# Unsigned-Long/slam-tricks

Hardware: AMD Instinct MI355X
Metric: LM iterations/sec + residuals/sec, 1k-cam/100k-pt BA (higher is better)
Workload: dtype f64

## Files before the change

slam-tricks_amd/csrc/ba_kernels.hip:

```cpp
#include <algorithm>

#include "ba_kernels.hpp"

namespace stba {

template <bool CAMS_IN_LDS, bool WITH_JAC>
__global__ __launch_bounds__(LIN_THREADS) void ba_linearize_kernel(LinArgs a) {
    extern __shared__ __attribute__((aligned(16))) double smem[];
    double* s_j8 = smem;
    double* s_cam = smem + (WITH_JAC ? LIN_THREADS * 9 : 0);
    const int tid = threadIdx.x;
    if (CAMS_IN_LDS) {
        for (int i = tid; i < a.n_cams * 7; i += LIN_THREADS) s_cam[i] = a.cams[i];
        __syncthreads();
    }
    double cost = 0.0;
    const int n_tiles = (a.n_obs + LIN_THREADS - 1) / LIN_THREADS;
    for (int tile = blockIdx.x; tile < n_tiles; tile += gridDim.x) {
        const int base = tile * LIN_THREADS;
        const int i = base + tid;
        if (i < a.n_obs) {
            const double2 f = a.feat[i];
            const int c = a.obs_cam[i], j = a.obs_pt[i];
            const double* cam = CAMS_IN_LDS ? (s_cam + c * 7) : (a.cams + (size_t)c * 7);
// ... 451 lines not shown
#pragma unroll
        for (int k = 0; k < 6; ++k) Hi[k] = 0.0;
    }
#pragma unroll
    for (int k = 0; k < 6; ++k) Hinv6[(size_t)j * 6 + k] = Hi[k];
}

__global__ __launch_bounds__(256) void ba_point_damp_invert_kernel(int n_pts, const double* __restrict__ Hpp6,
                                                                   const unsigned char* __restrict__ pt_fixed,
                                                                   double* __restrict__ scale, int init_scale, int use_scaling,
                                                                   double radius, double dmin, double dmax, double* __restrict__ dp,
                                                                   double* __restrict__ Hinv6, double* __restrict__ zero_buf, int zero_n) {
    const int j = blockIdx.x * 256 + threadIdx.x;
    if (j < zero_n) zero_buf[j] = 0.0;
    if (j >= n_pts) return;
    double H[6], Hi[6] = {0, 0, 0, 0, 0, 0};
#pragma unroll
    for (int k = 0; k < 6; ++k) H[k] = Hpp6[(size_t)j * 6 + k];
    const int dg[3] = {0, 3, 5};
#pragma unroll
    for (int k = 0; k < 3; ++k) {
        const size_t i = (size_t)j * 3 + k;
        const double h = H[dg[k]];
        double s = 1.0;
        if (use_scaling) {
            if (init_scale) { s = 1.0 / (1.0 + sqrt(h)); scale[i] = s; }
            else s = scale[i];
        } else if (init_scale) scale[i] = 1.0;
        const double s2 = s * s;
        const double v = fmin(fmax(h * s2, dmin), dmax);
        const double d = v / radius / s2;
        dp[i] = d;
        H[dg[k]] = h + d;
    }
    const bool fixed = pt_fixed ? (pt_fixed[j] != 0) : false;
    if (fixed || !inv3_sym6(H, Hi)) {
#pragma unroll
        for (int k = 0; k < 6; ++k) Hi[k] = 0.0;
    }
#pragma unroll
    for (int k = 0; k < 6; ++k) Hinv6[(size_t)j * 6 + k] = Hi[k];
}

int launch_point_damp_invert(int n_pts, const double* Hpp6, const unsigned char* pt_fixed, double* scale, int init_scale,
                             int use_scaling, double radius, double dmin, double dmax, double* dp, double* Hinv6,
                             double* zero_buf, int zero_n, hipStream_t st) {
    hipLaunchKernelGGL(ba_point_damp_invert_kernel, dim3((std::max(n_pts, zero_n) + 255) / 256), dim3(256), 0, st, n_pts, Hpp6, pt_fixed, scale,
                       init_scale, use_scaling, radius, dmin, dmax, dp, Hinv6, zero_buf, zero_n);
    STBA_HIP(hipGetLastError());
    return STBA_OK;
}

int launch_point_invert(int n_pts, const double* Hpp6, const double* dp, const unsigned char* pt_fixed,
                        double* Hinv6, hipStream_t st) {
    hipLaunchKernelGGL(ba_point_invert_kernel, dim3((n_pts + 255) / 256), dim3(256), 0, st, n_pts, Hpp6, dp,
                       pt_fixed, Hinv6);
    STBA_HIP(hipGetLastError());
    return STBA_OK;
}

template <int ROTS, bool GEN = false, int MODE = 0>
__global__ __launch_bounds__(SCHUR_THREADS, GEN ? 2 : 4) void ba_schur_pairs_kernel(SchurArgs a) {
    extern __shared__ __attribute__((aligned(16))) double smem[];
    const int task = blockIdx.x;
    const int c = a.task_cam[task];
    const int row_ncols = a.row_col_ptr[c + 1] - a.row_col_ptr[c];
    const int clo = a.task_col_lo[task], chi = a.task_col_hi[task];
    const int col0 = a.row_col_ptr[c] + clo, ncols = chi - clo;
    double* acc = smem;
    double* racc = smem + (size_t)a.max_cols * SCHUR_BLK_LD;
    double* cpart = racc + 8;
    int* cols = reinterpret_cast<int*>(cpart + 8 * SCHUR_CAM_LD);
    int* vsf = cols + a.max_cols;
    const int tid = threadIdx.x;
    const bool diag_piece = (chi == row_ncols);
    const int* vs_g = a.vs_first + a.task_vs_ptr[task];
    const int nslots = vs_g[ncols];
    for (int e = tid; e < nslots * SCHUR_BLK_LD; e += SCHUR_THREADS) acc[e] = 0.0;
    if (tid < 8) racc[tid] = 0.0;
    for (int e = tid; e < ncols; e += SCHUR_THREADS) cols[e] = a.row_cols[col0 + e];
    for (int e = tid; e <= ncols; e += SCHUR_THREADS) vsf[e] = vs_g[e];
    if (tid == 0) vsf[a.max_cols + 1] = 0;
    const bool lms = a.part != nullptr;
    if (!lms) {
        const int cend = min(a.lda, ((c * 6 + 5) / 128 + 1) * 128);
        const int z0 = (clo == 0) ? 0 : 6 * a.row_cols[col0];
        const int z1 = diag_piece ? cend : 6 * a.row_cols[col0 + ncols];
        for (int q = 0; q < 6; ++q) {
            double* row = a.S + (size_t)(c * 6 + q) * a.lda;
            for (int e = z0 + tid; e < z1; e += SCHUR_THREADS) row[e] = 0.0;
        }
    }
    __syncthreads();
    const int wv = tid >> 6;
    constexpr int mode = MODE;
    const int stride = mode == 0 ? 64 : SCHUR_THREADS;
    const int ent = task * (SCHUR_THREADS / 64) + (mode == 0 ? wv : 0);
    const int kb = a.pair_begin[ent], ke = a.pair_end[ent];
    const int ntrips = (ke - kb + stride - 1) / stride;
    int* turn = vsf + a.max_cols + 1;
    int k = kb + (mode == 0 ? (tid & 63) : tid);
    int4 rn = (k < ke) ? a.pair_rec[k] : make_int4(0, 0, 0, 0);
    for (int trip = 0; mode == 0 ? (k < ke) : (trip < ntrips); ++trip, k += stride) {
        const int4 rc = rn;
        const bool valid = mode == 0 ? true : (k < ke);
        if (k + stride < ke) rn = a.pair_rec[k + stride];
        if (mode == 1) {
        }
        double Hi[6], jc[12], jp[6], jc2[12], jp2[6];
#ifdef STBA_DEBUG_KNOBS
        const int gi = (a.ablate & 1) ? (rc.x & 63) : rc.x, gl = (a.ablate & 1) ? (rc.y & 63) : rc.y, gz = (a.ablate & 1) ? (rc.z & 63) : rc.z;
#else
        const int gi = rc.x, gl = rc.y, gz = rc.z;
#endif
#pragma unroll
        for (int k2 = 0; k2 < 6; ++k2) Hi[k2] = a.Hinv6[(size_t)gz * 6 + k2];
        load_jc_jp<GEN>(a.J8, a.omask, gi, jc, jp, a.Jc12);
        load_jc_jp<GEN>(a.J8, a.omask, gl, jc2, jp2, a.Jc12);
        const unsigned sl = (unsigned)rc.w;
        const int rot = (int)((sl >> 16) & 7u);
        double E[18];
#pragma unroll
        for (int q = 0; q < 6; ++q) {
            const double w0 = jc[q] * jp[0] + jc[6 + q] * jp[3];
            const double w1 = jc[q] * jp[1] + jc[6 + q] * jp[4];
            const double w2 = jc[q] * jp[2] + jc[6 + q] * jp[5];
            E[q * 3 + 0] = w0 * Hi[0] + w1 * Hi[1] + w2 * Hi[2];
            E[q * 3 + 1] = w0 * Hi[1] + w1 * Hi[3] + w2 * Hi[4];
            E[q * 3 + 2] = w0 * Hi[2] + w1 * Hi[4] + w2 * Hi[5];
        }
        double* blk = acc + (size_t)(sl & 0x3fffu) * SCHUR_BLK_LD;
        if (mode == 1) {
            const int want = trip * (SCHUR_THREADS / 64) + wv;
            while (__hip_atomic_load(turn, __ATOMIC_RELAXED, __HIP_MEMORY_SCOPE_WORKGROUP) != want) __builtin_amdgcn_s_sleep(1);
        }
        if (valid) {
#pragma unroll
        for (int s2 = 0; s2 < 6; ++s2) {
            double ja = jc2[s2], jb = jc2[6 + s2];
            int b = s2;
#pragma unroll
            for (int r = 1; r < ROTS; ++r) {
                const int bb = (s2 + r * (6 / ROTS)) % 6;
                if (rot == r) { ja = jc2[bb]; jb = jc2[6 + bb]; b = bb; }
            }
            const double w0 = ja * jp2[0] + jb * jp2[3];
            const double w1 = ja * jp2[1] + jb * jp2[4];
            const double w2 = ja * jp2[2] + jb * jp2[5];
            double* col = blk + b;
#ifdef STBA_DEBUG_KNOBS
            if (a.ablate & 2) {
                double sacc = 0.0;
#pragma unroll
                for (int q = 0; q < 6; ++q) sacc += E[q * 3] * w0 + E[q * 3 + 1] * w1 + E[q * 3 + 2] * w2;
                if (sacc == 1.2345e300) unsafeAtomicAdd(&col[0], sacc);
            } else
#endif
#pragma unroll
            for (int q = 0; q < 6; ++q)
                unsafeAtomicAdd(&col[q * 6], -(E[q * 3] * w0 + E[q * 3 + 1] * w1 + E[q * 3 + 2] * w2));
        }
        }
        if (mode == 1) {
            asm volatile("s_waitcnt lgkmcnt(0)" ::: "memory");
            if ((tid & 63) == 0) __hip_atomic_store(turn, trip * (SCHUR_THREADS / 64) + wv + 1, __ATOMIC_RELAXED, __HIP_MEMORY_SCOPE_WORKGROUP);
        }
    }
    if (diag_piece) {
        const int pb = lms ? a.task_p_lo[task] : a.cam_start[c];
        const int pe = lms ? a.task_p_hi[task] : a.cam_start[c + 1];
        {
            double h[27];
#pragma unroll
            for (int k = 0; k < 27; ++k) h[k] = 0.0;
            for (int p = pb + tid; p < pe; p += SCHUR_THREADS) {
// ... 1008 lines not shown
```

slam-tricks_amd/csrc/common.hpp:

```cpp
#pragma once
#include <hip/hip_runtime.h>

#include <chrono>
#include <cmath>
#include <cstdio>
#include <cstdlib>
#include <cstring>
#include <mutex>
#include <string>

#include "../../include/stba.h"

namespace stba {

extern thread_local std::string g_last_error;
inline int fail(int code, const std::string& msg) {
    g_last_error = msg;
    return code;
}
#define STBA_HIP(call)                                                                       \
    do {                                                                                     \
        hipError_t e_ = (call);                                                              \
        if (e_ != hipSuccess) {                                                              \
            return ::stba::fail((e_ == hipErrorNoDevice || e_ == hipErrorInvalidDevice)      \
// ... 83 lines not shown
        for (int q = 7; q >= 0; --q) w[q] = src[q];
        double st;
        std::memcpy(&st, &w[7], sizeof st);
        if (!accept(st) || (L > 0 && st != first_stamp)) return false;
        first_stamp = st;
        unsigned long long chk = stamped_mix(STAMPED_SALT, w[7]);
        for (int q = 0; q < STAMPED_PAYLOAD; ++q) chk = stamped_mix(chk, w[q]);
        if (chk != w[6]) return false;
        for (int q = 0; q < STAMPED_PAYLOAD; ++q) {
            const int pi = L * STAMPED_PAYLOAD + q;
            if (pi < n_payload) std::memcpy(&payload[pi], &w[q], sizeof(double));
        }
    }
    if (stamp_out) *stamp_out = first_stamp;
    return true;
}

enum class StreamState { running, finished, failed };
constexpr unsigned long STAMPED_QUERY_EVERY = 1ul << 14;
template <class Accept, class StreamCheck>
inline int stamped_wait(const volatile double* block, int n_payload, Accept accept, double* payload, StreamCheck stream_state,
                        const char* who, double limit_s) {
    const auto t0 = std::chrono::steady_clock::now();
    for (unsigned long n = 1; !stamped_try_read(block, n_payload, accept, payload); ++n) {
        if (n % STAMPED_QUERY_EVERY == 0) {
            std::string why;
            const StreamState s = stream_state(&why);
            if (s == StreamState::failed) return fail(STBA_ERR_HIP, std::string(who) + ": stream failed: " + why);
            if (s == StreamState::finished) {
                if (stamped_try_read(block, n_payload, accept, payload)) return STBA_OK;
                return fail(STBA_ERR_HIP, std::string(who) + ": the stream finished without writing the block the host waits for");
            }
            if (std::chrono::duration<double>(std::chrono::steady_clock::now() - t0).count() > limit_s)
                return fail(STBA_ERR_HIP, std::string(who) + ": timed out waiting for the device");
        }
#if defined(__x86_64__)
        __builtin_ia32_pause();
#endif
    }
    return STBA_OK;
}
inline auto hip_stream_state(hipStream_t st) {
    return [st](std::string* why) {
        hipError_t q = hipStreamQuery(st);
        if (q == hipErrorNotReady) return StreamState::running;
        if (q == hipSuccess) q = hipStreamSynchronize(st);
        if (q == hipSuccess) return StreamState::finished;
        *why = hipGetErrorString(q);
        return StreamState::failed;
    };
}

struct MappedBuffer {
    double* host = nullptr;
    double* dev = nullptr;
    size_t count = 0;
    int alloc(size_t n) {
        release();
        void *h = nullptr, *d = nullptr;
        STBA_HIP(hipHostMalloc(&h, n * sizeof(double), hipHostMallocMapped | hipHostMallocCoherent));
        const hipError_t e = hipHostGetDevicePointer(&d, h, 0);
        if (e != hipSuccess) {
            (void)hipHostFree(h);
            return fail(STBA_ERR_HIP, std::string("hipHostGetDevicePointer: ") + hipGetErrorString(e));
        }
        host = static_cast<double*>(h); dev = static_cast<double*>(d); count = n;
        zero();
        return STBA_OK;
    }
    void zero() { if (host) memset(host, 0, count * sizeof(double)); }
    void release() {
        if (host) (void)hipHostFree(host);
        host = dev = nullptr;
        count = 0;
    }
};

constexpr int CHOL_NB = 128;
inline int chol_padded_dim(int n) { return ((n + 1 + CHOL_NB - 1) / CHOL_NB) * CHOL_NB; }
constexpr int CHOL_FLAG_TIMEOUT = -2147483647;
inline int chol_flag_status(int flag_h) {
    return flag_h == CHOL_FLAG_TIMEOUT ? fail(STBA_ERR_HIP, "dense Cholesky: the persistent program timed out waiting for a dependency and the caller has no way to rebuild the matrix") : STBA_OK;
}
int chol_factor_solve_dev(double* A_dev, int lda, int n, double* x_dev, int* flag_dev, hipStream_t st);
int chol_factor_solve_stages(double* A_dev, int lda, int n, double* x_dev, int* flag_dev, hipStream_t st);
void chol_forget_stream(hipStream_t st);
void chol_note_timeout();
void chol_note_peer_timeout();
void chol_count_timeout();
void chol_set_spin_limit_us(double us);
int chol_timeout_count();

int chol_factor_solve_split(double* A_dev, int lda, int n, double* x_dev, int* flag_dev, hipStream_t st, hipEvent_t mid_event,
                            hipEvent_t pre_event = nullptr);
struct CholProfile {
    double ms_diag, ms_trsm, ms_syrk, ms_bwd;
    double syrk_flops;
    double syrk_flops_padded;
    int syrk_launches;
};
int chol_factor_solve_profiled(double* A_dev, int lda, int n, double* x_dev, int* flag_dev, hipStream_t st,
                               CholProfile* prof);
double chol_schedule_makespan(int nblk, int nq, int wg_per_q);
void chol_shard_model(int nblk, int n_gpus, int n_xcd, int wg_per_q, int rows_per_group, double hop_us, double tile_us, double* out3);
int chol_shard_row_owner(int row, int n_gpus, int rows_per_group);
int chol_prepare_padding_dev(double* A_dev, int lda, int n, const double* rhs_dev, hipStream_t st);
size_t chol_yyt_workspace_doubles(int lda, size_t kcols);
int chol_yyt_lower_dev(const double* Y, size_t ldy, size_t kcols, double* S, int lda, double* ws, hipStream_t st);
size_t chol_spd_inverse_workspace_doubles(int np);
int chol_spd_inverse_dev(double* W, int ldw, int np, int n_real, int* flag_dev, double* work, hipStream_t st);

__host__ __device__ inline void quat_to_rot(const double q[4], double R[9]) {
    const double x = q[0], y = q[1], z = q[2], w = q[3];
    const double xx = x * x, yy = y * y, zz = z * z;
    const double xy = x * y, xz = x * z, yz = y * z, wx = w * x, wy = w * y, wz = w * z;
    R[0] = 1 - 2 * (yy + zz); R[1] = 2 * (xy - wz);     R[2] = 2 * (xz + wy);
    R[3] = 2 * (xy + wz);     R[4] = 1 - 2 * (xx + zz); R[5] = 2 * (yz - wx);
    R[6] = 2 * (xz - wy);     R[7] = 2 * (yz + wx);     R[8] = 1 - 2 * (xx + yy);
}

__host__ __device__ inline void so3_exp(const double w[3], double q[4]) {
    const double th2 = w[0] * w[0] + w[1] * w[1] + w[2] * w[2];
    double imag, real;
    if (th2 < 1e-20) {
        const double th4 = th2 * th2;
        imag = 0.5 - th2 / 48.0 + th4 / 3840.0;
        real = 1.0 - th2 / 8.0 + th4 / 384.0;
    } else {
        const double th = sqrt(th2);
        imag = sin(0.5 * th) / th;
        real = cos(0.5 * th);
    }
    q[0] = imag * w[0]; q[1] = imag * w[1]; q[2] = imag * w[2]; q[3] = real;
}

__host__ __device__ inline void so3_plus(const double q[4], const double d[3], double out[4]) {
    double e[4];
    so3_exp(d, e);
    const double ax = q[0], ay = q[1], az = q[2], aw = q[3];
    const double bx = e[0], by = e[1], bz = e[2], bw = e[3];
    const double ox = aw * bx + ax * bw + ay * bz - az * by;
    const double oy = aw * by - ax * bz + ay * bw + az * bx;
    const double oz = aw * bz + ax * by - ay * bx + az * bw;
    const double ow = aw * bw - ax * bx - ay * by - az * bz;
    const double n = sqrt(ox * ox + oy * oy + oz * oz + ow * ow);
    out[0] = ox / n; out[1] = oy / n; out[2] = oz / n; out[3] = ow / n;
}

__host__ __device__ inline void left_jacobian_coeffs(double th2, double& a, double& b) {
    if (th2 < 1e-20) { a = 0.5 - th2 / 24.0; b = 1.0 / 6.0 - th2 / 120.0; return; }
    const double th = sqrt(th2), s = sin(0.5 * th) / (0.5 * th);
    a = 0.5 * s * s;
    b = (th - sin(th)) / (th2 * th);
}

__host__ __device__ inline void se3_exp_rt(const double xi[6], double R[9], double t[3]) {
    double q[4];
    so3_exp(xi + 3, q);
    quat_to_rot(q, R);
    const double w0 = xi[3], w1 = xi[4], w2 = xi[5];
    double a, b;
    left_jacobian_coeffs(w0 * w0 + w1 * w1 + w2 * w2, a, b);
    const double K[9] = {0, -w2, w1, w2, 0, -w0, -w1, w0, 0};
    double K2[9];
    for (int i = 0; i < 3; ++i)
        for (int j = 0; j < 3; ++j) K2[i * 3 + j] = K[i * 3] * K[j] + K[i * 3 + 1] * K[3 + j] + K[i * 3 + 2] * K[6 + j];
    for (int i = 0; i < 3; ++i) {
        double s = 0.0;
// ... 61 lines not shown
```

slam-tricks_amd/csrc/dense_chol.hip:

```cpp
#include <algorithm>
#include <atomic>
#include <cstdlib>
#include <map>
#include <mutex>
#include <queue>
#include <string>
#include <vector>

#include "common.hpp"

namespace stba {

constexpr int NB = CHOL_NB;
#ifndef MEGA_WAIT_SLEEP
#define MEGA_WAIT_SLEEP 1
#endif
#ifndef MEGA_POLL_SLEEP
#define MEGA_POLL_SLEEP 16
#endif

typedef double double4v __attribute__((ext_vector_type(4)));

__global__ void chol_pad_kernel(double* __restrict__ A, int lda, int n, const double* __restrict__ rhs) {
    const int r = n + blockIdx.x;
// ... 240 lines not shown
#pragma unroll
            for (int d = C - 1; d >= 1; --d) acc[d] = __builtin_amdgcn_mfma_f64_16x16x4f64(-lj[d], lprev, acc[d], 0, 0, 0);
            acc[0] = __builtin_amdgcn_mfma_f64_16x16x4f64(-lprev, lprev, acc[0], 0, 0, 0);
        }
        lprev = l;
    }
    if (C == 2) {
#pragma unroll
        for (int r = 0; r < 4; ++r) { sm.Mig[R & 1][0][r][lane] = acc[1][r]; sm.Mig[R & 1][1][r][lane] = acc[0][r]; }
    }
}

__device__ __forceinline__ void d2_bulk_row(const double* __restrict__ Ab, int lda, Diag2Smem& sm, int lane, int R) {
    const int n = lane & 15, g = lane >> 4;
    double4v acc[8];
#pragma unroll
    for (int d = 0; d < 8; ++d) if (d <= R) acc[d] = d2_load_tile(sm, R, R - d, n, g);
    double lprev = 0.0;
    switch (R) {
        case 7: d2_bulk_column<7>(sm, R, acc, lprev, lane); [[fallthrough]];
        case 6: d2_bulk_column<6>(sm, R, acc, lprev, lane); [[fallthrough]];
        case 5: d2_bulk_column<5>(sm, R, acc, lprev, lane); [[fallthrough]];
        case 4: d2_bulk_column<4>(sm, R, acc, lprev, lane); [[fallthrough]];
        case 3: d2_bulk_column<3>(sm, R, acc, lprev, lane); [[fallthrough]];
        default: d2_bulk_column<2>(sm, R, acc, lprev, lane);
    }
}

template <bool WT>
__device__ __forceinline__ void d2_bulk_wave(const double* __restrict__ Ab, int lda, Diag2Smem& sm, int lane, int R, int einv,
                                             double* __restrict__ dinv) {
    const int n = lane & 15, g = lane >> 4;
    d2_bulk_row(Ab, lda, sm, lane, R);
    double4v accE;
    auto inverse_step = [&](int I, int s) {
        const double le = mfma_l(sm.Gp[4 * I + s][lane], accE[s]);
        gst<WT>(&dinv[(I * 16 + 4 * s + g) * 16 + n], le);
        if (s < 3) accE = __builtin_amdgcn_mfma_f64_16x16x4f64(-sm.Lsl[d2_tix(I, I)][s][lane], le, accE, 0, 0, 0);
    };
#pragma unroll 1
    for (int J = R - 1; J < 8; ++J) {
        const int Ie = einv == 0 ? J - 1 : (einv == 1 && J == R - 1) ? 0 : -1;
        if (Ie >= 0) {
#pragma unroll
            for (int r = 0; r < 4; ++r) accE[r] = (n == 4 * r + g) ? 1.0 : 0.0;
        }
#pragma unroll
        for (int s = 0; s < 4; ++s) {
            D2_BARRIER();
            if (Ie >= 0) inverse_step(Ie, s);
        }
        if (J < 7) D2_BARRIER();
    }
    D2_BARRIER();
    if (einv == 1) {
#pragma unroll
        for (int r = 0; r < 4; ++r) accE[r] = (n == 4 * r + g) ? 1.0 : 0.0;
#pragma unroll
        for (int s = 0; s < 4; ++s) inverse_step(7, s);
    }
}

template <bool WT>
__device__ __forceinline__ void d2_store_wave(double* __restrict__ A, const double* __restrict__ Ab, int lda, int k0, Diag2Smem& sm, int lane) {
    d2_bulk_row(Ab, lda, sm, lane, 2);
#pragma unroll 1
    for (int J = 1; J < 8; ++J) {
#pragma unroll
        for (int s = 0; s < 4; ++s) {
            D2_BARRIER();
#pragma unroll
            for (int h = 0; h < 2; ++h) {
                const int Ip = (J - 1) + 2 * s + h;
                if (Ip < 8) d2_store_tile<WT>(A, lda, k0, sm, Ip, J - 1, lane);
            }
        }
        if (J < 7) D2_BARRIER();
    }
    D2_BARRIER();
    d2_store_tile<WT>(A, lda, k0, sm, 7, 7, lane);
}

template <bool WT>
__device__ __forceinline__ void diag_block2(double* __restrict__ A, int lda, int k0, int n_real,
                                            int* __restrict__ flag, double* __restrict__ dinv, double* smem, int t,
                                            long long* ph = nullptr) {
    Diag2Smem& sm = *reinterpret_cast<Diag2Smem*>(smem);
    const int w = __builtin_amdgcn_readfirstlane(t >> 6), lane = t & 63;
    const double* Ab = A + (size_t)k0 * lda + k0;
    PHASE_STAMP(0);
    d2_stage_block(Ab, lda, sm, t);
    D2_BARRIER();
    if (w == 0) d2_factor_wave(Ab, lda, k0, n_real, flag, sm, lane, ph);
    else if (w == 1) d2_follower_wave(Ab, lda, sm, lane);
    else if (w == 4) d2_store_wave<WT>(A, Ab, lda, k0, sm, lane);
    else d2_bulk_wave<WT>(Ab, lda, sm, lane, w == 5 ? 5 : w == 2 ? 7 : w == 6 ? 3 : w == 3 ? 6 : 4, w == 6 ? 0 : w == 7 ? 1 : -1, dinv);
}

__global__ __launch_bounds__(512) void chol_diag_kernel(double* __restrict__ A, int lda, int k0, int n_real,
                                                         int* __restrict__ flag, double* __restrict__ dinv) {
    extern __shared__ __attribute__((aligned(16))) double sm2[];
    diag_block2<false>(A, lda, k0, n_real, flag, dinv, sm2, threadIdx.x);
}

template <bool WT>
__device__ __forceinline__ void trsm_group(double* __restrict__ rowp, bool ident, int ident_row0, int nv,
                                           const double* __restrict__ Lb, int lda,
                                           const double* __restrict__ dinv, int lane) {
    const int n = lane & 15, g = lane >> 4;
    const int pm = 4 * (n & 3) + (n >> 2);
    double4v W[8];
#pragma unroll
    for (int J = 0; J < 8; ++J) {
        if (ident) {
#pragma unroll
            for (int r = 0; r < 4; ++r) W[J][r] = (16 * J + 4 * g + r == ident_row0 + n) ? 1.0 : 0.0;
        } else {
            W[J] = gld4(rowp + 16 * J + 4 * g);
        }
    }
    auto load_l = [&](int J, int I) -> double4v {
        const int row = 16 * J + pm;
        double4v v = gld4(Lb + (size_t)row * lda + 16 * I + 4 * g);
        if (row >= nv) v = double4v{0.0, 0.0, 0.0, 0.0};
        return -v;
    };
    auto load_inv = [&](int J) -> double4v {
        double4v v = gld4(dinv + (J * 16 + pm) * 16 + 4 * g);
        if (16 * J + pm >= nv) {
#pragma unroll
            for (int q = 0; q < 4; ++q) v[q] = (4 * g + q == pm) ? 1.0 : 0.0;
        }
        return v;
    };
    double4v Lc[8], Ln[8], iv, ivn;
    iv = load_inv(0);
#pragma unroll
    for (int J = 1; J < 8; ++J) Lc[J] = load_l(J, 0);
#pragma unroll
    for (int I = 0; I < 8; ++I) {
        if (I + 1 < 8) {
            ivn = load_inv(I + 1);
#pragma unroll
            for (int J = I + 2; J < 8; ++J) Ln[J] = load_l(J, I + 1);
        }
        double4v y = {0.0, 0.0, 0.0, 0.0};
#pragma unroll
        for (int q = 0; q < 4; ++q) y = __builtin_amdgcn_mfma_f64_16x16x4f64(iv[q], W[I][q], y, 0, 0, 0);
        W[I] = y;
#pragma unroll
        for (int J = I + 1; J < 8; ++J)
#pragma unroll
            for (int q = 0; q < 4; ++q) W[J] = __builtin_amdgcn_mfma_f64_16x16x4f64(Lc[J][q], y[q], W[J], 0, 0, 0);
        iv = ivn;
#pragma unroll
        for (int J = I + 2; J < 8; ++J) Lc[J] = Ln[J];
    }
#pragma unroll
    for (int J = 0; J < 8; ++J) gst4<WT>(rowp + 16 * J + 4 * g, W[J]);
}

__global__ __launch_bounds__(64) void chol_trsm_kernel(double* __restrict__ A, int lda, int k0, int n_groups,
                                                       double* __restrict__ Xinv, const double* __restrict__ dinv) {
    const int lane = threadIdx.x, grp = blockIdx.x;
    const bool ident = grp >= n_groups;
    const int e = grp - n_groups;
    const int nv = ident ? min(NB, (lda - 1) - k0) : NB;
    double* rowp = ident ? Xinv + (size_t)(16 * e + (lane & 15)) * NB
                         : A + (size_t)(k0 + NB + 16 * grp + (lane & 15)) * lda + k0;
    trsm_group<false>(rowp, ident, 16 * e, nv, A + (size_t)k0 * lda + k0, lda, dinv, lane);
}

template <int TM>
__global__ __launch_bounds__(256) void chol_syrk_kernel(double* __restrict__ A, int lda, int k0, int tile_mode) {
    constexpr int RBA = TM / 16;
    constexpr int WR = TM / 64;
    constexpr int WC = 4 / WR;
    constexpr int MB = 4;
    constexpr int NBK = 8 / WC;
    constexpr int PA = TM / 64;
    __shared__ __attribute__((aligned(16))) double sA[2][TM * 16];
    __shared__ __attribute__((aligned(16))) double sB[2][2048];
    const int sub = (TM == 64) ? (blockIdx.x & 1) : 0;
    const int id = (TM == 64) ? (blockIdx.x >> 1) : blockIdx.x;
    int ti, tj;
// ... 19 lines not shown
#pragma unroll
            for (int r = 0; r < 4; ++r) {
                const int row = row_i + wr * (MB * 16) + m * 16 + (lane >> 4) + 4 * r;
                const int col = row_j + wc * (NBK * 16) + n * 16 + (lane & 15);
                acc[m][n][r] = A[(size_t)row * lda + col];
            }

    double2 ga[PA][2], gb[2][2];
    const int lrow = lane & 15, lkp = lane >> 4;
    auto gload = [&](int kc) {
#pragma unroll
        for (int p = 0; p < 2; ++p)
#pragma unroll
            for (int h = 0; h < 2; ++h) {
                const int row = lrow + 16 * (w + 4 * p);
                const int k = 2 * (lkp + 4 * h);
                if (p < PA) ga[p < PA ? p : 0][h] = *reinterpret_cast<const double2*>(&A[(size_t)(row_i + row) * lda + k0 + kc * 16 + k]);
                gb[p][h] = *reinterpret_cast<const double2*>(&A[(size_t)(row_j + row) * lda + k0 + kc * 16 + k]);
            }
    };
    auto lstore = [&](int buf) {
#pragma unroll
        for (int p = 0; p < 2; ++p)
#pragma unroll
            for (int h = 0; h < 2; ++h) {
                const int rb = w + 4 * p;
                const int k = 2 * (lkp + 4 * h);
                if (p < PA) {
                    const int posa = (((k >> 2) * RBA + rb) << 6) + ((k & 3) << 4) + lrow;
                    sA[buf][posa] = ga[p < PA ? p : 0][h].x;
                    sA[buf][posa + 16] = ga[p < PA ? p : 0][h].y;
                }
                const int posb = (((k >> 2) * 8 + rb) << 6) + ((k & 3) << 4) + lrow;
                sB[buf][posb] = gb[p][h].x;
                sB[buf][posb + 16] = gb[p][h].y;
            }
    };
    gload(0);
    lstore(0);
    __syncthreads();
    constexpr int KC = NB / 16;
    for (int kc = 0; kc < KC; ++kc) {
        const int buf = kc & 1;
        if (kc + 1 < KC) gload(kc + 1);
#pragma unroll
        for (int kq = 0; kq < 4; ++kq) {
            double a[MB], b[NBK];
#pragma unroll
            for (int m = 0; m < MB; ++m) a[m] = -sA[buf][((kq * RBA + wr * MB + m) << 6) + lane];
#pragma unroll
            for (int n = 0; n < NBK; ++n) b[n] = sB[buf][((kq * 8 + wc * NBK + n) << 6) + lane];
#pragma unroll
            for (int m = 0; m < MB; ++m)
#pragma unroll
                for (int n = 0; n < NBK; ++n)
                    acc[m][n] = __builtin_amdgcn_mfma_f64_16x16x4f64(a[m], b[n], acc[m][n], 0, 0, 0);
        }
        if (kc + 1 < KC) lstore(buf ^ 1);
        __syncthreads();
    }
#pragma unroll
    for (int m = 0; m < MB; ++m)
#pragma unroll
        for (int n = 0; n < NBK; ++n)
#pragma unroll
            for (int r = 0; r < 4; ++r) {
                const int row = row_i + wr * (MB * 16) + m * 16 + (lane >> 4) + 4 * r;
                const int col = row_j + wc * (NBK * 16) + n * 16 + (lane & 15);
                A[(size_t)row * lda + col] = acc[m][n][r];
            }
}

static void launch_syrk(double* A, int lda, int k0, int tile_mode, int tiles128, hipStream_t st) {
    const bool use64 = tiles128 < 1000000;
    if (use64) hipLaunchKernelGGL(chol_syrk_kernel<64>, dim3(2 * tiles128), dim3(256), 0, st, A, lda, k0, tile_mode);
    else hipLaunchKernelGGL(chol_syrk_kernel<128>, dim3(tiles128), dim3(256), 0, st, A, lda, k0, tile_mode);
}

enum { TASK_D = 0, TASK_T = 1, TASK_TI = 2, TASK_U = 3, TASK_UQ = 4, TASK_TU = 5 };

constexpr int MEGA_MAX_Q = 16;
struct MegaArgs {
    double* A; int lda; int n; int nblk;
    const int4* tasks;
    int nq;
    int lstart[MEGA_MAX_Q + 1];
    signed char xcc_queue[16];
    int* sync;
    double* linv; size_t linv_stride;
    double* vbuf; int nwide;
    long long spin_limit;
    int* flag;
    long long* trace;
};
constexpr int MEGA_SYNC_HDR = MEGA_MAX_Q + 1;
constexpr int MEGA_ABORT = MEGA_MAX_Q;
constexpr int MEGA_SMEM_BYTES = 128 * 1024;
constexpr int MEGA_PREDRAW_NB = 2;

__device__ __forceinline__ int xcc_id() {
    unsigned v;
    asm volatile("s_getreg_b32 %0, hwreg(HW_REG_XCC_ID)" : "=s"(v));
    return (int)(v & 15u);
}
__global__ void xcc_probe_kernel(int* out) {
    if (threadIdx.x == 0) out[blockIdx.x] = xcc_id();
}

template <int TM, int KCH = 16>
__device__ __forceinline__ void syrk_tile512(double* __restrict__ A, int lda, int k0, int row_i, int row_j,
                                             double* smem, int t, int kchunks = NB / 16) {
    constexpr int WR = (TM == 128) ? 2 : 1, WC = 8 / WR;
    constexpr int MB = TM / (16 * WR);
    constexpr int NBK = 8 / WC;
    constexpr int RBA = TM / 16;
    constexpr int SA = TM * KCH, SB = 128 * KCH, NH = KCH / 8;
    double* sA = smem;
    double* sB = smem + 2 * SA;
    const int lane = t & 63, w = t >> 6;
    const int wr = w / WC, wc = w % WC;
    double4v acc[MB][NBK];
#pragma unroll
    for (int m = 0; m < MB; ++m)
#pragma unroll
        for (int n = 0; n < NBK; ++n)
#pragma unroll
            for (int r = 0; r < 4; ++r) {
                const int row = row_i + wr * (MB * 16) + m * 16 + (lane >> 4) + 4 * r;
                const int col = row_j + wc * (NBK * 16) + n * 16 + (lane & 15);
                acc[m][n][r] = A[(size_t)row * lda + col];
            }
    double2 ga[NH], gb[NH];
    const int lrow = lane & 15, lkp = lane >> 4;
    const bool stage_a = (RBA == 8) ? true : (w < RBA);
    auto gload = [&](int kc) {
#pragma unroll
        for (int h = 0; h < NH; ++h) {
            const int row = lrow + 16 * w;
            const int k = 2 * (lkp + 4 * h);
            if (stage_a) ga[h] = *reinterpret_cast<const double2*>(&A[(size_t)(row_i + row) * lda + k0 + kc * KCH + k]);
            gb[h] = *reinterpret_cast<const double2*>(&A[(size_t)(row_j + row) * lda + k0 + kc * KCH + k]);
        }
    };
    auto lstore = [&](int buf) {
#pragma unroll
        for (int h = 0; h < NH; ++h) {
            const int k = 2 * (lkp + 4 * h);
            if (stage_a) {
                const int posa = (((k >> 2) * RBA + w) << 6) + ((k & 3) << 4) + lrow;
                sA[buf * SA + posa] = -ga[h].x;
                sA[buf * SA + posa + 16] = -ga[h].y;
            }
            const int posb = (((k >> 2) * 8 + w) << 6) + ((k & 3) << 4) + lrow;
            sB[buf * SB + posb] = gb[h].x;
            sB[buf * SB + posb + 16] = gb[h].y;
        }
    };
    gload(0);
    lstore(0);
    __syncthreads();
    const int KC = kchunks * 16 / KCH;
    auto chunk = [&](int kc, int buf) {
        if (kc + 1 < KC) gload(kc + 1);
#pragma unroll
        for (int kq = 0; kq < KCH / 4; ++kq) {
            double a[MB], b[NBK];
#pragma unroll
            for (int m = 0; m < MB; ++m) a[m] = sA[buf * SA + (((kq * RBA + wr * MB + m) << 6) + lane)];
#pragma unroll
            for (int n = 0; n < NBK; ++n) b[n] = sB[buf * SB + (((kq * 8 + wc * NBK + n) << 6) + lane)];
#pragma unroll
            for (int m = 0; m < MB; ++m)
#pragma unroll
                for (int n = 0; n < NBK; ++n)
                    acc[m][n] = __builtin_amdgcn_mfma_f64_16x16x4f64(a[m], b[n], acc[m][n], 0, 0, 0);
        }
        if (kc + 1 < KC) lstore(buf ^ 1);
        __syncthreads();
    };
    for (int kc = 0; kc < KC; ++kc) chunk(kc, kc & 1);
#pragma unroll
    for (int m = 0; m < MB; ++m)
#pragma unroll
        for (int n = 0; n < NBK; ++n)
#pragma unroll
            for (int r = 0; r < 4; ++r) {
                const int row = row_i + wr * (MB * 16) + m * 16 + (lane >> 4) + 4 * r;
                const int col = row_j + wc * (NBK * 16) + n * 16 + (lane & 15);
                gst<false>(&A[(size_t)row * lda + col], acc[m][n][r]);
            }
}

template <int TM>
__device__ __forceinline__ void syrk_tile512_gen(double* __restrict__ Cb, int ldc, const double* __restrict__ Pi, size_t ldi,
                                             const double* __restrict__ Pj, size_t ldj, bool c_zero, double* smem, int t, int kchunks = NB / 16) {
    constexpr int WR = (TM == 128) ? 2 : 1, WC = 8 / WR;
    constexpr int MB = TM / (16 * WR);
    constexpr int NBK = 8 / WC;
    constexpr int RBA = TM / 16;
    double* sA = smem;
    double* sB = smem + 2 * TM * 16;
    const int lane = t & 63, w = t >> 6;
    const int wr = w / WC, wc = w % WC;
    double4v acc[MB][NBK];
#pragma unroll
    for (int m = 0; m < MB; ++m)
#pragma unroll
        for (int n = 0; n < NBK; ++n)
#pragma unroll
            for (int r = 0; r < 4; ++r) {
                const int row = wr * (MB * 16) + m * 16 + (lane >> 4) + 4 * r;
                const int col = wc * (NBK * 16) + n * 16 + (lane & 15);
                acc[m][n][r] = c_zero ? 0.0 : Cb[(size_t)row * ldc + col];
// ... 69 lines not shown
        if (wall_clock64() - t0 > limit) {
            __hip_atomic_store(abortf, 1, __ATOMIC_RELAXED, __HIP_MEMORY_SCOPE_AGENT);
            return false;
        }
    }
}

__device__ __forceinline__ bool trsm_compute512(double4v (&W)[8], const double* __restrict__ rowp, bool ident,
                                                int ident_row0, int nv, const double* __restrict__ Lb, int lda,
                                                const double* __restrict__ dinv, double* smem, int t, long long* ph,
                                                const int* dflag, int* abortf, int* s_ok, long long spin_limit, bool flag_known = false,
                                                bool active = true) {
    const int lane = t & 63;
    const int n = lane & 15, g = lane >> 4;
#pragma unroll
    for (int J = 0; J < 8; ++J) {
        if (!active) {
#pragma unroll
            for (int r = 0; r < 4; ++r) W[J][r] = 0.0;
        } else if (ident) {
#pragma unroll
            for (int r = 0; r < 4; ++r) W[J][r] = (16 * J + 4 * g + r == ident_row0 + n) ? 1.0 : 0.0;
        } else {
            W[J] = gld4(rowp + 16 * J + 4 * g);
        }
    }
    if (!flag_known) {
        if (t == 0) {
            *s_ok = mega_wait(dflag, 1, abortf, spin_limit) ? 1 : 0;
            asm volatile("buffer_inv sc1\n\ts_waitcnt vmcnt(0)" ::: "memory");
        }
        __syncthreads();
        if (!*s_ok) return false;
    }
    {
        double v[18];
#pragma unroll
        for (int s2 = 0; s2 < 18; ++s2) {
            const int e = t + 512 * s2;
            const int tile = e >> 8, r = (e >> 4) & 15, c = e & 15;
            if (s2 < 14) {
                const int I = (tile >= 27) ? 6 : (tile >= 25) ? 5 : (tile >= 22) ? 4 : (tile >= 18) ? 3 : (tile >= 13) ? 2 : (tile >= 7) ? 1 : 0;
                const int J = tile - (7 * I - I * (I - 1) / 2) + I + 1;
                const int row = 16 * J + r;
                v[s2] = -Lb[(size_t)row * lda + 16 * I + c];
                if (row >= nv) v[s2] = 0.0;
            } else {
                const int J = tile - 28;
                v[s2] = dinv[(J * 16 + r) * 16 + c];
                if (16 * J + r >= nv) v[s2] = (c == r) ? 1.0 : 0.0;
            }
        }
#pragma unroll
        for (int s2 = 0; s2 < 18; ++s2) {
            const int e = t + 512 * s2;
            const int tile = e >> 8, r = (e >> 4) & 15, c = e & 15;
            const int nn = 4 * (r & 3) + (r >> 2);
            smem[tile * 256 + (((c >> 2) << 4) | nn) * 4 + (c & 3)] = v[s2];
        }
    }
    __syncthreads();
    PHASE_STAMP(0);
    if (active) {
#pragma unroll
    for (int I = 0; I < 8; ++I) {
        const double4v iv = *reinterpret_cast<const double4v*>(smem + (28 + I) * 256 + lane * 4);
        double4v y = {0.0, 0.0, 0.0, 0.0};
#pragma unroll
        for (int q = 0; q < 4; ++q) y = __builtin_amdgcn_mfma_f64_16x16x4f64(iv[q], W[I][q], y, 0, 0, 0);
        W[I] = y;
#pragma unroll
        for (int J = I + 1; J < 8; ++J) {
            const int tile = 7 * I - I * (I - 1) / 2 + (J - I - 1);
            const double4v l = *reinterpret_cast<const double4v*>(smem + tile * 256 + lane * 4);
#pragma unroll
            for (int q = 0; q < 4; ++q) W[J] = __builtin_amdgcn_mfma_f64_16x16x4f64(l[q], y[q], W[J], 0, 0, 0);
        }
    }
    }
    PHASE_STAMP(1);
    return true;
}

__device__ __forceinline__ bool trsm_task512(double* __restrict__ rowp, bool ident, int ident_row0, int nv,
                                             const double* __restrict__ Lb, int lda,
                                             const double* __restrict__ dinv, double* smem, int t, long long* ph,
                                             const int* dflag, int* abortf, int* s_ok, long long spin_limit, bool flag_known = false,
                                             bool active = true) {
    double4v W[8];
    if (!trsm_compute512(W, rowp, ident, ident_row0, nv, Lb, lda, dinv, smem, t, ph, dflag, abortf, s_ok, spin_limit, flag_known, active)) return false;
    const int g = (t & 63) >> 4;
    if (active) {
#pragma unroll
        for (int J = 0; J < 8; ++J) gst4<true>(rowp + 16 * J + 4 * g, W[J]);
    }
    PHASE_STAMP(2);
    return true;
}

__device__ __forceinline__ bool tu4_task512(double* __restrict__ A, int lda, int k0, int rb, int q,
                                           const double* __restrict__ dinv, double* smem, int t, long long* ph,
                                           int* loaded, int* ver_diag, const int* dflag, int* abortf, int* s_ok, long long spin_limit,
                                           bool flag_known = false) {
    const int lane = t & 63, w = t >> 6;
    const int n = lane & 15, g = lane >> 4;
    double* rowp = A + (size_t)(rb * NB + 16 * w + n) * lda + k0;
    const int ntile = 4 * q + 3;
    double* Cb = A + (size_t)(rb * NB) * lda + rb * NB;
    double4v acc[2];
    int tm[2], tn[2];
#pragma unroll
    for (int s2 = 0; s2 < 2; ++s2) {
        const int e = w + 8 * s2;
        tm[s2] = (e < 2 * q + 1) ? 2 * q : 2 * q + 1;
        tn[s2] = (e < 2 * q + 1) ? e : e - (2 * q + 1);
        if (e < ntile) {
#pragma unroll
            for (int r = 0; r < 4; ++r) acc[s2][r] = Cb[(size_t)(16 * tm[s2] + g + 4 * r) * lda + 16 * tn[s2] + n];
        }
    }
    double4v W[8];
    if (!trsm_compute512(W, rowp, false, 0, NB, A + (size_t)k0 * lda + k0, lda, dinv, smem, t, ph, dflag, abortf, s_ok, spin_limit, flag_known)) return false;
    __syncthreads();
    if (t == 0) __hip_atomic_fetch_add(loaded, 1, __ATOMIC_RELAXED, __HIP_MEMORY_SCOPE_AGENT);
#pragma unroll
    for (int J = 0; J < 8; ++J) *reinterpret_cast<double4v*>(smem + (w * 8 + J) * 256 + lane * 4) = W[J];
    __syncthreads();
#pragma unroll
    for (int s2 = 0; s2 < 2; ++s2) {
        if (w + 8 * s2 < ntile) {
            const int m = tm[s2], np = tn[s2];
#pragma unroll
            for (int c = 0; c < 8; ++c) {
                const double4v fa = *reinterpret_cast<const double4v*>(smem + (m * 8 + c) * 256 + lane * 4);
                const double4v fb = *reinterpret_cast<const double4v*>(smem + (np * 8 + c) * 256 + lane * 4);
#pragma unroll
                for (int qq = 0; qq < 4; ++qq) acc[s2] = __builtin_amdgcn_mfma_f64_16x16x4f64(-fa[qq], fb[qq], acc[s2], 0, 0, 0);
            }
#pragma unroll
            for (int r = 0; r < 4; ++r) gst<false>(&Cb[(size_t)(16 * m + g + 4 * r) * lda + 16 * np + n], acc[s2][r]);
        }
    }
    asm volatile("s_waitcnt vmcnt(0)" ::: "memory");
    __syncthreads();
    if (t == 0) {
        __hip_atomic_fetch_add(ver_diag, 1, __ATOMIC_RELAXED, __HIP_MEMORY_SCOPE_AGENT);
        *s_ok = mega_wait(loaded, 4, abortf, spin_limit) ? 1 : 0;
    }
    __syncthreads();
    if (!*s_ok) return false;
    if ((w >> 1) == q) {
#pragma unroll
        for (int J = 0; J < 8; ++J) gst4<true>(rowp + 16 * J + 4 * g, W[J]);
    }
    PHASE_STAMP(2);
    return true;
}

constexpr int MEGA_NTU = 10;
__device__ __forceinline__ bool tu_task512(double* __restrict__ A, int lda, int k0, int rb, int q,
                                           const double* __restrict__ dinv, double* smem, int t, long long* ph,
                                           int* loaded, int* done_cnt, int* ver_diag, const int* dflag, int* abortf, int* s_ok, long long spin_limit,
                                           bool flag_known = false) {
    const int lane = t & 63, w = t >> 6;
    const int n = lane & 15, g = lane >> 4;
    int I = 0;
    while ((I + 1) * (I + 2) / 2 <= q) ++I;
    const int J = q - I * (I + 1) / 2;
    const bool diag = (I == J);
    const int nrow = diag ? 2 : 4;
    const bool active = w < nrow;
    const int trow = (w < 2) ? 2 * I + (w & 1) : 2 * J + (w & 1);
    double* rowp = A + (size_t)(rb * NB + 16 * trow + n) * lda + k0;
    const int ntile = diag ? 3 : 4;
    const int lm = diag ? (w >= 1 ? 1 : 0) : (w >> 1), ln = diag ? (w == 2 ? 1 : 0) : 2 + (w & 1);
    const int tm = 2 * I + lm, tn = diag ? 2 * I + ln : 2 * J + (w & 1);
    double* Cb = A + (size_t)(rb * NB) * lda + rb * NB;
    double4v acc = {0.0, 0.0, 0.0, 0.0};
    if (w < ntile) {
#pragma unroll
        for (int r = 0; r < 4; ++r) acc[r] = Cb[(size_t)(16 * tm + g + 4 * r) * lda + 16 * tn + n];
    }
    double4v W[8];
    if (!trsm_compute512(W, rowp, false, 0, NB, A + (size_t)k0 * lda + k0, lda, dinv, smem, t, ph, dflag, abortf, s_ok, spin_limit, flag_known, active)) return false;
    __syncthreads();
    if (t == 0) __hip_atomic_fetch_add(loaded, 1, __ATOMIC_RELAXED, __HIP_MEMORY_SCOPE_AGENT);
    if (active) {
#pragma unroll
        for (int J2 = 0; J2 < 8; ++J2) *reinterpret_cast<double4v*>(smem + (w * 8 + J2) * 256 + lane * 4) = W[J2];
    }
    __syncthreads();
    if (w < ntile) {
#pragma unroll
        for (int c = 0; c < 8; ++c) {
            const double4v fa = *reinterpret_cast<const double4v*>(smem + (lm * 8 + c) * 256 + lane * 4);
            const double4v fb = *reinterpret_cast<const double4v*>(smem + (ln * 8 + c) * 256 + lane * 4);
#pragma unroll
            for (int qq = 0; qq < 4; ++qq) acc = __builtin_amdgcn_mfma_f64_16x16x4f64(-fa[qq], fb[qq], acc, 0, 0, 0);
        }
#pragma unroll
        for (int r = 0; r < 4; ++r) gst<false>(&Cb[(size_t)(16 * tm + g + 4 * r) * lda + 16 * tn + n], acc[r]);
    }
    asm volatile("s_waitcnt vmcnt(0)" ::: "memory");
    __syncthreads();
    if (t == 0) {
        if (__hip_atomic_fetch_add(done_cnt, 1, __ATOMIC_RELAXED, __HIP_MEMORY_SCOPE_AGENT) == MEGA_NTU - 1)
            __hip_atomic_fetch_add(ver_diag, 4, __ATOMIC_RELAXED, __HIP_MEMORY_SCOPE_AGENT);
        *s_ok = (!diag || mega_wait(loaded, MEGA_NTU, abortf, spin_limit)) ? 1 : 0;
    }
    __syncthreads();
    if (!*s_ok) return false;
    if (diag && active) {
#pragma unroll
        for (int J2 = 0; J2 < 8; ++J2) gst4<true>(rowp + 16 * J2 + 4 * g, W[J2]);
    }
    PHASE_STAMP(2);
    return true;
}

__device__ __forceinline__ void syrk_q32(double* __restrict__ A, int lda, int k0, int row_i, int row_j, int t, long long* ph) {
    const int lane = t & 63, w = t >> 6;
    const int n = lane & 15, g = lane >> 4;
    const double* pa0 = A + (size_t)(row_i + n) * lda + k0 + 4 * g;
    const double* pa1 = pa0 + (size_t)16 * lda;
    const double* pb = A + (size_t)(row_j + 16 * w + n) * lda + k0 + 4 * g;
    double4v a0[8], a1[8], bb[8], acc[2];
#pragma unroll
    for (int c = 0; c < 8; ++c) { bb[c] = gld4(pb + 16 * c); a0[c] = gld4(pa0 + 16 * c); a1[c] = gld4(pa1 + 16 * c); }
#pragma unroll
    for (int m = 0; m < 2; ++m)
#pragma unroll
        for (int r = 0; r < 4; ++r) acc[m][r] = A[(size_t)(row_i + 16 * m + g + 4 * r) * lda + row_j + 16 * w + n];
    PHASE_STAMP(0);
#pragma unroll
    for (int c = 0; c < 8; ++c)
#pragma unroll
        for (int q = 0; q < 4; ++q) {
            acc[0] = __builtin_amdgcn_mfma_f64_16x16x4f64(-a0[c][q], bb[c][q], acc[0], 0, 0, 0);
            acc[1] = __builtin_amdgcn_mfma_f64_16x16x4f64(-a1[c][q], bb[c][q], acc[1], 0, 0, 0);
        }
#pragma unroll
    for (int m = 0; m < 2; ++m)
#pragma unroll
        for (int r = 0; r < 4; ++r) gst<false>(&A[(size_t)(row_i + 16 * m + g + 4 * r) * lda + row_j + 16 * w + n], acc[m][r]);
    PHASE_STAMP(1);
}

__global__ __launch_bounds__(256) void chol_reset_kernel(int* __restrict__ sync, int n, int* __restrict__ flag) {
    const int i = blockIdx.x * 256 + threadIdx.x;
    if (i < n) sync[i] = 0;
    if (i == 0) flag[0] = 0;
}

struct MegaView {
    int nblk, nrow;
    int* abortf; int* dflag; int* tuflag; int* tudone; int* tflag; int* ver;
};
__device__ __forceinline__ MegaView mega_view(const MegaArgs& a) {
    MegaView v;
    v.nblk = a.nblk;
    v.nrow = a.nblk + 4 * a.nwide;
    v.abortf = a.sync + MEGA_ABORT;
    v.dflag = a.sync + MEGA_SYNC_HDR;
    v.tuflag = v.dflag + a.nblk;
    v.tudone = v.tuflag + a.nblk;
    v.tflag = v.tudone + a.nblk;
    v.ver = v.tflag + a.nblk * v.nrow;
    return v;
}
__device__ __forceinline__ int mega_ldf(const int* p) { return __hip_atomic_load(p, __ATOMIC_RELAXED, __HIP_MEMORY_SCOPE_AGENT); }
__device__ __forceinline__ bool mega_ready(const MegaView& v, const int4 d, bool& tu_dset) {
    const int type = d.x & 0xff, b = d.y, ti = d.z, tj = d.w;
    const int nblk = v.nblk, nrow = v.nrow;
    auto first_panel = [&](int i) { return i < nblk ? 0 : i - nblk; };
    if (type == TASK_D) return mega_ldf(&v.ver[b * nblk + b]) >= 4 * b;
    if (type == TASK_T) {
        const int ve = mega_ldf(&v.ver[ti * nblk + b]), df = mega_ldf(&v.dflag[b]);
        return (ve >= 4 * (b - first_panel(ti))) & (df >= 1);
    }
    if (type == TASK_TI) return mega_ldf(&v.dflag[b]) >= 1;
    if (type == TASK_TU) {
        const int v0 = mega_ldf(&v.ver[(b + 1) * nblk + b]), v1 = mega_ldf(&v.ver[(b + 1) * nblk + b + 1]), df = mega_ldf(&v.dflag[b]);
        tu_dset = df >= 1;
        return (v0 >= 4 * b) & (v1 >= 4 * b);
    }
    const int i = (type == TASK_UQ) ? (ti >> 2) : ti;
    const int nbp = max(1, (d.x >> 16) & 0xff);
    const int f0 = mega_ldf(&v.tflag[b * nrow + i]), f1 = mega_ldf(&v.tflag[b * nrow + tj]), ve = mega_ldf(&v.ver[i * nblk + tj]);
    return (f0 >= 4) & (f1 >= 4) & (ve >= 4 * (b - nbp + 1 - first_panel(i)));
}

struct MegaTicket {
    int mine = -1;
    int4 md;
    bool done = false;
    int m_raw = 0;
    bool m_pending = false;
};
__device__ __forceinline__ int mega_next_task(const MegaArgs& a, const MegaView& v, MegaTicket& tk, int* ticket, int lbeg, int lend, int lane,
                                              bool& ok, bool& tu_dset, long long& t_poll) {
    t_poll = a.trace ? wall_clock64() : 0;
    ok = true;
    if (tk.mine < 0 && !tk.done) {
        if (!tk.m_pending && lane == 0) tk.m_raw = lbeg + atomicAdd(ticket, 1);
        tk.m_pending = false;
        tk.mine = __builtin_amdgcn_readfirstlane(tk.m_raw);
        if (tk.mine >= lend) { tk.mine = -1; tk.done = true; }
        else tk.md = a.tasks[tk.mine];
    }
    int pick = -2;
    if (tk.mine >= 0) {
        const long long t0 = wall_clock64();
        for (;;) {
            if (mega_ready(v, tk.md, tu_dset)) { pick = tk.mine; tk.mine = -1; break; }
            if (mega_ldf(v.abortf) != 0) { ok = false; pick = -1; break; }
            if (wall_clock64() - t0 > a.spin_limit) {
                __hip_atomic_store(v.abortf, 1, __ATOMIC_RELAXED, __HIP_MEMORY_SCOPE_AGENT);
                ok = false; pick = -1;
                break;
            }
            __builtin_amdgcn_s_sleep(MEGA_POLL_SLEEP);
        }
    }
    asm volatile("buffer_inv sc1\n\ts_waitcnt vmcnt(0)" ::: "memory");
    return pick;
}

__global__ __launch_bounds__(512) void chol_mega_kernel(MegaArgs a) {
    extern __shared__ __attribute__((aligned(16))) double smem[];
    __shared__ int s_task, s_ok, s_dset;
    const int t = threadIdx.x;
    const int nblk = a.nblk;
    const MegaView v = mega_view(a);
    int* abortf = v.abortf;
    int* dflag = v.dflag;
    int* tuflag = v.tuflag;
    const int nrow = v.nrow;
    int* tflag = v.tflag;
    int* ver = v.ver;
    auto tile_ptr = [&](int i, int j, int& ld) -> double* {
        if (i < nblk) { ld = a.lda; return a.A + (size_t)i * NB * a.lda + (size_t)j * NB; }
        const int p = i - nblk, qw = p >> 2;
        ld = 4 * NB;
        return a.vbuf + (size_t)qw * (4 * NB) * (4 * NB) + (size_t)(p & 3) * NB * (4 * NB) + (size_t)(j - 4 * qw) * NB;
    };
    auto first_panel = [&](int i) { return i < nblk ? 0 : i - nblk; };
    const int q = a.xcc_queue[xcc_id()];
    if (q < 0) return;
    int* ticket = a.sync + q;
    const int lbeg = a.lstart[q], lend = a.lstart[q + 1];
    MegaTicket tk;
    for (;;) {
        if (t < 64) {
            bool ok, tu_dset = false;
            long long t_poll;
            const int pick = mega_next_task(a, v, tk, ticket, lbeg, lend, t, ok, tu_dset, t_poll);
            if (t == 0) {
                if (a.trace && pick >= 0) {
                    a.trace[8 * (size_t)pick] = blockIdx.x; a.trace[8 * (size_t)pick + 1] = t_poll;
                    a.trace[8 * (size_t)pick + 2] = wall_clock64();
                }
                s_dset = tu_dset ? 1 : 0;
                s_task = pick;
                s_ok = ok ? 1 : 0;
            }
            if (!tk.done && pick >= 0 && (tk.md.x & 0xff) != TASK_TU && ((tk.md.x >> 16) & 0xff) <= MEGA_PREDRAW_NB) {
                if (t == 0) tk.m_raw = lbeg + atomicAdd(ticket, 1);
                tk.m_pending = true;
            }
        }
        __syncthreads();
        if (!s_ok) {
            if (t == 0) atomicExch(a.flag, CHOL_FLAG_TIMEOUT);
            break;
        }
        const int task = s_task;
        if (task < 0) break;
        const int4 d = a.tasks[task];
        const int type = d.x & 0xff, b = d.y, ti = d.z, tj = d.w;
        const int k0 = b * NB;
        int tt = t;
        asm volatile("" : "+v"(tt));
        double* li = a.linv + (size_t)b * a.linv_stride;
        long long* ph = a.trace ? a.trace + 8 * (size_t)task + 4 : nullptr;
        if (type == TASK_D) {
            diag_block2<true>(a.A, a.lda, k0, a.n, a.flag, li + NB * NB, smem, tt, ph);
        } else if (type == TASK_T) {
            const int lane = tt & 63, w = tt >> 6;
            int ldr;
            const bool active = (tj == 0) || (w < 4);
            const int row_in_tile = (tj == 0 ? 16 * w : 64 * (tj - 1) + 16 * (w & 3)) + (lane & 15);
            double* rowp = tile_ptr(ti, b, ldr) + (size_t)row_in_tile * ldr;
            if (!trsm_task512(rowp, false, 0, NB, a.A + (size_t)k0 * a.lda + k0, a.lda, li + NB * NB, smem, tt, ph, &dflag[b], abortf, &s_ok,
                              a.spin_limit, true, active)) {
                if (t == 0) atomicExch(a.flag, CHOL_FLAG_TIMEOUT);
                break;
            }
        } else if (type == TASK_TI) {
            const int lane = tt & 63, w = tt >> 6;
            const int nv = min(NB, (a.lda - 1) - k0);
            int ldr = NB;
            double* base = li;
            if (b < 4 * a.nwide) base = tile_ptr(nblk + b, b, ldr);
            double* rowp = base + (size_t)(16 * w + (lane & 15)) * ldr;
            if (!trsm_task512(rowp, true, 16 * w, nv, a.A + (size_t)k0 * a.lda + k0, a.lda, li + NB * NB, smem, tt, ph, &dflag[b], abortf, &s_ok,
                              a.spin_limit, true)) {
                if (t == 0) atomicExch(a.flag, CHOL_FLAG_TIMEOUT);
                break;
            }
        } else if (type == TASK_U) {
            if (ti < nblk) {
                const int nbp = max(1, (d.x >> 16) & 0xff);
                syrk_tile512<128>(a.A, a.lda, k0 - (nbp - 1) * NB, ti * NB, tj * NB, smem, tt, nbp * (NB / 16));
            } else {
                int ldc, ldi, ldj;
                double* Cb = tile_ptr(ti, tj, ldc);
                const double* Pi = tile_ptr(ti, b, ldi);
                const double* Pj = tile_ptr(tj, b, ldj);
                syrk_tile512_gen<128>(Cb, ldc, Pi, ldi, Pj, ldj, b == first_panel(ti), smem, tt);
            }
        } else if (type == TASK_TU) {
            const bool tu_ok = (tj == 2)
                ? tu4_task512(a.A, a.lda, k0, b + 1, ti, li + NB * NB, smem, tt, ph, &tuflag[b], &ver[(b + 1) * nblk + b + 1], &dflag[b], abortf, &s_ok,
                              a.spin_limit, s_dset != 0)
                : tu_task512(a.A, a.lda, k0, b + 1, ti, li + NB * NB, smem, tt, ph, &tuflag[b], &v.tudone[b], &ver[(b + 1) * nblk + b + 1], &dflag[b], abortf, &s_ok,
                             a.spin_limit, s_dset != 0);
            if (!tu_ok) {
                if (t == 0) atomicExch(a.flag, CHOL_FLAG_TIMEOUT);
                break;
            }
        } else {
            syrk_q32(a.A, a.lda, k0, (ti >> 2) * NB + (ti & 3) * 32, tj * NB, tt, ph);
        }
        asm volatile("s_waitcnt vmcnt(0)" ::: "memory");
        __syncthreads();
        if (t == 0) {
            if (type == TASK_D) __hip_atomic_fetch_add(&dflag[b], 1, __ATOMIC_RELAXED, __HIP_MEMORY_SCOPE_AGENT);
            else if (type == TASK_T) __hip_atomic_fetch_add(&tflag[b * nrow + ti], tj == 0 ? 4 : 2, __ATOMIC_RELAXED, __HIP_MEMORY_SCOPE_AGENT);
            else if (type == TASK_TI) { if (b < 4 * a.nwide) __hip_atomic_fetch_add(&tflag[b * nrow + nblk + b], 4, __ATOMIC_RELAXED, __HIP_MEMORY_SCOPE_AGENT); }
            else if (type == TASK_TU) { if (tj != 0) __hip_atomic_fetch_add(&tflag[b * nrow + b + 1], 1, __ATOMIC_RELAXED, __HIP_MEMORY_SCOPE_AGENT); }
            else if (type == TASK_U) __hip_atomic_fetch_add(&ver[ti * nblk + tj], 4 * max(1, (d.x >> 16) & 0xff), __ATOMIC_RELAXED, __HIP_MEMORY_SCOPE_AGENT);
            else if (type == TASK_UQ) __hip_atomic_fetch_add(&ver[(ti >> 2) * nblk + tj], 1, __ATOMIC_RELAXED, __HIP_MEMORY_SCOPE_AGENT);
            if (a.trace) a.trace[8 * (size_t)task + 3] = wall_clock64();
        }
    }
}

static int mega_task_row(const int4& tk) {
    switch (tk.x & 0xff) {
        case TASK_D: case TASK_TI: return tk.y;
        case TASK_TU: return tk.y + 1;
        case TASK_T: case TASK_U: return tk.z;
        default: return tk.z >> 2;
    }
}
static std::vector<int> mega_row_owner(int nblk, int nq, int nvirt = 0) {
    std::vector<int> owner((size_t)(nblk + nvirt), 0);
    for (int v = 0; v < nvirt; ++v) owner[(size_t)(nblk + v)] = v % nq;
    std::vector<double> load((size_t)nq, 0.0);
    for (int row = nblk - 1; row >= 0; --row) {
        int best = 0;
        for (int q = 1; q < nq; ++q)
            if (load[(size_t)q] < load[(size_t)best]) best = q;
        owner[(size_t)row] = best;
        load[(size_t)best] += 24.0 * row * (row - 1) / 2.0 + 23.0 * row + 110.0;
    }
    return owner;
}
struct MegaShardModel {
    int n_gpus = 1;
    int rows_per_group = 0;
    double hop_us = 0.0;
    double tile_us = 0.0;
    double cross_edges = 0.0;
    double tiles_in_max = 0.0;
};
static int mega_default_batch(int nblk) {
    const double tiles_per_wg = 0.5 * nblk * nblk / 256.0;
    int b = 2;
    while (b < 16 && tiles_per_wg / b >= 2.2) b *= 2;
    return b;
}
struct MegaMachine {
    int nq = 8;
    int wg = 32;
};
static void mega_build_tasks(int nblk, const MegaMachine& mach, std::vector<int4>& out, int* lstart, std::vector<float>* sim_start = nullptr,
                             double* makespan_out = nullptr, int nwide = 0, MegaShardModel* shard = nullptr) {
    struct Node { int4 tk; std::vector<int> succ; int indeg = 0; double dur = 0, prio = 0, start = 0, ready = 0, avail = 0; int q = 0; int last_pred = -1; };
    std::vector<Node> nodes;
    const int NBK = nblk;
    const int nq = mach.nq;
    const int nl = nq;
    std::vector<int> rowq = mega_row_owner(nblk, nq, 4 * nwide);
    const int n_gpus = shard ? shard->n_gpus : 1, q_per_gpu = nq / std::max(1, n_gpus);
    if (shard && n_gpus > 1) {
        const int R = shard->rows_per_group > 0 ? shard->rows_per_group : q_per_gpu;
        for (int row = 0; row < nblk; ++row) {
            const int local = (row / (R * n_gpus)) * R + row % R;
            rowq[(size_t)row] = ((row / R) % n_gpus) * q_per_gpu + local % q_per_gpu;
        }
    }
    auto gpu_of = [&](int l) { return n_gpus > 1 ? l / q_per_gpu : 0; };
    static const int QROWS = knob_int("STBA_MEGA_QROWS", 2);
    const int THALF_FROM = knob_int("STBA_MEGA_THALF_FROM", std::max(0, nblk - 30));
    static const double THALF_DUR = knob_double("STBA_MEGA_THALF_DUR", 0.6);
    const int TU10_FROM = knob_int("STBA_MEGA_TU10_FROM", std::max(0, nblk - 15));
    static const double TU10_DUR = knob_double("STBA_MEGA_TU10_DUR", 0.65);
    auto ntu = [&](int b) { return b >= TU10_FROM ? MEGA_NTU : 4; };
    const int DQ_FROM = knob_int("STBA_MEGA_DQ_FROM", std::max(0, nblk - 17));
    const int QFROM = knob_int("STBA_MEGA_QFROM", std::max(0, nblk - 17));
    std::vector<int> idD((size_t)NBK, -1), idTI((size_t)NBK, -1), idTU((size_t)NBK * MEGA_NTU, -1), idT((size_t)NBK * NBK, -1), idT2((size_t)NBK * NBK, -1),
        idUq((size_t)NBK * NBK * 4, -1), idU((size_t)NBK * NBK * NBK, -1), idUd((size_t)NBK * 4, -1);
    double DUR[6] = {23.0, 23.0, 19.0, 25.0, 16.5, 20.0};
    double DUR_K = 18.0;
// ... 148 lines not shown
    std::vector<std::vector<double>> idle_since((size_t)nl, std::vector<double>((size_t)mach.wg, 0.0));
    double now = 0.0;
    struct Pick { double key, start; int node; };
    std::vector<std::vector<Pick>> order((size_t)nl);
    auto push_ready = [&](int k) { ready_h[(size_t)nodes[(size_t)k].q].push(PI(nodes[(size_t)k].prio, k)); };
    for (int k = 0; k < (int)nodes.size(); ++k)
        if (nodes[(size_t)k].indeg == 0) push_ready(k);
    double makespan = 0.0;
    std::vector<double> tiles_in((size_t)std::max(1, n_gpus), 0.0);
    for (;;) {
        for (int l = 0; l < nl; ++l) {
            std::vector<double>& idl = idle_since[(size_t)l];
            Heap& hb = ready_h[(size_t)l];
            while (!idl.empty() && !hb.empty()) {
                const int k = hb.top().second;
                hb.pop();
                Node& nd = nodes[(size_t)k];
                const int ty = nd.tk.x & 0xff;
                const double adv = ty == TASK_D ? ADV_D : ty == TASK_TU ? ADV_TU : 0.0;
                order[(size_t)l].push_back({idl.back() - adv, now, k});
                idl.pop_back();
                nd.start = now;
                events.push(PI(now + nd.dur, k));
            }
        }
        if (events.empty()) break;
        const PI ev = events.top();
        events.pop();
        now = ev.first;
        if (ev.second < 0) {
            const int k = -(ev.second + 1);
            nodes[(size_t)k].ready = now;
            push_ready(k);
            continue;
        }
        makespan = now;
        const Node& nd = nodes[(size_t)ev.second];
        idle_since[(size_t)nd.q].push_back(now);
        const int g0 = gpu_of(nd.q);
        unsigned sent_to = 0;
        for (int sidx : nd.succ) {
            Node& sn = nodes[(size_t)sidx];
            double at = now;
            const int g1 = gpu_of(sn.q);
            if (g1 != g0) {
                at += shard->hop_us + shard->tile_us;
                shard->cross_edges += 1.0;
                if (!(sent_to >> g1 & 1u)) { sent_to |= 1u << g1; tiles_in[(size_t)g1] += 1.0; }
            }
            if (at > sn.avail) { sn.avail = at; sn.last_pred = ev.second; }
            if (--sn.indeg == 0) {
                if (sn.avail <= now) { sn.ready = now; push_ready(sidx); }
                else events.push(PI(sn.avail, -(sidx + 1)));
            }
        }
    }
    if (makespan_out) *makespan_out = makespan;
    if (shard) shard->tiles_in_max = *std::max_element(tiles_in.begin(), tiles_in.end());
    if (knob_str("STBA_MEGA_SIMDBG")) {
        static const char* NM[6] = {"D", "T", "TI", "U", "Uq", "TU"};
        for (int b = 0; b + 1 < NBK; ++b) {
            const Node& d0 = nodes[(size_t)idD[(size_t)b]];
            const Node& d1 = nodes[(size_t)idD[(size_t)b + 1]];
            const Node& tu = nodes[(size_t)idTU[(size_t)b * MEGA_NTU + ntu(b) - 1]];
            const double e0 = d0.start + d0.dur;
            fprintf(stderr, "b=%2d step %6.1f | TU ready %+6.1f start %+6.1f | D+1 ready %+6.1f start %+6.1f", b, d1.start - d0.start,
                    tu.ready - e0, tu.start - e0, d1.ready - e0, d1.start - e0);
            int k = idTU[(size_t)b * MEGA_NTU + ntu(b) - 1];
            for (int hop = 0; hop < 4 && k >= 0; ++hop) {
                const Node& nd = nodes[(size_t)k];
                fprintf(stderr, " <- %s(%d;%d,%d) rdy %+.1f st %+.1f", NM[nd.tk.x & 0xff], nd.tk.y, nd.tk.z, nd.tk.w, nd.ready - e0, nd.start - e0);
                k = nd.last_pred;
            }
            fprintf(stderr, "\n");
        }
    }
    out.clear();
    for (int l = 0; l < nl; ++l) {
        std::stable_sort(order[(size_t)l].begin(), order[(size_t)l].end(), [](const Pick& x, const Pick& y) {
            return x.key != y.key ? x.key < y.key : x.start < y.start;
        });
        lstart[l] = (int)out.size();
        for (const Pick& pk : order[(size_t)l]) {
            out.push_back(nodes[(size_t)pk.node].tk);
            if (sim_start) sim_start->push_back((float)pk.start);
        }
    }
    lstart[nl] = (int)out.size();
}

double chol_schedule_makespan(int nblk, int nq, int wg_per_q) {
    std::vector<int4> tasks;
    std::vector<int> lstart((size_t)nq + 1);
    double ms = 0.0;
    MegaMachine m;
    m.nq = nq; m.wg = wg_per_q;
    mega_build_tasks(nblk, m, tasks, lstart.data(), nullptr, &ms);
    return ms;
}

void chol_shard_model(int nblk, int n_gpus, int n_xcd, int wg_per_q, int rows_per_group, double hop_us, double tile_us, double* out3) {
    std::vector<int4> tasks;
    std::vector<int> lstart((size_t)n_gpus * n_xcd + 1);
    MegaShardModel sh;
    sh.n_gpus = n_gpus; sh.rows_per_group = rows_per_group; sh.hop_us = hop_us; sh.tile_us = tile_us;
    double ms = 0.0;
    MegaMachine m;
    m.nq = n_gpus * n_xcd; m.wg = wg_per_q;
    mega_build_tasks(nblk, m, tasks, lstart.data(), nullptr, &ms, 0, &sh);
    out3[0] = ms; out3[1] = sh.cross_edges; out3[2] = sh.tiles_in_max;
}

int chol_shard_row_owner(int row, int n_gpus, int rows_per_group) { return (row / std::max(1, rows_per_group)) % std::max(1, n_gpus); }

constexpr int BWD_ROW_CHUNKS = 8;
__global__ __launch_bounds__(1024) void chol_bwd_step_kernel(double* __restrict__ A, int lda, int k0, int has_next,
                                                             const double* __restrict__ Xinv, double* __restrict__ x) {
    __shared__ double xs[NB];
    __shared__ double part[BWD_ROW_CHUNKS][NB];
    __shared__ double ybuf[NB];
    const int t = threadIdx.x;
    const int kn = k0 + NB;
    const int nvn = has_next ? min(NB, (lda - 1) - kn) : 0;
    constexpr int RPC = NB / BWD_ROW_CHUNKS;
    const int rchunk = t >> 7, c = t & 127;
    const int c0 = (blockIdx.x > 0) ? (blockIdx.x - 1) * NB : k0;
    double lv[RPC];
#pragma unroll
    for (int j = 0; j < RPC; ++j) lv[j] = 0.0;
    if (has_next) {
        const double* col = A + (size_t)(kn + rchunk * RPC) * lda + c0 + c;
#pragma unroll
        for (int j = 0; j < RPC; ++j) lv[j] = col[(size_t)j * lda];
    }
    const int i = t >> 3, p8 = t & 7;
    double xv[16];
    double y_own = 0.0;
    const int nv = min(NB, (lda - 1) - k0);
    if (blockIdx.x == 0) {
        const double* xr = Xinv + (size_t)i * NB + p8 * 16;
#pragma unroll
        for (int j = 0; j < 16; ++j) xv[j] = xr[j];
        if (t < NB) y_own = (t < nv) ? A[(size_t)(lda - 1) * lda + k0 + t] : 0.0;
    }
    double y_upd = 0.0;
    if (blockIdx.x > 0 && t < NB) y_upd = A[(size_t)(lda - 1) * lda + c0 + t];
    if (t < NB) xs[t] = (t < nvn) ? x[kn + t] : 0.0;
    __syncthreads();
    double s = 0.0;
#pragma unroll
    for (int j = 0; j < RPC; ++j) s = fma(lv[j], xs[rchunk * RPC + j], s);
    part[rchunk][c] = s;
    __syncthreads();
    if (blockIdx.x > 0) {
        if (t < NB) {
            double acc = 0.0;
#pragma unroll
            for (int q = 0; q < BWD_ROW_CHUNKS; ++q) acc += part[q][t];
            A[(size_t)(lda - 1) * lda + c0 + t] = y_upd - acc;
        }
        return;
    }
    if (t < NB) {
        double yv = y_own;
#pragma unroll
        for (int q = 0; q < BWD_ROW_CHUNKS; ++q) yv -= part[q][t];
        ybuf[t] = (t < nv) ? yv : 0.0;
// ... 60 lines not shown
    s += __shfl_xor(s, 16, 64);
    if (cc == 0) x[row0 + r] = s;
}

struct MegaDevice {
    std::mutex m;
    bool probed = false;
    int ncu = 0, nq = 0;
    signed char xcc_queue[16];
    hipEvent_t last = nullptr;
    hipStream_t last_stream = nullptr;
    int cooldown = 0;
};
static MegaDevice& mega_device(int dev) {
    static std::mutex mm;
    static std::map<int, MegaDevice> devs;
    std::lock_guard<std::mutex> g(mm);
    return devs[dev];
}

static int mega_device_init(MegaDevice& D, hipStream_t st) {
    if (D.probed) return STBA_OK;
    int dev = 0;
    hipDeviceProp_t prop;
    STBA_HIP(hipGetDevice(&dev));
    STBA_HIP(hipGetDeviceProperties(&prop, dev));
    D.ncu = prop.multiProcessorCount;
    int* probe = nullptr;
    std::vector<int> h((size_t)D.ncu);
    STBA_HIP(hipMalloc(reinterpret_cast<void**>(&probe), h.size() * sizeof(int)));
    hipLaunchKernelGGL(xcc_probe_kernel, dim3(D.ncu), dim3(512), 0, st, probe);
    hipError_t e = hipMemcpyAsync(h.data(), probe, h.size() * sizeof(int), hipMemcpyDeviceToHost, st);
    if (e == hipSuccess) e = hipStreamSynchronize(st);
    (void)hipFree(probe);
    STBA_HIP(e);
    for (int i = 0; i < 16; ++i) D.xcc_queue[i] = -1;
    int per_xcc[16] = {0};
    D.nq = 0;
    for (int x : h) {
        if (D.xcc_queue[x & 15] < 0) D.xcc_queue[x & 15] = (signed char)D.nq++;
        per_xcc[x & 15]++;
    }
    for (int i = 0; i < 16; ++i)
        if (D.xcc_queue[i] >= 0 && per_xcc[i] < MEGA_NTU)
            return fail(STBA_ERR_HIP, "chol: fewer than 10 workgroups per XCD (the TU tasks of a step need one each)");
    if (!D.last) STBA_HIP(hipEventCreateWithFlags(&D.last, hipEventDisableTiming));
    D.probed = true;
    return STBA_OK;
}

void chol_forget_stream(hipStream_t st) {
    for (int dev = 0; dev < 64; ++dev) {
        MegaDevice& D = mega_device(dev);
        std::lock_guard<std::mutex> g(D.m);
        if (D.last_stream == st) D.last_stream = nullptr;
        if (dev > 0 && !D.probed) break;
    }
}

static std::atomic<int> g_timeouts{0};
static std::atomic<long long> g_spin_override{0};
void chol_set_spin_limit_us(double us) { g_spin_override.store(us > 0.0 ? std::max(1LL, (long long)(us * 100.0)) : 0LL); }
void chol_note_timeout() {
    g_timeouts.fetch_add(1);
    int dev = 0;
    if (hipGetDevice(&dev) != hipSuccess) return;
    MegaDevice& D = mega_device(dev);
    std::lock_guard<std::mutex> g(D.m);
    D.cooldown = 64;
}
void chol_count_timeout() { g_timeouts.fetch_add(1); }
void chol_note_peer_timeout() {
    int dev = 0;
    if (hipGetDevice(&dev) != hipSuccess) return;
    MegaDevice& D = mega_device(dev);
    std::lock_guard<std::mutex> g(D.m);
    D.cooldown = 64;
}
int chol_timeout_count() { return g_timeouts.load(); }

enum { CHOL_PERSISTENT = 0, CHOL_STAGES = 1 };

static int chol_run(double* A, int lda, int n, double* x_dev, int* flag_dev, hipStream_t st, CholProfile* prof,
                    hipEvent_t mid_event = nullptr, int schedule = CHOL_PERSISTENT, hipEvent_t pre_event = nullptr) {
    if (lda % NB != 0 || lda < n + 1) return fail(STBA_ERR_INVALID_ARGUMENT, "chol: bad padded dimension");
    const int nblk = lda / NB;
    int cur_dev = 0;
    STBA_HIP(hipGetDevice(&cur_dev));
    if (!prof && schedule == CHOL_PERSISTENT) {
        MegaDevice& D = mega_device(cur_dev);
        std::lock_guard<std::mutex> g(D.m);
        if (D.cooldown > 0) { --D.cooldown; schedule = CHOL_STAGES; }
    }
    const bool stages = prof != nullptr || schedule == CHOL_STAGES;
    constexpr size_t LINV_STRIDE = (size_t)NB * NB + 8 * 256;
    struct MegaPlan {
        int nblk = 0, nwide = -1, ntasks = 0;
        int lstart[MEGA_MAX_Q + 1] = {0};
        int4* tasks = nullptr; int* sync = nullptr; size_t sync_ints = 0;
        double makespan_us = 0.0;
        std::vector<float> sim_start;
    };
    struct DevWs { double* linv = nullptr; int linv_blocks = 0; double* vbuf = nullptr; int vbuf_blocks = 0; MegaPlan plan; };
    static thread_local std::map<int, DevWs> ws_by_dev;
    DevWs& ws = ws_by_dev[cur_dev];
    double*& linv = ws.linv;
    int& linv_blocks = ws.linv_blocks;
    if (linv_blocks < nblk) {
        if (linv) (void)hipFree(linv);
        linv = nullptr; linv_blocks = 0;
        STBA_HIP(hipMalloc(reinterpret_cast<void**>(&linv), (size_t)nblk * LINV_STRIDE * sizeof(double)));
        linv_blocks = nblk;
    }
    const int nwide = stages ? 0 : (nblk - 1) / 4;
    if (ws.vbuf_blocks < nwide) {
        if (ws.vbuf) (void)hipFree(ws.vbuf);
        ws.vbuf = nullptr; ws.vbuf_blocks = 0;
        STBA_HIP(hipMalloc(reinterpret_cast<void**>(&ws.vbuf), (size_t)nwide * 16 * NB * NB * sizeof(double)));
        ws.vbuf_blocks = nwide;
    }
    static DeviceOnce diag_attr;
    STBA_TRY(diag_attr.run([]() -> int {
        STBA_HIP(hipFuncSetAttribute(reinterpret_cast<const void*>(chol_diag_kernel), hipFuncAttributeMaxDynamicSharedMemorySize, (int)sizeof(Diag2Smem)));
        return STBA_OK;
    }));
    auto launch_panel_diag = [&](int b, hipStream_t s_) {
        double* li = linv + (size_t)b * LINV_STRIDE;
        hipLaunchKernelGGL(chol_diag_kernel, dim3(1), dim3(512), sizeof(Diag2Smem), s_, A, lda, b * NB, n, flag_dev, li + NB * NB);
    };
    auto launch_panel_trsm = [&](int b, hipStream_t s_) {
        double* li = linv + (size_t)b * LINV_STRIDE;
        const int groups = (nblk - b - 1) * (NB / 16);
        hipLaunchKernelGGL(chol_trsm_kernel, dim3(groups + NB / 16), dim3(64), 0, s_, A, lda, b * NB, groups, li, li + NB * NB);
    };
    std::vector<hipEvent_t> ev;
    if (prof) {
        ev.resize((size_t)nblk * 4 + 2);
        for (auto& e : ev) STBA_HIP(hipEventCreate(&e));
        memset(prof, 0, sizeof *prof);
    }
    auto mark = [&](size_t k) -> int { if (prof) STBA_HIP(hipEventRecord(ev[k], st)); return STBA_OK; };
    if (stages) {
        {
            MegaDevice& D = mega_device(cur_dev);
            std::lock_guard<std::mutex> dev_lock(D.m);
            if (!D.last) STBA_HIP(hipEventCreateWithFlags(&D.last, hipEventDisableTiming));
            if (D.last_stream != nullptr && D.last_stream != st) {
                STBA_HIP(hipEventRecord(D.last, D.last_stream));
                STBA_HIP(hipStreamWaitEvent(st, D.last, 0));
            }
            D.last_stream = st;
        }
        STBA_HIP(hipMemsetAsync(flag_dev, 0, sizeof(int), st));
        for (int b = 0; b < nblk; ++b) {
            const int k0 = b * NB;
            const int mt = nblk - b - 1;
            STBA_TRY(mark(4 * (size_t)b + 0));
            launch_panel_diag(b, st);
            STBA_TRY(mark(4 * (size_t)b + 1));
            launch_panel_trsm(b, st);
            STBA_TRY(mark(4 * (size_t)b + 2));
            if (mt > 0) launch_syrk(A, lda, k0, 0, mt * (mt + 1) / 2, st);
            STBA_TRY(mark(4 * (size_t)b + 3));
            if (mt > 0 && prof) {
                const double m = std::max(0, n - (k0 + NB));
                prof->syrk_flops += m * (m + 1.0) * NB;
                prof->syrk_flops_padded += (double)(mt * (mt + 1) / 2) * 2.0 * NB * NB * NB;
                prof->syrk_launches += 1;
            }
        }
    } else {
        MegaDevice& D = mega_device(cur_dev);
        std::lock_guard<std::mutex> dev_lock(D.m);
        STBA_TRY(mega_device_init(D, st));
        MegaPlan& plan = ws.plan;
        if (plan.nblk != nblk || plan.nwide != nwide) {
            if (plan.tasks) (void)hipFree(plan.tasks);
            if (plan.sync) (void)hipFree(plan.sync);
            plan = MegaPlan();
            MegaMachine mach;
            mach.nq = D.nq;
            mach.wg = std::max(MEGA_NTU, D.ncu / D.nq);
            std::vector<int4> tasks;
            mega_build_tasks(nblk, mach, tasks, plan.lstart, &plan.sim_start, &plan.makespan_us, nwide);
            STBA_HIP(hipMalloc(reinterpret_cast<void**>(&plan.tasks), tasks.size() * sizeof(int4)));
            STBA_HIP(hipMemcpy(plan.tasks, tasks.data(), tasks.size() * sizeof(int4), hipMemcpyHostToDevice));
            plan.sync_ints = MEGA_SYNC_HDR + 3 * (size_t)nblk + 2 * (size_t)nblk * (nblk + 4 * nwide);
            STBA_HIP(hipMalloc(reinterpret_cast<void**>(&plan.sync), plan.sync_ints * sizeof(int)));
            plan.ntasks = (int)tasks.size();
            plan.nblk = nblk; plan.nwide = nwide;
        }
        hipLaunchKernelGGL(chol_reset_kernel, dim3((unsigned)((plan.sync_ints + 255) / 256)), dim3(256), 0, st, plan.sync, (int)plan.sync_ints, flag_dev);
        MegaArgs ma;
        ma.A = A; ma.lda = lda; ma.n = n; ma.nblk = nblk;
        ma.tasks = plan.tasks; ma.nq = D.nq; ma.sync = plan.sync;
        memcpy(ma.lstart, plan.lstart, sizeof ma.lstart);
        memcpy(ma.xcc_queue, D.xcc_queue, sizeof ma.xcc_queue);
        ma.linv = linv; ma.linv_stride = LINV_STRIDE; ma.flag = flag_dev;
        ma.vbuf = ws.vbuf; ma.nwide = nwide;
        ma.spin_limit = (long long)std::max(25e3, 40.0 * plan.makespan_us) * 100LL;
        if (g_spin_override.load() > 0) ma.spin_limit = g_spin_override.load();
        static const char* TRACE = knob_str("STBA_MEGA_TRACE");
        ma.trace = nullptr;
        if (TRACE) STBA_HIP(hipMalloc(reinterpret_cast<void**>(&ma.trace), (size_t)plan.ntasks * 8 * sizeof(long long)));
        struct TraceGuard { long long*& p; ~TraceGuard() { if (p) { (void)hipFree(p); p = nullptr; } } } trace_guard{ma.trace};
        static DeviceOnce attr_set;
        STBA_TRY(attr_set.run([]() -> int {
            STBA_HIP(hipFuncSetAttribute(reinterpret_cast<const void*>(chol_mega_kernel),
                                         hipFuncAttributeMaxDynamicSharedMemorySize, MEGA_SMEM_BYTES));
            return STBA_OK;
        }));
        if (D.last_stream != nullptr && D.last_stream != st) {
            STBA_HIP(hipEventRecord(D.last, D.last_stream));
            STBA_HIP(hipStreamWaitEvent(st, D.last, 0));
        }
        if (pre_event) STBA_HIP(hipEventRecord(pre_event, st));
        hipLaunchKernelGGL(chol_mega_kernel, dim3(D.ncu), dim3(512), MEGA_SMEM_BYTES, st, ma);
        D.last_stream = st;
        if (TRACE) {
            std::vector<long long> h((size_t)plan.ntasks * 8);
            std::vector<int4> ht((size_t)plan.ntasks);
            STBA_HIP(hipStreamSynchronize(st));
            STBA_HIP(hipMemcpy(h.data(), ma.trace, h.size() * sizeof(long long), hipMemcpyDeviceToHost));
            STBA_HIP(hipMemcpy(ht.data(), plan.tasks, ht.size() * sizeof(int4), hipMemcpyDeviceToHost));
            if (FILE* f = fopen(TRACE, "wb")) {
                fwrite(&plan.ntasks, sizeof(int), 1, f);
                fwrite(ht.data(), sizeof(int4), ht.size(), f);
                fwrite(h.data(), sizeof(long long), h.size(), f);
                fwrite(plan.sim_start.data(), sizeof(float), plan.sim_start.size(), f);
                fclose(f);
            }
        }
    }
    STBA_TRY(mark((size_t)nblk * 4));
    if (mid_event) STBA_HIP(hipEventRecord(mid_event, st));
    for (int b = nblk - 1; b >= 4 * nwide; --b) {
        const int k0 = b * NB;
        const int has_next = (b < nblk - 1) ? 1 : 0;
        const int grid = 1 + (has_next ? b : 0);
        hipLaunchKernelGGL(chol_bwd_step_kernel, dim3(grid), dim3(1024), 0, st, A, lda, k0, has_next, linv + (size_t)b * LINV_STRIDE, x_dev);
    }
    for (int qw = nwide - 1; qw >= 0; --qw) {
        const int row0 = qw * 4 * NB;
        if (qw == nwide - 1) hipLaunchKernelGGL(chol_bwd_apply_kernel<4>, dim3((row0 + 4 * NB) / 32), dim3(1024), 0, st, A, lda, row0 + 4 * NB, x_dev);
        else hipLaunchKernelGGL(chol_bwd_apply_kernel<16>, dim3((row0 + 4 * NB) / 32), dim3(1024), 0, st, A, lda, row0 + 4 * NB, x_dev);
        hipLaunchKernelGGL(chol_bwd_wide_solve_kernel, dim3(4 * NB / BWD_SOLVE_ROWS), dim3(32 * BWD_SOLVE_ROWS), 0, st, A, lda, ws.vbuf + (size_t)qw * 16 * NB * NB, row0, x_dev);
    }
    STBA_TRY(mark((size_t)nblk * 4 + 1));
    STBA_HIP(hipGetLastError());
    if (prof) {
        STBA_HIP(hipStreamSynchronize(st));
        float ms = 0.f;
        for (int b = 0; b < nblk; ++b) {
            (void)hipEventElapsedTime(&ms, ev[4 * (size_t)b + 0], ev[4 * (size_t)b + 1]); prof->ms_diag += ms;
            (void)hipEventElapsedTime(&ms, ev[4 * (size_t)b + 1], ev[4 * (size_t)b + 2]); prof->ms_trsm += ms;
            (void)hipEventElapsedTime(&ms, ev[4 * (size_t)b + 2], ev[4 * (size_t)b + 3]); prof->ms_syrk += ms;
        }
        (void)hipEventElapsedTime(&ms, ev[(size_t)nblk * 4], ev[(size_t)nblk * 4 + 1]); prof->ms_bwd = ms;
        for (auto& e : ev) (void)hipEventDestroy(e);
    }
    return STBA_OK;
}

size_t chol_spd_inverse_workspace_doubles(int np) { return (size_t)(np / NB) * ((size_t)NB * NB + 8 * 256); }
int chol_spd_inverse_dev(double* W, int ldw, int np, int n_real, int* flag_dev, double* work, hipStream_t st) {
    if (np % NB != 0 || ldw != 2 * np || np <= 0) return fail(STBA_ERR_INVALID_ARGUMENT, "chol_spd_inverse_dev: bad dimensions");
    constexpr size_t LINV_STRIDE = (size_t)NB * NB + 8 * 256;
    static DeviceOnce diag_attr;
    STBA_TRY(diag_attr.run([]() -> int {
        STBA_HIP(hipFuncSetAttribute(reinterpret_cast<const void*>(chol_diag_kernel), hipFuncAttributeMaxDynamicSharedMemorySize, (int)sizeof(Diag2Smem)));
        return STBA_OK;
    }));
    STBA_HIP(hipMemsetAsync(flag_dev, 0, sizeof(int), st));
    const int nblk = ldw / NB;
    for (int b = 0; b < np / NB; ++b) {
        double* li = work + (size_t)b * LINV_STRIDE;
        const int mt = nblk - b - 1;
// ... 11 lines not shown
                                                       int per_xcd) {
    extern __shared__ __attribute__((aligned(16))) double smem[];
    const int w = (int)(blockIdx.x % 8) * per_xcd + (int)(blockIdx.x / 8);
    if (blockIdx.x / 8 >= (unsigned)per_xcd || w >= ntiles * nsplit) return;
    const int split = w / ntiles, tile = w % ntiles;
    const int I = tile_ij[tile].x, J = tile_ij[tile].y;
    const int c0 = split * chunks_per_split, c1 = min(chunks_total, c0 + chunks_per_split);
    double* Cb = (nsplit == 1) ? S + (size_t)I * NB * lda + (size_t)J * NB : ws + ((size_t)split * ntiles + tile) * NB * NB;
    const int ldc = (nsplit == 1) ? lda : NB;
    if (c1 <= c0) {
        for (int e = threadIdx.x; e < NB * NB; e += 512) Cb[(size_t)(e / NB) * ldc + e % NB] = 0.0;
        return;
    }
    syrk_tile512_gen<128>(Cb, ldc, Y + (size_t)I * NB * ldy + (size_t)c0 * 16, ldy, Y + (size_t)J * NB * ldy + (size_t)c0 * 16, ldy, true, smem,
                          threadIdx.x, c1 - c0);
}
__global__ __launch_bounds__(256) void yyt_reduce_kernel(const double* __restrict__ ws, int ntiles, int nsplit, double* __restrict__ S, int lda,
                                                         const int2* __restrict__ tile_ij) {
    const int tile = blockIdx.x / (NB * NB / 256);
    const int e = (blockIdx.x % (NB * NB / 256)) * 256 + threadIdx.x;
    const int I = tile_ij[tile].x, J = tile_ij[tile].y;
    const int r = e / NB, c = e % NB;
    double s = 0.0;
    if (nsplit == 1) s = S[((size_t)I * NB + r) * lda + (size_t)J * NB + c];
    else for (int k = 0; k < nsplit; ++k) s += ws[((size_t)k * ntiles + tile) * NB * NB + e];
    if (I == J && c > r) s = 0.0;
    S[((size_t)I * NB + r) * lda + (size_t)J * NB + c] = s;
}
static int yyt_splits(int ntiles, int chunks_total) {
    int ns = (4096 + ntiles - 1) / ntiles;
    ns = std::min(ns, 64);
    ns = std::min(ns, std::max(1, chunks_total / 8));
    return std::max(1, ns);
}
size_t chol_yyt_workspace_doubles(int lda, size_t kcols) {
    const int nb = lda / NB, ntiles = nb * (nb + 1) / 2;
    const int ns = yyt_splits(ntiles, (int)(kcols / 16));
    return ns == 1 ? 0 : (size_t)ns * ntiles * NB * NB;
}
static int yyt_tile_list(int nb, int2** out_dev) {
    static std::mutex m;
    static std::map<std::pair<int, int>, int2*> cache;
    int dev = 0;
    STBA_HIP(hipGetDevice(&dev));
    std::lock_guard<std::mutex> g(m);
    auto it = cache.find({dev, nb});
    if (it == cache.end()) {
        std::vector<int2> h;
        for (int bi = 0; bi * 8 < nb; ++bi)
            for (int bj = 0; bj <= bi; ++bj)
                for (int i = bi * 8; i < std::min(nb, bi * 8 + 8); ++i)
                    for (int j = bj * 8; j < std::min(nb, bj * 8 + 8); ++j)
                        if (j <= i) h.push_back(make_int2(i, j));
        int2* d = nullptr;
        STBA_HIP(hipMalloc(reinterpret_cast<void**>(&d), h.size() * sizeof(int2)));
        STBA_HIP(hipMemcpy(d, h.data(), h.size() * sizeof(int2), hipMemcpyHostToDevice));
        it = cache.emplace(std::make_pair(dev, nb), d).first;
    }
    *out_dev = it->second;
    return STBA_OK;
}
int chol_yyt_lower_dev(const double* Y, size_t ldy, size_t kcols, double* S, int lda, double* ws, hipStream_t st) {
    if (lda % NB != 0 || kcols % 16 != 0 || ldy < kcols) return fail(STBA_ERR_INVALID_ARGUMENT, "chol_yyt_lower_dev: bad dimensions");
    const int nb = lda / NB, ntiles = nb * (nb + 1) / 2;
    const int chunks_total = (int)(kcols / 16);
    const int ns = yyt_splits(ntiles, chunks_total);
    if (ns > 1 && !ws) return fail(STBA_ERR_INVALID_ARGUMENT, "chol_yyt_lower_dev: workspace missing");
    const int cps = (chunks_total + ns - 1) / ns;
    constexpr int LDS = 2 * (128 + 128) * 16 * (int)sizeof(double);
    static DeviceOnce attr;
    STBA_TRY(attr.run([]() -> int {
        STBA_HIP(hipFuncSetAttribute(reinterpret_cast<const void*>(yyt_tile_kernel), hipFuncAttributeMaxDynamicSharedMemorySize, LDS));
        return STBA_OK;
    }));
    int2* tile_ij = nullptr;
    STBA_TRY(yyt_tile_list(nb, &tile_ij));
    const int per_xcd = (ntiles * ns + 7) / 8;
    hipLaunchKernelGGL(yyt_tile_kernel, dim3((unsigned)(per_xcd * 8)), dim3(512), LDS, st, Y, ldy, S, lda, ntiles, ns, cps, chunks_total, ws, tile_ij, per_xcd);
    hipLaunchKernelGGL(yyt_reduce_kernel, dim3((unsigned)(ntiles * (NB * NB / 256))), dim3(256), 0, st, ws, ntiles, ns, S, lda, tile_ij);
    STBA_HIP(hipGetLastError());
    return STBA_OK;
}

int chol_factor_solve_dev(double* A, int lda, int n, double* x_dev, int* flag_dev, hipStream_t st) {
    return chol_run(A, lda, n, x_dev, flag_dev, st, nullptr);
}

int chol_factor_solve_stages(double* A, int lda, int n, double* x_dev, int* flag_dev, hipStream_t st) {
    return chol_run(A, lda, n, x_dev, flag_dev, st, nullptr, nullptr, CHOL_STAGES);
}

int chol_factor_solve_split(double* A, int lda, int n, double* x_dev, int* flag_dev, hipStream_t st, hipEvent_t mid_event, hipEvent_t pre_event) {
    return chol_run(A, lda, n, x_dev, flag_dev, st, nullptr, mid_event, CHOL_PERSISTENT, pre_event);
}

int chol_factor_solve_profiled(double* A, int lda, int n, double* x_dev, int* flag_dev, hipStream_t st,
                               CholProfile* prof) {
    return chol_run(A, lda, n, x_dev, flag_dev, st, prof);
}


}
```

slam-tricks_amd/csrc/stba_engine.hip:

```cpp
#include <algorithm>
#include <atomic>
#include <chrono>
#include <memory>
#include <thread>
#include <vector>

#include "ba_kernels.hpp"
#include "iterative_schur.hpp"
#include "dogleg.hpp"
#include "inner_iterations.hpp"
#include "lm_policy.hpp"

namespace stba {

thread_local std::string g_last_error;

int require_device() {
    int n = 0;
    hipError_t e = hipGetDeviceCount(&n);
    if (e != hipSuccess || n <= 0)
        return fail(STBA_ERR_NO_DEVICE, std::string("no HIP device visible (") +
                                            (e == hipSuccess ? "count=0" : hipGetErrorString(e)) +
                                            "); libstba has no CPU fallback");
    return STBA_OK;
}

template <class T>
static int upload(T* dst, const T* src, size_t count, hipStream_t st) {
    if (count == 0) return STBA_OK;
    STBA_HIP(hipMemcpyAsync(dst, src, count * sizeof(T), hipMemcpyHostToDevice, st));
    return STBA_OK;
}

template <class T>
static int download(T* dst, const T* src, size_t count, hipStream_t st) {
    if (count == 0) return STBA_OK;
    STBA_HIP(hipMemcpyAsync(dst, src, count * sizeof(T), hipMemcpyDeviceToHost, st));
    return STBA_OK;
}

enum { SC_COST2 = 0, SC_GPMAX0 = 8, SC_MAX_WORLD = 64 };
enum { TS_COST2 = 0, TS_STEP2 = 1, TS_X2 = 2, TS_MODEL = 3, TS_TIMEOUT = 4, TS_CAM = 5, TS_COUNT = 8,
       TS_SPEC_COST2 = 8, TS_LIN_COST2 = 9, TS_LIN_GMAX = 10, TS_BLOCK = 11 };

}

using namespace stba;

template <typename F>
static void host_parallel_for(int n, F fn) {
    const int nt = std::max(1, std::min({16, (int)std::thread::hardware_concurrency(), n / 64}));
    if (nt <= 1) { fn(0, n, 0); return; }
    std::vector<std::thread> th;
    for (int k = 0; k < nt; ++k) th.emplace_back([=] { fn((int)((long)n * k / nt), (int)((long)n * (k + 1) / nt), k); });
    for (auto& t : th) t.join();
}

struct stba_ba {
    int nc = 0, np = 0, no = 0, n = 0, lda = 0;
    hipStream_t st = nullptr;
    bool own_stream = false;
    std::vector<int> perm;
    double* cams[2] = {nullptr, nullptr};
    double* pts[2] = {nullptr, nullptr};
    int cur = 0;
    double2* feat = nullptr;
    int *obs_cam = nullptr, *obs_pt = nullptr, *pt_start = nullptr;
    int *cam_perm = nullptr, *chunk_begin = nullptr, *chunk_end = nullptr, *cam_chunk_start = nullptr;
    int n_chunks = 0;
    int *task_cam = nullptr, *cam_start = nullptr, *row_col_ptr = nullptr, *row_cols = nullptr;
    int *task_col_lo = nullptr, *task_col_hi = nullptr;
    int n_tasks = 0, max_cols = 0;
    int *task_p_lo = nullptr, *task_p_hi = nullptr, *row_task_ptr = nullptr, *row_tasks = nullptr;
    long long* task_part_off = nullptr;
    double* schur_part = nullptr;
    bool lm_slices = false;
    std::shared_ptr<void> create_leftovers;
    int *pair_begin = nullptr, *pair_end = nullptr;
    int *task_vs_ptr = nullptr, *vs_first = nullptr;
    int schur_plan_mode = 0;
    int4* pair_rec = nullptr;
    double schur_pairs = 0.0, schur_lds_atomics = 0.0;
    int schur_mode = STBA_SCHUR_PAIRS, schur_mode_auto = STBA_SCHUR_PAIRS;
    bool have_pair_plan = false;
    double* Y = nullptr; size_t ldy = 0, ykcols = 0;
    double *yv = nullptr, *yws = nullptr;
    unsigned char* dup_run = nullptr;
    bool dup_overflow = false;
    int stage_cooldown = 0;
    unsigned char *cam_fixed = nullptr, *pt_fixed = nullptr;
    double2* r = nullptr;
    double* J8 = nullptr;
    stba_ba_linearize_fn hl_fn = nullptr;
    void* hl_user = nullptr;
    double* Jc12 = nullptr;
    std::vector<double> hl_cams, hl_pts, hl_r, hl_jc, hl_jp, hl_stage, hl_cost_stage;
    unsigned char* omask = nullptr;
    double *Hpp6 = nullptr, *gp = nullptr, *Hinv6 = nullptr, *dp = nullptr, *scale_p = nullptr;
    double *Hcc = nullptr, *gc = nullptr, *cam_partial = nullptr, *dc = nullptr, *scale_c = nullptr;
    double* Sbuf = nullptr;
    double *dxc = nullptr, *dxp = nullptr;
    double *cost_partial = nullptr, *upd_partial_c = nullptr, *upd_partial_p = nullptr;
    double* trial = nullptr;
    MappedBuffer ts_host;
    double ts_seq = 0.0;
    double ts_vals[TS_BLOCK] = {0};
    int* flag = nullptr;
    int lin_grid = 1;
    stba_allreduce_fn ar = nullptr;
    void* ar_user = nullptr;
    int rank = 0, world = 1;
    bool have_lin = false, have_blocks = false, have_reduced = false, have_dxc = false, have_dxp = false;
    bool scale_init = false;
    hipEvent_t ev_ar[2] = {};
    bool ar_timing_pending = false, ar_timing_on = false;
    double ar_ms = 0.0, ar_bytes = 0.0; int ar_calls = 0;
    hipEvent_t ev[15] = {};
    CovStore* cov = nullptr;
    bool iterative = false;
    int pcg_precond = STBA_PRECOND_JACOBI, pcg_min = 0, pcg_max = 500, pcg_check = 4;
    double pcg_eta = 0.1;
    stba_pcg_summary pcg_sum{};
    double *pcg_vec = nullptr, *pcg_minv = nullptr, *pcg_sj = nullptr, *pcg_part = nullptr;
    PcgState* pcg_state = nullptr;
    MappedBuffer pcg_host;
    double pcg_seq = 0.0;
    int pcg_last_it = 0, pcg_last_cap = 0;
    std::vector<int> pcg_per_iter;
    int trust_region = STBA_TR_LEVENBERG_MARQUARDT;
    double *dl_uc = nullptr, *dl_up = nullptr, *dl_part = nullptr, *dl_sc = nullptr;
    MappedBuffer dl_host;
    double dl_seq = 0.0;
    stba_dogleg_summary dl_sum{};
    bool inner_on = false;
    double inner_tol = 1e-3;
    struct InnerGroup { int cam_lo, cam_hi, pt_lo, pt_hi; };
    std::vector<InnerGroup> inner_groups;
    std::vector<int> inner_cam_h, inner_pt_h;
    std::vector<unsigned char> inner_mask_h, inner_kind_h;
    int *inner_cam = nullptr, *inner_pt = nullptr, *inner_it = nullptr, *inner_gate = nullptr;
    unsigned char* inner_mask = nullptr;
    double *inner_sc = nullptr, *inner_part = nullptr;
    hipEvent_t inner_ev[2] = {};
    stba_inner_summary inner_sum{};

    size_t s_count() const { return iterative ? 0 : (size_t)lda * lda; }
    double* S() const { return iterative ? nullptr : Sbuf; }
    double* ex_diag() const { return Sbuf + s_count(); }
    double* ex_gc() const { return Sbuf + s_count() + lda; }
    double* rhs() const { return Sbuf + s_count() + 2 * (size_t)lda; }
    double* ex_scalar() const { return Sbuf + s_count() + 3 * (size_t)lda; }
    size_t sbuf_count() const { return s_count() + 4 * (size_t)lda; }
    double* Spack = nullptr;
    std::vector<int> h_row_col_ptr, h_row_cols;
    int pk_state = 0;
    int pk_nz = 0;
    int2* pk_blocks = nullptr;
    size_t pack_count() const {
        return (pk_state == 2 ? (size_t)pk_nz * 36 : (size_t)n * (n + 1) / 2) + 4 * (size_t)lda;
    }
};

namespace stba {

static void ba_free(stba_ba* b) {
    b->create_leftovers.reset();
    cov_store_free(b->cov);
    auto F = [](void* p) { if (p) (void)hipFree(p); };
    F(b->cams[0]); F(b->cams[1]); F(b->pts[0]); F(b->pts[1]); F(b->feat); F(b->obs_cam); F(b->obs_pt);
    F(b->pt_start); F(b->cam_perm); F(b->chunk_begin); F(b->chunk_end); F(b->cam_chunk_start); F(b->cam_fixed);
    F(b->pt_fixed); F(b->r); F(b->J8); F(b->Jc12); F(b->omask); F(b->Hpp6); F(b->gp); F(b->Hinv6); F(b->dp); F(b->scale_p);
    F(b->Hcc); F(b->gc); F(b->cam_partial); F(b->dc); F(b->scale_c); F(b->Sbuf); F(b->Spack); F(b->pk_blocks); F(b->dxc); F(b->dxp);
    F(b->task_cam); F(b->cam_start); F(b->task_col_lo); F(b->task_col_hi); F(b->row_col_ptr); F(b->row_cols);
    F(b->task_p_lo); F(b->task_p_hi); F(b->row_task_ptr); F(b->row_tasks); F(b->task_part_off); F(b->schur_part);
    F(b->pair_begin); F(b->pair_end); F(b->pair_rec); F(b->task_vs_ptr); F(b->vs_first); F(b->Y); F(b->yv); F(b->yws); F(b->dup_run);
    F(b->cost_partial); F(b->upd_partial_c); F(b->upd_partial_p); F(b->trial); F(b->flag);
    F(b->pcg_vec); F(b->pcg_minv); F(b->pcg_sj); F(b->pcg_part); F(b->pcg_state);
    b->pcg_host.release();
    F(b->dl_uc); F(b->dl_up); F(b->dl_part); F(b->dl_sc);
    b->dl_host.release();
    F(b->inner_cam); F(b->inner_pt); F(b->inner_it); F(b->inner_gate); F(b->inner_mask); F(b->inner_sc); F(b->inner_part);
    for (auto& e : b->inner_ev) if (e) (void)hipEventDestroy(e);
    for (auto& e : b->ev) if (e) (void)hipEventDestroy(e);
    for (auto& e : b->ev_ar) if (e) (void)hipEventDestroy(e);
    b->ts_host.release();
    if (b->st) { (void)hipStreamSynchronize(b->st); chol_forget_stream(b->st); }
    if (b->own_stream && b->st) (void)hipStreamDestroy(b->st);
    delete b;
}

static LinArgs lin_args(stba_ba* b, int which, bool store_r) {
    LinArgs a;
    a.n_obs = b->no; a.n_cams = b->nc;
    a.cams = b->cams[which]; a.pts = b->pts[which];
    a.feat = b->feat; a.obs_cam = b->obs_cam; a.obs_pt = b->obs_pt;
    a.cam_fixed = b->cam_fixed; a.pt_fixed = b->pt_fixed;
    a.r = store_r ? b->r : nullptr; a.J8 = b->J8; a.cost_partial = b->cost_partial;
    return a;
}

static int ba_host_linearize(stba_ba* b, int which, bool with_jac) {
    const size_t no = (size_t)b->no;
    b->hl_cams.resize((size_t)b->nc * 7); b->hl_pts.resize((size_t)b->np * 3); b->hl_r.resize(no * 2);
    if (with_jac) { b->hl_jc.resize(no * 12); b->hl_jp.resize(no * 6); }
    STBA_TRY(download(b->hl_cams.data(), b->cams[which], b->hl_cams.size(), b->st));
    STBA_TRY(download(b->hl_pts.data(), b->pts[which], b->hl_pts.size(), b->st));
    STBA_HIP(hipStreamSynchronize(b->st));
    if (b->hl_fn(b->hl_user, b->hl_cams.data(), b->hl_pts.data(), b->hl_r.data(), with_jac ? b->hl_jc.data() : nullptr,
                 with_jac ? b->hl_jp.data() : nullptr) != 0)
        return fail(STBA_ERR_CALLBACK, "host lineariser failed (a cost function returned false)");
    double c2 = 0.0;
    for (size_t k = 0; k < no * 2; ++k) c2 += b->hl_r[k] * b->hl_r[k];
    if (!std::isfinite(c2)) return fail(STBA_ERR_CALLBACK, "host lineariser: non-finite residual");
    b->hl_cost_stage.assign((size_t)b->lin_grid, 0.0);
    b->hl_cost_stage[0] = c2;
    STBA_TRY(upload(b->cost_partial, b->hl_cost_stage.data(), b->hl_cost_stage.size(), b->st));
    STBA_HIP(hipStreamSynchronize(b->st));
    std::vector<double>& st = b->hl_stage;
    if (with_jac) {
        st.resize(no * 12);
        for (size_t p = 0; p < no; ++p) { const size_t i = (size_t)b->perm[p]; memcpy(&st[p * 2], &b->hl_r[i * 2], 2 * sizeof(double)); }
        STBA_TRY(upload(reinterpret_cast<double*>(b->r), st.data(), no * 2, b->st));
        STBA_HIP(hipStreamSynchronize(b->st));
        for (size_t p = 0; p < no; ++p) {
            const size_t i = (size_t)b->perm[p];
            st[p * 8] = 0.0; st[p * 8 + 1] = 0.0;
            memcpy(&st[p * 8 + 2], &b->hl_jp[i * 6], 6 * sizeof(double));
        }
        STBA_TRY(upload(b->J8, st.data(), no * 8, b->st));
        STBA_HIP(hipStreamSynchronize(b->st));
        for (size_t p = 0; p < no; ++p) memcpy(&st[p * 12], &b->hl_jc[(size_t)b->perm[p] * 12], 12 * sizeof(double));
        STBA_TRY(upload(b->Jc12, st.data(), no * 12, b->st));
        STBA_HIP(hipStreamSynchronize(b->st));
    }
    return STBA_OK;
}

static int ba_linearize(stba_ba* b, int which, double* cost2_dev) {
    if (b->hl_fn) STBA_TRY(ba_host_linearize(b, which, true));
    else STBA_TRY(launch_linearize(lin_args(b, which, true), true, b->lin_grid, b->st));
    return launch_sum_partials(b->cost_partial, b->lin_grid, 1, 1, cost2_dev, b->st);
}

static int ba_cost_only(stba_ba* b, int which, double* cost2_dev) {
    if (b->hl_fn) STBA_TRY(ba_host_linearize(b, which, false));
    else STBA_TRY(launch_linearize(lin_args(b, which, false), false, b->lin_grid, b->st));
    return launch_sum_partials(b->cost_partial, b->lin_grid, 1, 1, cost2_dev, b->st);
}

static int ba_normal_blocks(stba_ba* b) {
    return launch_point_blocks(b->np, b->pt_start, b->J8, b->omask, b->r, b->Hpp6, b->gp, b->upd_partial_p, b->st);
}
static int ba_linearize_lm(stba_ba* b, int which) {
    if (b->hl_fn) return ba_host_linearize(b, which, true);
    return launch_linearize(lin_args(b, which, true), true, b->lin_grid, b->st);
// ... 398 lines not shown
    stba_lm_summary s;
    memset(&s, 0, sizeof s);
    const double t_start = wall_s();
    const bool fixed = fixed_iterations > 0;
    const int max_iter = fixed ? fixed_iterations : opt.max_num_iterations;
    float ms = 0.f;
    hipEvent_t* ev = b->ev;
    const bool timing = opt.phase_timing != 0;
    b->ar_timing_on = timing;

    b->scale_init = false;
    b->ar_ms = 0.0; b->ar_bytes = 0.0; b->ar_calls = 0; b->ar_timing_pending = false;
    memset(&b->pcg_sum, 0, sizeof b->pcg_sum);
    b->pcg_per_iter.clear();
    Damping dm;
    dm.dmin = opt.min_lm_diagonal; dm.dmax = opt.max_lm_diagonal; dm.use_scaling = opt.jacobi_scaling;
    TrustRegion region(opt);
    double cost = 0.0, gmax = 0.0;
    bool inner_active = b->inner_on;
    if (b->inner_on) {
        inner_summary_reset(b);
        if (timing) for (auto& e : b->inner_ev) if (!e) STBA_HIP(hipEventCreate(&e));
    }

    if (timing) STBA_HIP(hipEventRecord(ev[0], b->st));
    STBA_TRY(ba_linearize_lm(b, b->cur));
    STBA_TRY(ba_normal_blocks(b));
    if (timing) STBA_HIP(hipEventRecord(ev[1], b->st));
    STBA_TRY(ba_fill_scalar_slots(b, b->trial + TS_COST2));
    bool need_build = true;
    bool lin_timing_pending = true;

    static const bool SPECULATE = knob_int("STBA_LM_SPECULATE", 1) != 0;
    const bool deferred_ok = (cb == nullptr) && !opt.minimizer_progress_to_stdout;
    bool pending = false, pending_accepted = false;
    int pending_iter = 0, pending_lin_ev = 8, spec_ev = 13;

    int iter = 0, chol_timeouts = 0, build_end_ev = 3;
    s.termination_type = STBA_NO_CONVERGENCE;
    s.termination_reason = STBA_TERM_MAX_ITER;
    bool first = true;
    double x_norm = 0.0;

    while (true) {
        if (!first) {
            if (iter >= max_iter) {
                s.termination_type = fixed ? STBA_CONVERGENCE : STBA_NO_CONVERGENCE;
                s.termination_reason = fixed ? STBA_TERM_FIXED : STBA_TERM_MAX_ITER;
                break;
            }
            if (!fixed && region.below_min(opt)) {
                s.termination_type = STBA_CONVERGENCE; s.termination_reason = STBA_TERM_MIN_RADIUS;
                break;
            }
        }
        dm.radius = region.radius;
        const bool built_here = need_build;
        if (need_build) {
            if (timing) STBA_HIP(hipEventRecord(ev[2], b->st));
            STBA_TRY(ba_build(b, dm));
            if (timing) STBA_HIP(hipEventRecord(ev[3], b->st));
            build_end_ev = 3;
        }
        const int solve_start_ev = build_end_ev;
        if (first) {
            STBA_TRY(ba_read_linear_scalars(b, &cost, &gmax));
            s.initial_cost = cost;
            trace_start(trace, cost, gmax, region.radius);
            first = false;
            if (opt.minimizer_progress_to_stdout) progress_start(cost, gmax, region.radius);
            if (!std::isfinite(cost)) {
                s.termination_type = STBA_FAILURE; s.termination_reason = STBA_TERM_SOLVER_FAIL;
                break;
            }
            if (!fixed && gmax <= opt.gradient_tolerance) {
                s.termination_type = STBA_CONVERGENCE; s.termination_reason = STBA_TERM_GRADIENT;
                break;
            }
            if (max_iter <= 0) break;
        }
        ++iter;
        int flag_h = 0, pcg_fail = 0;
        if (b->iterative) STBA_TRY(ba_pcg_solve(b, &pcg_fail));
        else if (b->stage_cooldown > 0) { --b->stage_cooldown; STBA_TRY(chol_factor_solve_stages(b->S(), b->lda, b->n, b->dxc, b->flag, b->st)); }
        else STBA_TRY(chol_factor_solve_dev(b->S(), b->lda, b->n, b->dxc, b->flag, b->st));
        if (timing) STBA_HIP(hipEventRecord(ev[4], b->st));
        STBA_TRY(ba_backsub_trial(b));
        if (timing) STBA_HIP(hipEventRecord(ev[5], b->st));
        const bool fast = deferred_ok && SPECULATE && !b->hl_fn && !b->iterative && !inner_active;
        if (fast && !b->ts_host.host) STBA_TRY(b->ts_host.alloc((size_t)stamped_doubles(TS_BLOCK)));
        const bool speculate = fast && !(fixed && iter >= max_iter);
        const double seq = fast ? (b->ts_seq += 1.0) : 0.0;
        STBA_TRY(ba_trial(b, fast ? b->ts_host.dev : nullptr, true, speculate, seq));
        if (timing) STBA_HIP(hipEventRecord(ev[6], b->st));
        double isc[2] = {0.0, 0.0};
        if (inner_active) {
            if (timing) STBA_HIP(hipEventRecord(b->inner_ev[0], b->st));
            STBA_TRY(ba_inner_after_trial(b));
            if (timing) STBA_HIP(hipEventRecord(b->inner_ev[1], b->st));
        }
        const double* ts = b->ts_vals;
        bool speculated = false;
        if (fast) {
            if (speculate) {
                spec_ev = (spec_ev == 8) ? 13 : 8;
                if (timing) STBA_HIP(hipEventRecord(ev[spec_ev], b->st));
                STBA_TRY(ba_normal_blocks(b));
                if (timing) STBA_HIP(hipEventRecord(ev[spec_ev + 1], b->st));
                STBA_TRY(ba_fill_scalar_slots(b, b->trial + TS_SPEC_COST2));
                speculated = true;
            }
            STBA_TRY(stamped_wait(b->ts_host.host, TS_BLOCK, [seq](double st) { return st == seq; }, b->ts_vals, hip_stream_state(b->st),
                                  "trial point", 120.0));
            flag_h = (int)ts[TS_SPEC_COST2];
        } else {
            STBA_TRY(download(b->ts_vals, b->trial, TS_BLOCK, b->st));
            STBA_TRY(download(&flag_h, b->flag, 1, b->st));
            if (inner_active) STBA_TRY(download(isc, b->inner_sc, 2, b->st));
            STBA_HIP(hipStreamSynchronize(b->st));
            if (inner_active && timing && hipEventElapsedTime(&ms, b->inner_ev[0], b->inner_ev[1]) == hipSuccess) b->inner_sum.sweep_ms += ms;
        }
        if (pcg_fail) flag_h = 1;
        if (pending) {
            const double c2 = 0.5 * ts[TS_LIN_COST2], g2 = ts[TS_LIN_GMAX];
            if (timing && hipEventElapsedTime(&ms, ev[pending_lin_ev], ev[pending_lin_ev + 1]) == hipSuccess) s.ms_linearize += ms;
            if (timing && hipEventElapsedTime(&ms, ev[10], ev[11]) == hipSuccess) s.ms_schur += ms;
            gmax = g2;
            if (pending_accepted) cost = c2;
            if (trace) trace[(size_t)pending_iter * STBA_TRACE_COLS + 2] = g2;
            pending = false;
            if (pending_accepted && !fixed && g2 <= opt.gradient_tolerance) {
                --iter;
                s.termination_type = STBA_CONVERGENCE; s.termination_reason = STBA_TERM_GRADIENT;
                break;
            }
        }
        if (b->iterative) ba_pcg_account(b, iter);
        if (flag_h == CHOL_FLAG_TIMEOUT || ts[TS_TIMEOUT] > 0.0) {
            if (b->ar) { b->stage_cooldown = 64; if (flag_h == CHOL_FLAG_TIMEOUT) chol_count_timeout(); }
            else chol_note_timeout();
            if (++chol_timeouts > 8) return fail(STBA_ERR_HIP, "dense Cholesky: the persistent program timed out repeatedly");
            if (speculated) {
                STBA_TRY(ba_linearize_lm(b, b->cur));
                STBA_TRY(ba_normal_blocks(b));
                STBA_TRY(ba_fill_scalar_slots(b, b->trial + TS_COST2));
            }
            need_build = true;
            --iter;
            continue;
        }
        if (timing) {
            if (lin_timing_pending) { (void)hipEventElapsedTime(&ms, ev[0], ev[1]); s.ms_linearize += ms; }
            if (built_here) { (void)hipEventElapsedTime(&ms, ev[2], ev[3]); s.ms_schur += ms; }
            (void)hipEventElapsedTime(&ms, ev[solve_start_ev], ev[4]); s.ms_solve += ms;
            (void)hipEventElapsedTime(&ms, ev[4], ev[5]); s.ms_backsub += ms;
            (void)hipEventElapsedTime(&ms, ev[5], ev[6]); s.ms_cost += ms;
        }
        lin_timing_pending = false;
        chol_timeouts = 0;

        bool step_ok = (flag_h == 0);
        double new_cost = 0.5 * ts[TS_COST2];
        double step_norm = std::sqrt(ts[TS_STEP2] + ts[TS_CAM + 0]);
        x_norm = std::sqrt(ts[TS_X2] + ts[TS_CAM + 1]);
        double model_change = ts[TS_MODEL] + ts[TS_CAM + 2];
        if (step_ok && (!(model_change > 0.0) || !std::isfinite(model_change) || !std::isfinite(new_cost)))
            step_ok = false;
        bool inner_useful = false;
// ... 28 lines not shown
        }
        need_build = true;
        if ((accepted || fixed) && !(fixed && iter >= max_iter)) {
            const int e0 = deferred_ok ? spec_ev : 0, e2 = deferred_ok ? 10 : 2;
            if (!(speculated && accepted)) {
                if (timing) STBA_HIP(hipEventRecord(ev[e0], b->st));
                STBA_TRY(ba_linearize_lm(b, b->cur));
                STBA_TRY(ba_normal_blocks(b));
                if (timing) STBA_HIP(hipEventRecord(ev[e0 + 1], b->st));
                STBA_TRY(ba_fill_scalar_slots(b, b->trial + TS_COST2));
            }
            dm.radius = region.radius;
            if (timing) STBA_HIP(hipEventRecord(ev[e2], b->st));
            STBA_TRY(ba_build(b, dm));
            if (timing) STBA_HIP(hipEventRecord(ev[e2 + 1], b->st));
            build_end_ev = e2 + 1;
            need_build = false;
            lin_timing_pending = false;
            if (deferred_ok) {
                pending = true; pending_accepted = accepted; pending_iter = iter;
                pending_lin_ev = spec_ev;
                if (accepted) cost = new_cost;
            } else {
                double c2, g2;
                STBA_TRY(ba_read_linear_scalars(b, &c2, &g2));
                if (timing) {
                    (void)hipEventElapsedTime(&ms, ev[0], ev[1]); s.ms_linearize += ms;
                    (void)hipEventElapsedTime(&ms, ev[2], ev[3]); s.ms_schur += ms;
                }
                gmax = g2;
                if (accepted) cost = c2;
            }
        }
        else if (speculated && !accepted) {
            STBA_TRY(ba_linearize_lm(b, b->cur));
            STBA_TRY(ba_normal_blocks(b));
            STBA_TRY(ba_fill_scalar_slots(b, b->trial + TS_COST2));
        }
        if (trace) { trace[(size_t)iter * STBA_TRACE_COLS + 2] = gmax; trace[(size_t)iter * STBA_TRACE_COLS + 5] = region.radius; }
        if (opt.minimizer_progress_to_stdout) progress_step(iter, cost, v, gmax, step_norm, region.radius);
        if (cb) {
            if (cb(cb_user, iter, cost, v.cost_change, gmax, step_norm, region.radius, accepted ? 1 : 0) != 0) {
                s.termination_type = STBA_CONVERGENCE; s.termination_reason = STBA_TERM_USER;
                break;
            }
        }
        if (!pending && accepted && !fixed && gmax <= opt.gradient_tolerance) {
            s.termination_type = STBA_CONVERGENCE; s.termination_reason = STBA_TERM_GRADIENT;
            break;
        }
    }
    STBA_HIP(hipStreamSynchronize(b->st));
    if (pending) {
        double c2, g2;
        STBA_TRY(ba_read_linear_scalars(b, &c2, &g2));
        gmax = g2;
        if (pending_accepted) cost = c2;
        if (trace) trace[(size_t)pending_iter * STBA_TRACE_COLS + 2] = g2;
        if (pending_accepted && !fixed && g2 <= opt.gradient_tolerance &&
            (s.termination_reason == STBA_TERM_MAX_ITER || s.termination_reason == STBA_TERM_MIN_RADIUS)) {
            s.termination_type = STBA_CONVERGENCE; s.termination_reason = STBA_TERM_GRADIENT;
        }
        pending = false;
    }
    ba_collect_allreduce_time(b);
    s.ms_allreduce = b->ar_ms; s.allreduce_bytes = b->ar_bytes; s.allreduce_calls = b->ar_calls;
    finish_summary(&s, iter, cost, region.radius, gmax, t_start);
    b->pcg_sum.linear_solve_ms = b->iterative ? s.ms_solve : 0.0;
    b->have_lin = b->have_blocks = b->have_reduced = b->have_dxc = b->have_dxp = false;
    if (sum) *sum = s;
    return STBA_OK;
}

static int ba_dogleg_alloc(stba_ba* b) {
    if (b->dl_sc) return STBA_OK;
    STBA_TRY(dev_alloc(&b->dl_uc, (size_t)std::max(b->n, 1)));
    STBA_TRY(dev_alloc(&b->dl_up, (size_t)std::max(b->np, 1) * 3));
    STBA_TRY(dev_alloc(&b->dl_part, dogleg_partial_doubles(b->nc, b->np)));
    STBA_TRY(dev_alloc(&b->dl_sc, 8));
    return b->dl_host.alloc((size_t)stamped_doubles(DL_BLOCK));
}

static int ba_dogleg_gauss_newton(stba_ba* b, const Damping& dm) {
    STBA_TRY(chol_factor_solve_dev(b->S(), b->lda, b->n, b->dxc, b->flag, b->st));
    STBA_TRY(launch_backsub(b->np, b->pt_start, b->obs_cam, b->J8, b->omask, b->Hinv6, b->gp, b->dxc, b->dxp, b->st, nullptr,
                            b->hl_fn ? b->Jc12 : nullptr));
    DoglegArgs a;
    a.n_cams = b->nc; a.n_pts = b->np;
    a.pt_start = b->pt_start; a.obs_cam = b->obs_cam; a.obs_pt = b->obs_pt;
    a.J8 = b->J8; a.omask = b->omask; a.Jc12 = b->hl_fn ? b->Jc12 : nullptr;
    a.cam_fixed = b->cam_fixed; a.pt_fixed = b->pt_fixed;
    a.hc = b->ex_diag(); a.gc = b->ex_gc(); a.scale_c = b->scale_c;
    a.Hpp6 = b->Hpp6; a.gp = b->gp; a.scale_p = b->scale_p;
    a.dmin = dm.dmin; a.dmax = dm.dmax;
    a.dxc = b->dxc; a.dxp = b->dxp; a.uc = b->dl_uc; a.up = b->dl_up;
    a.partial = b->dl_part; a.scalars = b->dl_sc;
    return launch_dogleg_terms(a, b->st);
}

static int ba_dogleg_step(stba_ba* b, double radius, double seq) {
    DoglegStepArgs a;
    a.n_cams = b->nc; a.n_pts = b->np;
    a.scalars = b->dl_sc; a.uc = b->dl_uc; a.up = b->dl_up; a.dxc = b->dxc; a.dxp = b->dxp;
    a.cams = b->cams[b->cur]; a.pts = b->pts[b->cur]; a.cam_fixed = b->cam_fixed; a.pt_fixed = b->pt_fixed;
    a.cams_new = b->cams[b->cur ^ 1]; a.pts_new = b->pts[b->cur ^ 1];
    a.partial_c = b->upd_partial_c; a.partial_p = b->upd_partial_p;
    a.host_out = b->dl_host.dev; a.seq = seq;
    return launch_dogleg_step(a, radius, b->st);
}

constexpr int kMaxConsecutiveInvalidSteps = 5;

static int ba_run_dogleg(stba_ba* b, const stba_lm_options* opt_in, stba_lm_summary* sum, double* trace, stba_iteration_callback cb,
                         void* cb_user) {
    stba_lm_options opt;
    if (opt_in) opt = *opt_in; else default_options(&opt);
    stba_lm_summary s;
    memset(&s, 0, sizeof s);
    const double t_start = wall_s();
    const int max_iter = opt.max_num_iterations;
    STBA_TRY(ba_dogleg_alloc(b));
    if (!b->ts_host.host) STBA_TRY(b->ts_host.alloc((size_t)stamped_doubles(TS_BLOCK)));
    b->scale_init = false;
    b->ar_ms = 0.0; b->ar_bytes = 0.0; b->ar_calls = 0; b->ar_timing_pending = false; b->ar_timing_on = false;
    memset(&b->pcg_sum, 0, sizeof b->pcg_sum);
    b->pcg_per_iter.clear();
    stba_dogleg_summary ds{};
    ds.struct_size = sizeof ds;
    Damping dm;
    dm.dmin = opt.min_lm_diagonal; dm.dmax = opt.max_lm_diagonal; dm.use_scaling = opt.jacobi_scaling;
    DoglegRegion region(opt);
    double cost = 0.0, gmax = 0.0;

    STBA_TRY(ba_linearize_lm(b, b->cur));
    STBA_TRY(ba_normal_blocks(b));
    STBA_TRY(ba_fill_scalar_slots(b, b->trial + TS_COST2));
    const bool deferred_ok = (cb == nullptr) && !opt.minimizer_progress_to_stdout;
    bool need_build = true, need_gn = true, first = true, pending = false, pending_accepted = false;
    int pending_iter = 0, iter = 0, chol_timeouts = 0, invalid_in_a_row = 0;
    s.termination_type = STBA_NO_CONVERGENCE;
    s.termination_reason = STBA_TERM_MAX_ITER;
    double hd[DL_BLOCK] = {0.0};

    while (true) {
        if (!first) {
            if (iter >= max_iter) break;
            if (region.below_min(opt)) { s.termination_type = STBA_CONVERGENCE; s.termination_reason = STBA_TERM_MIN_RADIUS; break; }
        }
        if (need_build) {
            dm.radius = 1.0 / region.mu;
            STBA_TRY(ba_build(b, dm));
            need_build = false;
        }
        if (first) {
            STBA_TRY(ba_read_linear_scalars(b, &cost, &gmax));
            s.initial_cost = cost;
            trace_start(trace, cost, gmax, region.radius);
            first = false;
            if (opt.minimizer_progress_to_stdout) progress_start(cost, gmax, region.radius);
            if (!std::isfinite(cost)) { s.termination_type = STBA_FAILURE; s.termination_reason = STBA_TERM_SOLVER_FAIL; break; }
            if (gmax <= opt.gradient_tolerance) { s.termination_type = STBA_CONVERGENCE; s.termination_reason = STBA_TERM_GRADIENT; break; }
            if (max_iter <= 0) break;
        }
        ++iter;
        bool have_gn = true, reused = !need_gn;
        if (need_gn) {
            if (region.can_factor()) {
// ... 516 lines not shown
                            }
                            if (rot_by_rank) for (size_t x = x0; x < x1; ++x) rank_of[(size_t)(pair_rec[x].w & 0x3fff)] = 0;
                        }
                    }
                }
            }
        });
        for (int v : max_slots_thr) max_slots = std::max(max_slots, v);
    }
    b->max_cols = std::max(task_max_cols, max_slots);
    {
        double at = 0.0;
        size_t n_diag = 0;
        for (size_t v : diag_pairs_thr) n_diag += v;
        at = 36.0 * (double)(n_pair_rec - n_diag) + 21.0 * (double)n_diag;
        b->schur_pairs = (double)n_pair_rec; b->schur_lds_atomics = at;
    }
    std::vector<long long> task_part_off;
    std::vector<int> row_task_ptr, row_tasks;
    size_t part_doubles = 0;
    if (b->lm_slices) {
        const int ntask = (int)task_cam.size();
        task_part_off.resize((size_t)ntask);
        for (int k = 0; k < ntask; ++k) {
            task_part_off[(size_t)k] = (long long)part_doubles;
            part_doubles += (size_t)(task_col_hi[(size_t)k] - task_col_lo[(size_t)k]) * 36 + 64;
        }
        std::vector<std::vector<std::pair<int, int>>> by_row((size_t)n_cams);
        for (int k = 0; k < ntask; ++k) by_row[(size_t)task_cam[(size_t)k]].push_back({task_p_lo[(size_t)k], k});
        row_task_ptr.assign((size_t)n_cams + 1, 0);
        for (int c = 0; c < n_cams; ++c) {
            std::sort(by_row[(size_t)c].begin(), by_row[(size_t)c].end());
            for (auto& pr : by_row[(size_t)c]) row_tasks.push_back(pr.second);
            row_task_ptr[(size_t)c + 1] = (int)row_tasks.size();
        }
    }
    tmark("pair plan");
    std::vector<unsigned char> cmask;
    if (cam_fixed) {
        cmask.resize(n_cams);
        for (int c = 0; c < n_cams; ++c) {
            unsigned m = 0;
            for (int a = 0; a < 6; ++a) if (cam_fixed[c * 6 + a]) m |= (1u << a);
            cmask[c] = (unsigned char)m;
        }
    }
    const int n_tiles = (n_obs + LIN_THREADS - 1) / LIN_THREADS;
    const size_t lds = lin_lds_bytes(n_cams, lin_lds_bytes(n_cams, true, true) <= (size_t)LIN_MAX_LDS, true);
    const int per_cu = std::max(1, std::min(4, (int)((160 * 1024) / std::max<size_t>(lds, 1))));
    b->lin_grid = std::max(1, std::min(n_tiles, num_cu * per_cu));

    tmark("masks");
#define A_(call) do { rc = (call); if (rc != STBA_OK) return bail(rc); } while (0)
    const size_t no = (size_t)n_obs, np = (size_t)n_pts, nc = (size_t)n_cams;
    for (int k = 0; k < 2; ++k) { A_(dev_alloc(&b->cams[k], nc * 7)); A_(dev_alloc(&b->pts[k], np * 3)); }
    A_(dev_alloc(&b->feat, no)); A_(dev_alloc(&b->obs_cam, no)); A_(dev_alloc(&b->obs_pt, no));
    A_(dev_alloc(&b->pt_start, np + 1)); A_(dev_alloc(&b->cam_perm, no));
    A_(dev_alloc(&b->chunk_begin, (size_t)b->n_chunks)); A_(dev_alloc(&b->chunk_end, (size_t)b->n_chunks));
    A_(dev_alloc(&b->cam_chunk_start, nc + 1));
    A_(dev_alloc(&b->task_cam, std::max<size_t>(task_cam.size(), 1))); A_(dev_alloc(&b->cam_start, nc + 1));
    A_(dev_alloc(&b->task_col_lo, std::max<size_t>(task_cam.size(), 1))); A_(dev_alloc(&b->task_col_hi, std::max<size_t>(task_cam.size(), 1)));
    A_(dev_alloc(&b->row_col_ptr, nc + 1)); A_(dev_alloc(&b->row_cols, std::max<size_t>(row_cols.size(), 1)));
    A_(dev_alloc(&b->pair_begin, std::max<size_t>(pair_begin.size(), 1))); A_(dev_alloc(&b->pair_end, std::max<size_t>(pair_end.size(), 1)));
    A_(dev_alloc(&b->pair_rec, std::max<size_t>(n_pair_rec, 1)));
    A_(dev_alloc(&b->task_vs_ptr, std::max<size_t>(task_vs_ptr.size(), 1))); A_(dev_alloc(&b->vs_first, std::max<size_t>(vs_first.size(), 1)));
    if (cam_fixed) A_(dev_alloc(&b->cam_fixed, nc));
    if (pt_fixed) A_(dev_alloc(&b->pt_fixed, np));
    if (b->lm_slices) {
        A_(dev_alloc(&b->task_p_lo, task_p_lo.size())); A_(dev_alloc(&b->task_p_hi, task_p_hi.size())); A_(dev_alloc(&b->task_part_off, task_part_off.size()));
        A_(dev_alloc(&b->row_task_ptr, row_task_ptr.size())); A_(dev_alloc(&b->row_tasks, std::max<size_t>(row_tasks.size(), 1)));
        A_(dev_alloc(&b->schur_part, std::max<size_t>(part_doubles, 1)));
        A_(upload(b->task_p_lo, task_p_lo.data(), task_p_lo.size(), b->st)); A_(upload(b->task_p_hi, task_p_hi.data(), task_p_hi.size(), b->st));
        A_(upload(b->task_part_off, task_part_off.data(), task_part_off.size(), b->st));
        A_(upload(b->row_task_ptr, row_task_ptr.data(), row_task_ptr.size(), b->st)); A_(upload(b->row_tasks, row_tasks.data(), row_tasks.size(), b->st));
    }
    if (!dup_run.empty()) { A_(dev_alloc(&b->dup_run, no)); A_(upload(b->dup_run, dup_run.data(), no, b->st)); }
    A_(dev_alloc(&b->r, no)); A_(dev_alloc(&b->J8, no * 8));
    if (cam_fixed || pt_fixed) A_(dev_alloc(&b->omask, no));
    A_(dev_alloc(&b->Hpp6, np * 6)); A_(dev_alloc(&b->gp, np * 3)); A_(dev_alloc(&b->Hinv6, np * 6));
    A_(dev_alloc(&b->dp, np * 3)); A_(dev_alloc(&b->scale_p, np * 3));
    A_(dev_alloc(&b->Hcc, nc * 36)); A_(dev_alloc(&b->gc, nc * 6)); A_(dev_alloc(&b->cam_partial, (size_t)b->n_chunks * 28));
    A_(dev_alloc(&b->dc, nc * 6)); A_(dev_alloc(&b->scale_c, nc * 6));
    A_(dev_alloc(&b->Sbuf, b->sbuf_count()));
    A_(dev_alloc(&b->dxc, (size_t)b->lda)); A_(dev_alloc(&b->dxp, np * 3));
    A_(dev_alloc(&b->cost_partial, (size_t)b->lin_grid));
    A_(dev_alloc(&b->upd_partial_c, (size_t)backsub_cam_grid(n_cams) * 4));
    A_(dev_alloc(&b->upd_partial_p, (size_t)(point_blocks_grid(n_pts) + 1) * 4));
    A_(dev_alloc(&b->trial, (size_t)TS_BLOCK)); A_(dev_alloc(&b->flag, 1));
    if (iterative) A_(ba_pcg_alloc(b));

    tmark("device allocations");
    A_(upload(b->cams[0], cams, nc * 7, b->st)); A_(upload(b->pts[0], pts, np * 3, b->st));
    A_(upload(reinterpret_cast<double*>(b->feat), s_feat.data(), no * 2, b->st));
    A_(upload(b->obs_cam, s_cam.data(), no, b->st)); A_(upload(b->obs_pt, s_pt.data(), no, b->st));
    A_(upload(b->pt_start, pt_start.data(), np + 1, b->st)); A_(upload(b->cam_perm, cam_perm.data(), no, b->st));
    A_(upload(b->chunk_begin, chunk_begin.data(), (size_t)b->n_chunks, b->st));
    A_(upload(b->chunk_end, chunk_end.data(), (size_t)b->n_chunks, b->st));
    A_(upload(b->cam_chunk_start, cam_chunk_start.data(), nc + 1, b->st));
    A_(upload(b->task_cam, task_cam.data(), task_cam.size(), b->st));
    A_(upload(b->cam_start, cam_start.data(), nc + 1, b->st));
    A_(upload(b->task_col_lo, task_col_lo.data(), task_cam.size(), b->st));
    A_(upload(b->task_col_hi, task_col_hi.data(), task_cam.size(), b->st));
    b->h_row_col_ptr = row_col_ptr; b->h_row_cols = row_cols;
    A_(upload(b->row_col_ptr, row_col_ptr.data(), nc + 1, b->st));
    if (!row_cols.empty()) A_(upload(b->row_cols, row_cols.data(), row_cols.size(), b->st));
    A_(upload(b->pair_begin, pair_begin.data(), pair_begin.size(), b->st)); A_(upload(b->pair_end, pair_end.data(), pair_end.size(), b->st));
    if (n_pair_rec > 0) A_(upload(b->pair_rec, pair_rec.get(), n_pair_rec, b->st));
    A_(upload(b->task_vs_ptr, task_vs_ptr.data(), task_vs_ptr.size(), b->st)); A_(upload(b->vs_first, vs_first.data(), vs_first.size(), b->st));
    if (cam_fixed) A_(upload(b->cam_fixed, cmask.data(), nc, b->st));
    std::vector<unsigned char> omask;
    if (b->omask) {
        omask.resize(no);
        for (size_t p2 = 0; p2 < no; ++p2)
            omask[p2] = (unsigned char)((cam_fixed ? cmask[(size_t)s_cam[p2]] : 0u) | ((pt_fixed && pt_fixed[(size_t)s_pt[p2]]) ? 64u : 0u));
        A_(upload(b->omask, omask.data(), no, b->st));
    }
    if (pt_fixed) A_(upload(b->pt_fixed, pt_fixed, np, b->st));
    if (hipMemsetAsync(b->dxc, 0, (size_t)b->lda * sizeof(double), b->st) != hipSuccess ||
        hipMemsetAsync(b->Sbuf, 0, b->sbuf_count() * sizeof(double), b->st) != hipSuccess ||
        hipStreamSynchronize(b->st) != hipSuccess)
        return bail(fail(STBA_ERR_HIP, "stba_ba_create: initial memset/sync failed"));
#undef A_
    tmark("uploads + sync");
    {
        struct Garbage {
            std::unique_ptr<int4[]> pair_rec;
            std::vector<int> a, b2, c, d, e, f;
            std::vector<double> g;
            std::vector<unsigned char> h, i;
            std::vector<std::vector<int>> j;
        };
        Garbage* gb = new (std::nothrow) Garbage{std::move(pair_rec), std::move(s_cam), std::move(s_pt), std::move(cam_perm), std::move(pt_start),
                                                 std::move(vs_first), std::move(row_cols), std::move(s_feat), std::move(dup_run), std::move(omask),
                                                 std::move(cnt_of)};
        if (gb) b->create_leftovers = std::shared_ptr<void>(gb, [](void* q) { delete static_cast<Garbage*>(q); });
    }
    *out = b;
    return STBA_OK;
}

int stba_ba_create(stba_ba** out, int n_cams, int n_pts, int n_obs, const double* cams, const double* pts,
                   const int* obs_cam, const int* obs_pt, const double* obs_feat, const unsigned char* cam_fixed,
                   const unsigned char* pt_fixed, void* hip_stream) {
    return ba_create(out, n_cams, n_pts, n_obs, cams, pts, obs_cam, obs_pt, obs_feat, cam_fixed, pt_fixed, hip_stream, false);
}

int stba_ba_create_ex(stba_ba** out, int n_cams, int n_pts, int n_obs, const double* cams, const double* pts,
                      const int* obs_cam, const int* obs_pt, const double* obs_feat, const unsigned char* cam_fixed,
                      const unsigned char* pt_fixed, void* hip_stream, const stba_ba_create_options* opt) {
    if (out) *out = nullptr;
    int solver = STBA_LINEAR_DENSE_SCHUR;
    if (opt) {
        if (opt->struct_size < offsetof(stba_ba_create_options, linear_solver) + sizeof(int))
            return fail(STBA_ERR_INVALID_ARGUMENT, "stba_ba_create_ex: options.struct_size is smaller than any version of the struct");
        solver = opt->linear_solver;
    }
    if (solver != STBA_LINEAR_DENSE_SCHUR && solver != STBA_LINEAR_ITERATIVE_SCHUR)
        return fail(STBA_ERR_INVALID_ARGUMENT, "stba_ba_create_ex: unknown linear_solver " + std::to_string(solver));
    return ba_create(out, n_cams, n_pts, n_obs, cams, pts, obs_cam, obs_pt, obs_feat, cam_fixed, pt_fixed, hip_stream,
                     solver == STBA_LINEAR_ITERATIVE_SCHUR);
}

static int refuse_iterative(const stba_ba* b, const char* who, const char* why) {
    if (!b || !b->iterative) return STBA_OK;
    return fail(STBA_ERR_INVALID_ARGUMENT, std::string(who) + ": this engine uses ITERATIVE_SCHUR, " + why);
}

int stba_ba_set_pcg(stba_ba* b, int preconditioner, double eta, int min_iterations, int max_iterations, int check_every) {
    if (!b) return fail(STBA_ERR_INVALID_ARGUMENT, "null engine");
    if (!b->iterative) return fail(STBA_ERR_INVALID_ARGUMENT, "stba_ba_set_pcg: the engine uses the dense Schur solver (stba_ba_create_ex)");
    if (preconditioner < STBA_PRECOND_IDENTITY || preconditioner > STBA_PRECOND_SCHUR_JACOBI || !(eta >= 0.0) || min_iterations < 0 ||
        max_iterations < 1 || min_iterations > max_iterations || check_every < 1)
        return fail(STBA_ERR_INVALID_ARGUMENT, "stba_ba_set_pcg: bad argument");
    b->pcg_precond = preconditioner; b->pcg_eta = eta; b->pcg_min = min_iterations; b->pcg_max = max_iterations; b->pcg_check = check_every;
    return STBA_OK;
}

int stba_ba_last_pcg_summary(stba_ba* b, stba_pcg_summary* out) {
    if (!b || !out) return fail(STBA_ERR_INVALID_ARGUMENT, "null argument");
    *out = b->pcg_sum;
    return STBA_OK;
}

int stba_ba_last_pcg_iterations(stba_ba* b, int* per_iteration, int n) {
    if (!b || n < 0 || (n > 0 && !per_iteration)) return fail(STBA_ERR_INVALID_ARGUMENT, "stba_ba_last_pcg_iterations: bad argument");
    for (int k = 0; k < n; ++k) per_iteration[k] = (size_t)k < b->pcg_per_iter.size() ? b->pcg_per_iter[(size_t)k] : 0;
    return STBA_OK;
}

int stba_ba_time_schur_apply(stba_ba* b, int reps, double* ms_avg) {
    if (!b || reps <= 0 || !ms_avg) return fail(STBA_ERR_INVALID_ARGUMENT, "stba_ba_time_schur_apply: bad argument");
    if (!b->iterative) return fail(STBA_ERR_INVALID_ARGUMENT, "stba_ba_time_schur_apply: the engine uses the dense Schur solver");
    if (!b->have_blocks) return fail(STBA_ERR_STATE, "stba_ba_time_schur_apply needs stba_ba_schur_apply first");
    const PcgVecs v = pcg_vecs(b);
    STBA_HIP(hipEventRecord(b->ev[0], b->st));
    for (int k = 0; k < reps; ++k) {
        STBA_TRY(ba_is_landmark_pass(b, v.p, nullptr, nullptr));
        STBA_TRY(ba_is_camera_pass(b, IS_FINAL_APPLY, v.p, v.q, nullptr, nullptr));
    }
    STBA_HIP(hipEventRecord(b->ev[1], b->st));
    STBA_HIP(hipStreamSynchronize(b->st));
    float ms = 0.f;
    STBA_HIP(hipEventElapsedTime(&ms, b->ev[0], b->ev[1]));
    *ms_avg = (double)ms / reps;
    return STBA_OK;
}

int stba_ba_schur_apply(stba_ba* b, const double* dc, const double* dp, int which, const double* x, double* y) {
    if (!b || !dc || !dp || !y || which < 0 || which > 2) return fail(STBA_ERR_INVALID_ARGUMENT, "stba_ba_schur_apply: bad argument");
    if (!b->iterative) return fail(STBA_ERR_INVALID_ARGUMENT, "stba_ba_schur_apply: the engine uses the dense Schur solver (stba_ba_reduced_system)");
    if (!b->have_blocks) return fail(STBA_ERR_STATE, "stba_ba_schur_apply needs stba_ba_normal_blocks first");
    STBA_TRY(upload(b->dc, dc, (size_t)b->n, b->st));
    STBA_TRY(upload(b->dp, dp, (size_t)b->np * 3, b->st));
    Damping dm;
    dm.explicit_d = true;
    STBA_TRY(launch_point_invert(b->np, b->Hpp6, b->dp, b->pt_fixed, b->Hinv6, b->st));
    STBA_TRY(ba_camera_blocks(b));
    double* out_dev = b->rhs();
    if (!x) STBA_TRY(ba_is_rhs(b));
    else {
        const PcgVecs v = pcg_vecs(b);
        STBA_TRY(upload(which == 0 ? v.p : v.r, x, (size_t)b->n, b->st));
        if (which == 0) {
            STBA_TRY(ba_is_landmark_pass(b, v.p, nullptr, nullptr));
            STBA_TRY(ba_is_camera_pass(b, IS_FINAL_APPLY, v.p, v.q, nullptr, nullptr));
            out_dev = v.q;
        } else {
            STBA_TRY(ba_is_precond(b, which == 1 ? STBA_PRECOND_JACOBI : STBA_PRECOND_SCHUR_JACOBI));
            STBA_TRY(launch_is_vec(b->nc, IS_VEC_PRECOND, v, b->st));
            out_dev = v.z;
        }
    }
    STBA_TRY(download(y, out_dev, (size_t)b->n, b->st));
    STBA_HIP(hipStreamSynchronize(b->st));
    b->have_reduced = b->have_dxc = b->have_dxp = false;
    return STBA_OK;
}

int stba_ba_set_schur_mode(stba_ba* ba, int mode) {
    STBA_TRY(refuse_iterative(ba, "stba_ba_set_schur_mode", "which forms no Schur complement"));
    if (!ba || mode < STBA_SCHUR_AUTO || mode > STBA_SCHUR_DENSE) return fail(STBA_ERR_INVALID_ARGUMENT, "stba_ba_set_schur_mode: bad argument");
    if (mode == STBA_SCHUR_AUTO) mode = ba->schur_mode_auto;
    if (mode == STBA_SCHUR_PAIRS && !ba->have_pair_plan)
        return fail(STBA_ERR_INVALID_ARGUMENT, "stba_ba_set_schur_mode: this engine was created without a pair plan (too many observation pairs)");
    if (mode == STBA_SCHUR_DENSE && ba->dup_overflow)
        return fail(STBA_ERR_INVALID_ARGUMENT, "stba_ba_set_schur_mode: more than 255 observations of one (camera, landmark) pair: the dense form cannot take this problem");
    if (mode == STBA_SCHUR_DENSE) STBA_TRY(ba_dense_alloc(ba));
    ba->schur_mode = mode;
    ba->have_reduced = ba->have_dxc = ba->have_dxp = false;
    return STBA_OK;
}
int stba_ba_schur_mode(const stba_ba* ba, int* mode) {
    if (!ba || !mode) return fail(STBA_ERR_INVALID_ARGUMENT, "stba_ba_schur_mode: bad argument");
    *mode = ba->schur_mode;
    return STBA_OK;
}

int stba_ba_destroy(stba_ba* ba) {
    if (!ba) return STBA_OK;
    if (ba->st) (void)hipStreamSynchronize(ba->st);
    ba_free(ba);
    return STBA_OK;
}

int stba_ba_set_params(stba_ba* b, const double* cams, const double* pts) {
    if (!b) return fail(STBA_ERR_INVALID_ARGUMENT, "null engine");
    if (cams) STBA_TRY(upload(b->cams[b->cur], cams, (size_t)b->nc * 7, b->st));
    if (pts) STBA_TRY(upload(b->pts[b->cur], pts, (size_t)b->np * 3, b->st));
    STBA_HIP(hipStreamSynchronize(b->st));
    b->have_lin = b->have_blocks = b->have_reduced = b->have_dxc = b->have_dxp = false;
    return STBA_OK;
}

int stba_ba_set_features(stba_ba* b, const double* obs_feat) {
    if (!b || (!obs_feat && b->no > 0)) return fail(STBA_ERR_INVALID_ARGUMENT, "stba_ba_set_features: null argument");
    if (b->no == 0) return STBA_OK;
    std::vector<double> s_feat((size_t)b->no * 2);
    for (int p = 0; p < b->no; ++p) {
        const size_t i = (size_t)b->perm[(size_t)p];
        s_feat[2 * (size_t)p] = obs_feat[2 * i]; s_feat[2 * (size_t)p + 1] = obs_feat[2 * i + 1];
    }
    STBA_TRY(upload(reinterpret_cast<double*>(b->feat), s_feat.data(), (size_t)b->no * 2, b->st));
    STBA_HIP(hipStreamSynchronize(b->st));
    b->have_lin = b->have_blocks = b->have_reduced = b->have_dxc = b->have_dxp = false;
    return STBA_OK;
}

int stba_get_device(int* device) {
    if (!device) return fail(STBA_ERR_INVALID_ARGUMENT, "stba_get_device: null argument");
    STBA_TRY(require_device());
    STBA_HIP(hipGetDevice(device));
    return STBA_OK;
}
int stba_set_device(int device) {
    STBA_TRY(require_device());
    STBA_HIP(hipSetDevice(device));
    return STBA_OK;
}

int stba_ba_get_params(stba_ba* b, double* cams, double* pts) {
    if (!b) return fail(STBA_ERR_INVALID_ARGUMENT, "null engine");
    if (cams) STBA_TRY(download(cams, b->cams[b->cur], (size_t)b->nc * 7, b->st));
    if (pts) STBA_TRY(download(pts, b->pts[b->cur], (size_t)b->np * 3, b->st));
    STBA_HIP(hipStreamSynchronize(b->st));
    return STBA_OK;
}

int stba_ba_set_host_linearizer(stba_ba* b, stba_ba_linearize_fn fn, void* user) {
    if (!b) return fail(STBA_ERR_INVALID_ARGUMENT, "null engine");
    if (fn && b->inner_on) return fail(STBA_ERR_INVALID_ARGUMENT, "stba_ba_set_host_linearizer: this engine has inner iterations (device residuals only)");
    if (fn && !b->Jc12) STBA_TRY(dev_alloc(&b->Jc12, (size_t)b->no * 12));
    b->hl_fn = fn; b->hl_user = user;
    b->have_lin = b->have_blocks = b->have_reduced = b->have_dxc = b->have_dxp = false;
    return STBA_OK;
}

int stba_ba_set_allreduce(stba_ba* b, stba_allreduce_fn fn, void* user, int rank, int world_size) {
    STBA_TRY(refuse_iterative(b, "stba_ba_set_allreduce", "which runs on one rank only"));
    if (b && b->trust_region == STBA_TR_TRADITIONAL_DOGLEG)
        return fail(STBA_ERR_INVALID_ARGUMENT, "stba_ba_set_allreduce: this engine uses DOGLEG, which runs on one rank only");
    if (b && b->inner_on && (fn || world_size > 1))
        return fail(STBA_ERR_INVALID_ARGUMENT, "stba_ba_set_allreduce: this engine has inner iterations, which run on one rank only");
    if (!b || world_size < 1 || rank < 0 || rank >= world_size || world_size > SC_MAX_WORLD)
        return fail(STBA_ERR_INVALID_ARGUMENT, "stba_ba_set_allreduce: bad rank/world");
    if (!fn && world_size > 1) return fail(STBA_ERR_INVALID_ARGUMENT, "stba_ba_set_allreduce: world_size > 1 needs a hook");
    b->ar = fn; b->ar_user = user; b->rank = rank; b->world = world_size;
    b->pk_state = 0; b->pk_nz = 0;
    if (b->pk_blocks) { (void)hipFree(b->pk_blocks); b->pk_blocks = nullptr; }
    if (b->Spack) { (void)hipFree(b->Spack); b->Spack = nullptr; }
    return STBA_OK;
// ... 11 lines not shown
    STBA_TRY(ba_linearize(b, b->cur, b->trial + TS_COST2));
    double c2 = 0.0;
    STBA_TRY(download(&c2, b->trial + TS_COST2, 1, b->st));
    const size_t no = (size_t)b->no;
    std::vector<double> tr, tjc, tjp;
    if (r) { tr.resize(no * 2); STBA_TRY(download(tr.data(), reinterpret_cast<double*>(b->r), no * 2, b->st)); }
    double *djc = nullptr, *djp = nullptr;
    struct TmpGuard { double*& a; double*& c; ~TmpGuard() { if (a) (void)hipFree(a); if (c) (void)hipFree(c); } } tmp_guard{djc, djp};
    if ((Jc || Jp) && b->hl_fn) return fail(STBA_ERR_STATE, "stba_ba_evaluate: with a host lineariser the Jacobians are the caller's own");
    if (Jc || Jp) {
        if (Jc) STBA_TRY(dev_alloc(&djc, no * 12));
        if (Jp) STBA_TRY(dev_alloc(&djp, no * 6));
        STBA_TRY(launch_expand_jacobian(b->no, b->J8, b->omask, djc, djp, b->st));
        if (Jc) { tjc.resize(no * 12); STBA_TRY(download(tjc.data(), djc, no * 12, b->st)); }
        if (Jp) { tjp.resize(no * 6); STBA_TRY(download(tjp.data(), djp, no * 6, b->st)); }
    }
    STBA_HIP(hipStreamSynchronize(b->st));
    for (size_t p = 0; p < no; ++p) {
        const size_t i = (size_t)b->perm[p];
        if (r) memcpy(r + i * 2, tr.data() + p * 2, 2 * sizeof(double));
        if (Jc) memcpy(Jc + i * 12, tjc.data() + p * 12, 12 * sizeof(double));
        if (Jp) memcpy(Jp + i * 6, tjp.data() + p * 6, 6 * sizeof(double));
    }
    if (cost) *cost = 0.5 * c2;
    b->have_lin = true;
    b->have_blocks = b->have_reduced = b->have_dxc = b->have_dxp = false;
    return STBA_OK;
}

int stba_ba_cost(stba_ba* b, double* cost) {
    if (!b || !cost) return fail(STBA_ERR_INVALID_ARGUMENT, "null argument");
    STBA_TRY(ba_cost_only(b, b->cur, b->trial + TS_COST2));
    double c2 = 0.0;
    STBA_TRY(download(&c2, b->trial + TS_COST2, 1, b->st));
    STBA_HIP(hipStreamSynchronize(b->st));
    *cost = 0.5 * c2;
    return STBA_OK;
}

int stba_ba_normal_blocks(stba_ba* b, double* Hcc, double* gc, double* Hpp, double* gp) {
    if (!b) return fail(STBA_ERR_INVALID_ARGUMENT, "null engine");
    if (!b->have_lin) return fail(STBA_ERR_STATE, "stba_ba_normal_blocks needs stba_ba_evaluate first");
    STBA_TRY(ba_normal_blocks(b));
    STBA_TRY(ba_camera_blocks(b));
    std::vector<double> h6;
    if (Hcc) STBA_TRY(download(Hcc, b->Hcc, (size_t)b->nc * 36, b->st));
    if (gc) STBA_TRY(download(gc, b->gc, (size_t)b->nc * 6, b->st));
    if (Hpp) { h6.resize((size_t)b->np * 6); STBA_TRY(download(h6.data(), b->Hpp6, h6.size(), b->st)); }
    if (gp) STBA_TRY(download(gp, b->gp, (size_t)b->np * 3, b->st));
    STBA_HIP(hipStreamSynchronize(b->st));
    if (Hpp)
        for (size_t j = 0; j < (size_t)b->np; ++j) {
            const double* s = h6.data() + j * 6;
            double* d = Hpp + j * 9;
            d[0] = s[0]; d[1] = s[1]; d[2] = s[2]; d[3] = s[1]; d[4] = s[3]; d[5] = s[4]; d[6] = s[2]; d[7] = s[4]; d[8] = s[5];
        }
    b->have_blocks = true;
    return STBA_OK;
}

int stba_ba_reduced_system(stba_ba* b, const double* dc, const double* dp, double* S, double* rhs) {
    STBA_TRY(refuse_iterative(b, "stba_ba_reduced_system", "which never forms the reduced system (stba_ba_schur_apply applies it)"));
    if (!b || !dc || !dp) return fail(STBA_ERR_INVALID_ARGUMENT, "null argument");
    if (!b->have_blocks) return fail(STBA_ERR_STATE, "stba_ba_reduced_system needs stba_ba_normal_blocks first");
    STBA_TRY(upload(b->dc, dc, (size_t)b->n, b->st));
    STBA_TRY(upload(b->dp, dp, (size_t)b->np * 3, b->st));
    Damping dm;
    dm.explicit_d = true;
    STBA_HIP(hipMemsetAsync(b->ex_scalar(), 0, (size_t)b->lda * sizeof(double), b->st));
    STBA_TRY(ba_build_reduced(b, dm));
    if (S) STBA_HIP(hipMemcpy2DAsync(S, (size_t)b->n * sizeof(double), b->S(), (size_t)b->lda * sizeof(double),
                                     (size_t)b->n * sizeof(double), (size_t)b->n, hipMemcpyDeviceToHost, b->st));
    if (rhs) STBA_TRY(download(rhs, b->rhs(), (size_t)b->n, b->st));
    STBA_HIP(hipStreamSynchronize(b->st));
    b->have_reduced = true;
    b->have_dxc = b->have_dxp = false;
    return STBA_OK;
}

int stba_ba_solve_reduced(stba_ba* b, double* dxc) {
    STBA_TRY(refuse_iterative(b, "stba_ba_solve_reduced", "which has no reduced system to factor"));
    if (!b) return fail(STBA_ERR_INVALID_ARGUMENT, "null engine");
    if (!b->have_reduced) return fail(STBA_ERR_STATE, "stba_ba_solve_reduced needs stba_ba_reduced_system first");
    STBA_TRY(chol_factor_solve_dev(b->S(), b->lda, b->n, b->dxc, b->flag, b->st));
    int flag_h = 0;
    STBA_TRY(download(&flag_h, b->flag, 1, b->st));
    if (dxc) STBA_TRY(download(dxc, b->dxc, (size_t)b->n, b->st));
    STBA_HIP(hipStreamSynchronize(b->st));
    b->have_reduced = false;
    if (flag_h == CHOL_FLAG_TIMEOUT && !b->ar && b->have_blocks) {
        chol_note_timeout();
        Damping dm;
        dm.explicit_d = true;
        STBA_HIP(hipMemsetAsync(b->ex_scalar(), 0, (size_t)b->lda * sizeof(double), b->st));
        STBA_TRY(ba_build_reduced(b, dm));
        STBA_TRY(chol_factor_solve_stages(b->S(), b->lda, b->n, b->dxc, b->flag, b->st));
        STBA_TRY(download(&flag_h, b->flag, 1, b->st));
        if (dxc) STBA_TRY(download(dxc, b->dxc, (size_t)b->n, b->st));
        STBA_HIP(hipStreamSynchronize(b->st));
    }
    STBA_TRY(chol_flag_status(flag_h));
    if (flag_h != 0) return fail(STBA_ERR_NOT_POSITIVE_DEFINITE, "reduced camera system: pivot " + std::to_string(flag_h));
    b->have_dxc = true;
    return STBA_OK;
}

int stba_ba_back_substitute(stba_ba* b, double* dxp) {
    if (!b) return fail(STBA_ERR_INVALID_ARGUMENT, "null engine");
    if (!b->have_dxc) return fail(STBA_ERR_STATE, "stba_ba_back_substitute needs stba_ba_solve_reduced first");
    STBA_TRY(launch_backsub(b->np, b->pt_start, b->obs_cam, b->J8, b->omask, b->Hinv6, b->gp, b->dxc, b->dxp, b->st, nullptr, b->hl_fn ? b->Jc12 : nullptr));
    if (dxp) STBA_TRY(download(dxp, b->dxp, (size_t)b->np * 3, b->st));
    STBA_HIP(hipStreamSynchronize(b->st));
    b->have_dxp = true;
    return STBA_OK;
}

int stba_ba_apply_step(stba_ba* b, int accept, double* new_cost) {
    if (!b) return fail(STBA_ERR_INVALID_ARGUMENT, "null engine");
    if (!b->have_dxp) return fail(STBA_ERR_STATE, "stba_ba_apply_step needs stba_ba_back_substitute first");
    STBA_TRY(ba_trial(b, nullptr));
    double ts[TS_COUNT];
    STBA_TRY(download(ts, b->trial, TS_COUNT, b->st));
    STBA_HIP(hipStreamSynchronize(b->st));
    if (new_cost) *new_cost = 0.5 * ts[TS_COST2];
    if (accept) {
        b->cur ^= 1;
        b->have_lin = b->have_blocks = b->have_reduced = b->have_dxc = b->have_dxp = false;
    }
    return STBA_OK;
}

int stba_ba_solve(stba_ba* b, const stba_lm_options* opt, stba_lm_summary* summary, double* trace,
                  stba_iteration_callback cb, void* cb_user) {
    if (!b) return fail(STBA_ERR_INVALID_ARGUMENT, "null engine");
    b->dl_sum = stba_dogleg_summary{};
    if (b->trust_region == STBA_TR_TRADITIONAL_DOGLEG) {
        if (b->inner_on) return fail(STBA_ERR_INVALID_ARGUMENT, "stba_ba_solve: inner iterations are not supported with DOGLEG");
        return ba_run_dogleg(b, opt, summary, trace, cb, cb_user);
    }
    return ba_run_lm(b, opt, 0, summary, trace, cb, cb_user);
}

int stba_ba_set_trust_region(stba_ba* b, int strategy) {
    if (!b) return fail(STBA_ERR_INVALID_ARGUMENT, "null engine");
    if (strategy != STBA_TR_LEVENBERG_MARQUARDT && strategy != STBA_TR_TRADITIONAL_DOGLEG)
        return fail(STBA_ERR_INVALID_ARGUMENT, "stba_ba_set_trust_region: unknown strategy " + std::to_string(strategy));
    if (strategy == STBA_TR_TRADITIONAL_DOGLEG) {
        if (b->iterative)
            return fail(STBA_ERR_INVALID_ARGUMENT, "stba_ba_set_trust_region: DOGLEG only supports exact factorization based linear solvers "
                        "(this engine uses ITERATIVE_SCHUR)");
        if (b->ar) return fail(STBA_ERR_INVALID_ARGUMENT, "stba_ba_set_trust_region: DOGLEG runs on one rank only (an all-reduce hook is set)");
    }
    b->trust_region = strategy;
    return STBA_OK;
}

int stba_ba_last_dogleg_summary(stba_ba* b, stba_dogleg_summary* out) {
    if (!b || !out) return fail(STBA_ERR_INVALID_ARGUMENT, "null argument");
    const size_t want = out->struct_size;
    if (want < offsetof(stba_dogleg_summary, factorizations) + sizeof(int))
        return fail(STBA_ERR_INVALID_ARGUMENT, "stba_ba_last_dogleg_summary: out->struct_size is smaller than any version of the struct");
    stba_dogleg_summary s = b->dl_sum;
    s.struct_size = want;
    memcpy(out, &s, std::min(want, sizeof s));
    return STBA_OK;
}

int stba_ba_set_inner_iterations(stba_ba* b, int enable, double tolerance, const int* cam_rot_group, const int* cam_pos_group,
                                 const int* pt_group) {
    if (!b) return fail(STBA_ERR_INVALID_ARGUMENT, "null engine");
    if (!enable) {
        b->inner_on = false;
        return STBA_OK;
    }
    if (!(tolerance >= 0.0) || !std::isfinite(tolerance))
        return fail(STBA_ERR_INVALID_ARGUMENT, "stba_ba_set_inner_iterations: the tolerance must be finite and >= 0");
    if (b->ar) return fail(STBA_ERR_INVALID_ARGUMENT, "stba_ba_set_inner_iterations: inner iterations run on one rank only (an all-reduce hook is set)");
    if (b->hl_fn) return fail(STBA_ERR_INVALID_ARGUMENT, "stba_ba_set_inner_iterations: not with a host lineariser");
    const int nc = b->nc, np = b->np, no = b->no;
// ... 740 lines not shown
```

Before: 370.0.

## Factor Schur complement into separate buffer so S stays pristine and needs no zeroing

The dense Cholesky now reads the Schur matrix S on the first touch of each tile and writes its factor into a separate buffer Afac. Tasks whose first-block tiles are flagged read from S0, and the staged path copies S into Afac up front. S is therefore never overwritten, so the Schur build kernel no longer zeroes S's rows each iteration. This removes a per-iteration zero-fill of the dense matrix, at the cost of an extra n×n buffer and a full device copy on the staged fallback path.

```diff
diff --git a/slam-tricks_amd/csrc/ba_kernels.hip b/slam-tricks_amd/csrc/ba_kernels.hip
--- a/slam-tricks_amd/csrc/ba_kernels.hip
+++ b/slam-tricks_amd/csrc/ba_kernels.hip
@@ -557,15 +557,6 @@
     for (int e = tid; e <= ncols; e += SCHUR_THREADS) vsf[e] = vs_g[e];
     if (tid == 0) vsf[a.max_cols + 1] = 0;
     const bool lms = a.part != nullptr;
-    if (!lms) {
-        const int cend = min(a.lda, ((c * 6 + 5) / 128 + 1) * 128);
-        const int z0 = (clo == 0) ? 0 : 6 * a.row_cols[col0];
-        const int z1 = diag_piece ? cend : 6 * a.row_cols[col0 + ncols];
-        for (int q = 0; q < 6; ++q) {
-            double* row = a.S + (size_t)(c * 6 + q) * a.lda;
-            for (int e = z0 + tid; e < z1; e += SCHUR_THREADS) row[e] = 0.0;
-        }
-    }
     __syncthreads();
     const int wv = tid >> 6;
     constexpr int mode = MODE;
diff --git a/slam-tricks_amd/csrc/common.hpp b/slam-tricks_amd/csrc/common.hpp
--- a/slam-tricks_amd/csrc/common.hpp
+++ b/slam-tricks_amd/csrc/common.hpp
@@ -189,8 +189,8 @@
 inline int chol_flag_status(int flag_h) {
     return flag_h == CHOL_FLAG_TIMEOUT ? fail(STBA_ERR_HIP, "dense Cholesky: the persistent program timed out waiting for a dependency and the caller has no way to rebuild the matrix") : STBA_OK;
 }
-int chol_factor_solve_dev(double* A_dev, int lda, int n, double* x_dev, int* flag_dev, hipStream_t st);
-int chol_factor_solve_stages(double* A_dev, int lda, int n, double* x_dev, int* flag_dev, hipStream_t st);
+int chol_factor_solve_dev(double* A_dev, int lda, int n, double* x_dev, int* flag_dev, hipStream_t st, const double* S0 = nullptr);
+int chol_factor_solve_stages(double* A_dev, int lda, int n, double* x_dev, int* flag_dev, hipStream_t st, const double* S0 = nullptr);
 void chol_forget_stream(hipStream_t st);
 void chol_note_timeout();
 void chol_note_peer_timeout();
diff --git a/slam-tricks_amd/csrc/dense_chol.hip b/slam-tricks_amd/csrc/dense_chol.hip
--- a/slam-tricks_amd/csrc/dense_chol.hip
+++ b/slam-tricks_amd/csrc/dense_chol.hip
@@ -346,12 +346,12 @@
 }
 
 template <bool WT>
-__device__ __forceinline__ void diag_block2(double* __restrict__ A, int lda, int k0, int n_real,
+__device__ __forceinline__ void diag_block2(double* __restrict__ A, const double* __restrict__ Asrc, int lda, int k0, int n_real,
                                             int* __restrict__ flag, double* __restrict__ dinv, double* smem, int t,
                                             long long* ph = nullptr) {
     Diag2Smem& sm = *reinterpret_cast<Diag2Smem*>(smem);
     const int w = __builtin_amdgcn_readfirstlane(t >> 6), lane = t & 63;
-    const double* Ab = A + (size_t)k0 * lda + k0;
+    const double* Ab = Asrc + (size_t)k0 * lda + k0;
     PHASE_STAMP(0);
     d2_stage_block(Ab, lda, sm, t);
     D2_BARRIER();
@@ -364,7 +364,7 @@
 __global__ __launch_bounds__(512) void chol_diag_kernel(double* __restrict__ A, int lda, int k0, int n_real,
                                                          int* __restrict__ flag, double* __restrict__ dinv) {
     extern __shared__ __attribute__((aligned(16))) double sm2[];
-    diag_block2<false>(A, lda, k0, n_real, flag, dinv, sm2, threadIdx.x);
+    diag_block2<false>(A, A, lda, k0, n_real, flag, dinv, sm2, threadIdx.x);
 }
 
 template <bool WT>
@@ -550,6 +550,7 @@
 constexpr int MEGA_MAX_Q = 16;
 struct MegaArgs {
     double* A; int lda; int n; int nblk;
+    const double* S0;
     const int4* tasks;
     int nq;
     int lstart[MEGA_MAX_Q + 1];
@@ -561,6 +562,7 @@
     int* flag;
     long long* trace;
 };
+constexpr int MEGA_FIRST = 0x100;
 constexpr int MEGA_SYNC_HDR = MEGA_MAX_Q + 1;
 constexpr int MEGA_ABORT = MEGA_MAX_Q;
 constexpr int MEGA_SMEM_BYTES = 128 * 1024;
@@ -576,7 +578,7 @@
 }
 
 template <int TM, int KCH = 16>
-__device__ __forceinline__ void syrk_tile512(double* __restrict__ A, int lda, int k0, int row_i, int row_j,
+__device__ __forceinline__ void syrk_tile512(double* __restrict__ A, const double* __restrict__ Csrc, int lda, int k0, int row_i, int row_j,
                                              double* smem, int t, int kchunks = NB / 16) {
     constexpr int WR = (TM == 128) ? 2 : 1, WC = 8 / WR;
     constexpr int MB = TM / (16 * WR);
@@ -596,7 +598,7 @@
             for (int r = 0; r < 4; ++r) {
                 const int row = row_i + wr * (MB * 16) + m * 16 + (lane >> 4) + 4 * r;
                 const int col = row_j + wc * (NBK * 16) + n * 16 + (lane & 15);
-                acc[m][n][r] = A[(size_t)row * lda + col];
+                acc[m][n][r] = Csrc[(size_t)row * lda + col];
             }
     double2 ga[NH], gb[NH];
     const int lrow = lane & 15, lkp = lane >> 4;
@@ -832,13 +834,13 @@
     return true;
 }
 
-__device__ __forceinline__ bool trsm_task512(double* __restrict__ rowp, bool ident, int ident_row0, int nv,
+__device__ __forceinline__ bool trsm_task512(double* __restrict__ rowp, const double* __restrict__ rowsrc, bool ident, int ident_row0, int nv,
                                              const double* __restrict__ Lb, int lda,
                                              const double* __restrict__ dinv, double* smem, int t, long long* ph,
                                              const int* dflag, int* abortf, int* s_ok, long long spin_limit, bool flag_known = false,
                                              bool active = true) {
     double4v W[8];
-    if (!trsm_compute512(W, rowp, ident, ident_row0, nv, Lb, lda, dinv, smem, t, ph, dflag, abortf, s_ok, spin_limit, flag_known, active)) return false;
+    if (!trsm_compute512(W, rowsrc, ident, ident_row0, nv, Lb, lda, dinv, smem, t, ph, dflag, abortf, s_ok, spin_limit, flag_known, active)) return false;
     const int g = (t & 63) >> 4;
     if (active) {
 #pragma unroll
@@ -848,13 +850,15 @@
     return true;
 }
 
-__device__ __forceinline__ bool tu4_task512(double* __restrict__ A, int lda, int k0, int rb, int q,
+__device__ __forceinline__ bool tu4_task512(double* __restrict__ A, const double* __restrict__ Asrc, int lda, int k0, int rb, int q,
                                            const double* __restrict__ dinv, double* smem, int t, long long* ph,
                                            int* loaded, int* ver_diag, const int* dflag, int* abortf, int* s_ok, long long spin_limit,
                                            bool flag_known = false) {
     const int lane = t & 63, w = t >> 6;
     const int n = lane & 15, g = lane >> 4;
     double* rowp = A + (size_t)(rb * NB + 16 * w + n) * lda + k0;
+    const double* rowsrc = Asrc + (size_t)(rb * NB + 16 * w + n) * lda + k0;
+    const double* Cs = Asrc + (size_t)(rb * NB) * lda + rb * NB;
     const int ntile = 4 * q + 3;
     double* Cb = A + (size_t)(rb * NB) * lda + rb * NB;
     double4v acc[2];
@@ -866,11 +870,11 @@
         tn[s2] = (e < 2 * q + 1) ? e : e - (2 * q + 1);
         if (e < ntile) {
 #pragma unroll
-            for (int r = 0; r < 4; ++r) acc[s2][r] = Cb[(size_t)(16 * tm[s2] + g + 4 * r) * lda + 16 * tn[s2] + n];
+            for (int r = 0; r < 4; ++r) acc[s2][r] = Cs[(size_t)(16 * tm[s2] + g + 4 * r) * lda + 16 * tn[s2] + n];
         }
     }
     double4v W[8];
-    if (!trsm_compute512(W, rowp, false, 0, NB, A + (size_t)k0 * lda + k0, lda, dinv, smem, t, ph, dflag, abortf, s_ok, spin_limit, flag_known)) return false;
+    if (!trsm_compute512(W, rowsrc, false, 0, NB, A + (size_t)k0 * lda + k0, lda, dinv, smem, t, ph, dflag, abortf, s_ok, spin_limit, flag_known)) return false;
     __syncthreads();
     if (t == 0) __hip_atomic_fetch_add(loaded, 1, __ATOMIC_RELAXED, __HIP_MEMORY_SCOPE_AGENT);
 #pragma unroll
@@ -908,7 +912,7 @@
 }
 
 constexpr int MEGA_NTU = 10;
-__device__ __forceinline__ bool tu_task512(double* __restrict__ A, int lda, int k0, int rb, int q,
+__device__ __forceinline__ bool tu_task512(double* __restrict__ A, const double* __restrict__ Asrc, int lda, int k0, int rb, int q,
                                            const double* __restrict__ dinv, double* smem, int t, long long* ph,
                                            int* loaded, int* done_cnt, int* ver_diag, const int* dflag, int* abortf, int* s_ok, long long spin_limit,
                                            bool flag_known = false) {
@@ -922,6 +926,8 @@
     const bool active = w < nrow;
     const int trow = (w < 2) ? 2 * I + (w & 1) : 2 * J + (w & 1);
     double* rowp = A + (size_t)(rb * NB + 16 * trow + n) * lda + k0;
+    const double* rowsrc = Asrc + (size_t)(rb * NB + 16 * trow + n) * lda + k0;
+    const double* Cs = Asrc + (size_t)(rb * NB) * lda + rb * NB;
     const int ntile = diag ? 3 : 4;
     const int lm = diag ? (w >= 1 ? 1 : 0) : (w >> 1), ln = diag ? (w == 2 ? 1 : 0) : 2 + (w & 1);
     const int tm = 2 * I + lm, tn = diag ? 2 * I + ln : 2 * J + (w & 1);
@@ -929,10 +935,10 @@
     double4v acc = {0.0, 0.0, 0.0, 0.0};
     if (w < ntile) {
 #pragma unroll
-        for (int r = 0; r < 4; ++r) acc[r] = Cb[(size_t)(16 * tm + g + 4 * r) * lda + 16 * tn + n];
+        for (int r = 0; r < 4; ++r) acc[r] = Cs[(size_t)(16 * tm + g + 4 * r) * lda + 16 * tn + n];
     }
     double4v W[8];
-    if (!trsm_compute512(W, rowp, false, 0, NB, A + (size_t)k0 * lda + k0, lda, dinv, smem, t, ph, dflag, abortf, s_ok, spin_limit, flag_known, active)) return false;
+    if (!trsm_compute512(W, rowsrc, false, 0, NB, A + (size_t)k0 * lda + k0, lda, dinv, smem, t, ph, dflag, abortf, s_ok, spin_limit, flag_known, active)) return false;
     __syncthreads();
     if (t == 0) __hip_atomic_fetch_add(loaded, 1, __ATOMIC_RELAXED, __HIP_MEMORY_SCOPE_AGENT);
     if (active) {
@@ -968,7 +974,7 @@
     return true;
 }
 
-__device__ __forceinline__ void syrk_q32(double* __restrict__ A, int lda, int k0, int row_i, int row_j, int t, long long* ph) {
+__device__ __forceinline__ void syrk_q32(double* __restrict__ A, const double* __restrict__ Csrc, int lda, int k0, int row_i, int row_j, int t, long long* ph) {
     const int lane = t & 63, w = t >> 6;
     const int n = lane & 15, g = lane >> 4;
     const double* pa0 = A + (size_t)(row_i + n) * lda + k0 + 4 * g;
@@ -980,7 +986,7 @@
 #pragma unroll
     for (int m = 0; m < 2; ++m)
 #pragma unroll
-        for (int r = 0; r < 4; ++r) acc[m][r] = A[(size_t)(row_i + 16 * m + g + 4 * r) * lda + row_j + 16 * w + n];
+        for (int r = 0; r < 4; ++r) acc[m][r] = Csrc[(size_t)(row_i + 16 * m + g + 4 * r) * lda + row_j + 16 * w + n];
     PHASE_STAMP(0);
 #pragma unroll
     for (int c = 0; c < 8; ++c)
@@ -1133,15 +1139,17 @@
         asm volatile("" : "+v"(tt));
         double* li = a.linv + (size_t)b * a.linv_stride;
         long long* ph = a.trace ? a.trace + 8 * (size_t)task + 4 : nullptr;
+        const double* As = (d.x & MEGA_FIRST) ? a.S0 : a.A;
         if (type == TASK_D) {
-            diag_block2<true>(a.A, a.lda, k0, a.n, a.flag, li + NB * NB, smem, tt, ph);
+            diag_block2<true>(a.A, As, a.lda, k0, a.n, a.flag, li + NB * NB, smem, tt, ph);
         } else if (type == TASK_T) {
             const int lane = tt & 63, w = tt >> 6;
             int ldr;
             const bool active = (tj == 0) || (w < 4);
             const int row_in_tile = (tj == 0 ? 16 * w : 64 * (tj - 1) + 16 * (w & 3)) + (lane & 15);
             double* rowp = tile_ptr(ti, b, ldr) + (size_t)row_in_tile * ldr;
-            if (!trsm_task512(rowp, false, 0, NB, a.A + (size_t)k0 * a.lda + k0, a.lda, li + NB * NB, smem, tt, ph, &dflag[b], abortf, &s_ok,
+            const double* rowsrc = (d.x & MEGA_FIRST) ? a.S0 + ((size_t)ti * NB + row_in_tile) * a.lda + (size_t)b * NB : rowp;
+            if (!trsm_task512(rowp, rowsrc, false, 0, NB, a.A + (size_t)k0 * a.lda + k0, a.lda, li + NB * NB, smem, tt, ph, &dflag[b], abortf, &s_ok,
                               a.spin_limit, true, active)) {
                 if (t == 0) atomicExch(a.flag, CHOL_FLAG_TIMEOUT);
                 break;
@@ -1153,7 +1161,7 @@
             double* base = li;
             if (b < 4 * a.nwide) base = tile_ptr(nblk + b, b, ldr);
             double* rowp = base + (size_t)(16 * w + (lane & 15)) * ldr;
-            if (!trsm_task512(rowp, true, 16 * w, nv, a.A + (size_t)k0 * a.lda + k0, a.lda, li + NB * NB, smem, tt, ph, &dflag[b], abortf, &s_ok,
+            if (!trsm_task512(rowp, rowp, true, 16 * w, nv, a.A + (size_t)k0 * a.lda + k0, a.lda, li + NB * NB, smem, tt, ph, &dflag[b], abortf, &s_ok,
                               a.spin_limit, true)) {
                 if (t == 0) atomicExch(a.flag, CHOL_FLAG_TIMEOUT);
                 break;
@@ -1161,7 +1169,7 @@
         } else if (type == TASK_U) {
             if (ti < nblk) {
                 const int nbp = max(1, (d.x >> 16) & 0xff);
-                syrk_tile512<128>(a.A, a.lda, k0 - (nbp - 1) * NB, ti * NB, tj * NB, smem, tt, nbp * (NB / 16));
+                syrk_tile512<128>(a.A, As, a.lda, k0 - (nbp - 1) * NB, ti * NB, tj * NB, smem, tt, nbp * (NB / 16));
             } else {
                 int ldc, ldi, ldj;
                 double* Cb = tile_ptr(ti, tj, ldc);
@@ -1171,16 +1179,16 @@
             }
         } else if (type == TASK_TU) {
             const bool tu_ok = (tj == 2)
-                ? tu4_task512(a.A, a.lda, k0, b + 1, ti, li + NB * NB, smem, tt, ph, &tuflag[b], &ver[(b + 1) * nblk + b + 1], &dflag[b], abortf, &s_ok,
+                ? tu4_task512(a.A, As, a.lda, k0, b + 1, ti, li + NB * NB, smem, tt, ph, &tuflag[b], &ver[(b + 1) * nblk + b + 1], &dflag[b], abortf, &s_ok,
                               a.spin_limit, s_dset != 0)
-                : tu_task512(a.A, a.lda, k0, b + 1, ti, li + NB * NB, smem, tt, ph, &tuflag[b], &v.tudone[b], &ver[(b + 1) * nblk + b + 1], &dflag[b], abortf, &s_ok,
+                : tu_task512(a.A, As, a.lda, k0, b + 1, ti, li + NB * NB, smem, tt, ph, &tuflag[b], &v.tudone[b], &ver[(b + 1) * nblk + b + 1], &dflag[b], abortf, &s_ok,
                              a.spin_limit, s_dset != 0);
             if (!tu_ok) {
                 if (t == 0) atomicExch(a.flag, CHOL_FLAG_TIMEOUT);
                 break;
             }
         } else {
-            syrk_q32(a.A, a.lda, k0, (ti >> 2) * NB + (ti & 3) * 32, tj * NB, tt, ph);
+            syrk_q32(a.A, As, a.lda, k0, (ti >> 2) * NB + (ti & 3) * 32, tj * NB, tt, ph);
         }
         asm volatile("s_waitcnt vmcnt(0)" ::: "memory");
         __syncthreads();
@@ -1495,7 +1503,11 @@
         });
         lstart[l] = (int)out.size();
         for (const Pick& pk : order[(size_t)l]) {
-            out.push_back(nodes[(size_t)pk.node].tk);
+            int4 tk = nodes[(size_t)pk.node].tk;
+            const int ty = tk.x & 0xff, nbp = std::max(1, (tk.x >> 16) & 0xff);
+            const int row = ty == TASK_UQ ? (tk.z >> 2) : (ty == TASK_T || ty == TASK_U) ? tk.z : 0;
+            if (ty != TASK_TI && row < NBK && tk.y - nbp + 1 == 0) tk.x |= MEGA_FIRST;
+            out.push_back(tk);
             if (sim_start) sim_start->push_back((float)pk.start);
         }
     }
@@ -1722,7 +1734,7 @@
 enum { CHOL_PERSISTENT = 0, CHOL_STAGES = 1 };
 
 static int chol_run(double* A, int lda, int n, double* x_dev, int* flag_dev, hipStream_t st, CholProfile* prof,
-                    hipEvent_t mid_event = nullptr, int schedule = CHOL_PERSISTENT, hipEvent_t pre_event = nullptr) {
+                    hipEvent_t mid_event = nullptr, int schedule = CHOL_PERSISTENT, hipEvent_t pre_event = nullptr, const double* S0 = nullptr) {
     if (lda % NB != 0 || lda < n + 1) return fail(STBA_ERR_INVALID_ARGUMENT, "chol: bad padded dimension");
     const int nblk = lda / NB;
     int cur_dev = 0;
@@ -1792,6 +1804,7 @@
             D.last_stream = st;
         }
         STBA_HIP(hipMemsetAsync(flag_dev, 0, sizeof(int), st));
+        if (S0 && S0 != A) STBA_HIP(hipMemcpyAsync(A, S0, (size_t)lda * lda * sizeof(double), hipMemcpyDeviceToDevice, st));
         for (int b = 0; b < nblk; ++b) {
             const int k0 = b * NB;
             const int mt = nblk - b - 1;
@@ -1833,6 +1846,7 @@
         hipLaunchKernelGGL(chol_reset_kernel, dim3((unsigned)((plan.sync_ints + 255) / 256)), dim3(256), 0, st, plan.sync, (int)plan.sync_ints, flag_dev);
         MegaArgs ma;
         ma.A = A; ma.lda = lda; ma.n = n; ma.nblk = nblk;
+        ma.S0 = S0 ? S0 : A;
         ma.tasks = plan.tasks; ma.nq = D.nq; ma.sync = plan.sync;
         memcpy(ma.lstart, plan.lstart, sizeof ma.lstart);
         memcpy(ma.xcc_queue, D.xcc_queue, sizeof ma.xcc_queue);
@@ -2010,12 +2024,12 @@
     return STBA_OK;
 }
 
-int chol_factor_solve_dev(double* A, int lda, int n, double* x_dev, int* flag_dev, hipStream_t st) {
-    return chol_run(A, lda, n, x_dev, flag_dev, st, nullptr);
-}
-
-int chol_factor_solve_stages(double* A, int lda, int n, double* x_dev, int* flag_dev, hipStream_t st) {
-    return chol_run(A, lda, n, x_dev, flag_dev, st, nullptr, nullptr, CHOL_STAGES);
+int chol_factor_solve_dev(double* A, int lda, int n, double* x_dev, int* flag_dev, hipStream_t st, const double* S0) {
+    return chol_run(A, lda, n, x_dev, flag_dev, st, nullptr, nullptr, CHOL_PERSISTENT, nullptr, S0);
+}
+
+int chol_factor_solve_stages(double* A, int lda, int n, double* x_dev, int* flag_dev, hipStream_t st, const double* S0) {
+    return chol_run(A, lda, n, x_dev, flag_dev, st, nullptr, nullptr, CHOL_STAGES, nullptr, S0);
 }
 
 int chol_factor_solve_split(double* A, int lda, int n, double* x_dev, int* flag_dev, hipStream_t st, hipEvent_t mid_event, hipEvent_t pre_event) {
diff --git a/slam-tricks_amd/csrc/stba_engine.hip b/slam-tricks_amd/csrc/stba_engine.hip
--- a/slam-tricks_amd/csrc/stba_engine.hip
+++ b/slam-tricks_amd/csrc/stba_engine.hip
@@ -99,6 +99,7 @@
     double *Hpp6 = nullptr, *gp = nullptr, *Hinv6 = nullptr, *dp = nullptr, *scale_p = nullptr;
     double *Hcc = nullptr, *gc = nullptr, *cam_partial = nullptr, *dc = nullptr, *scale_c = nullptr;
     double* Sbuf = nullptr;
+    double* Afac = nullptr;
     double *dxc = nullptr, *dxp = nullptr;
     double *cost_partial = nullptr, *upd_partial_c = nullptr, *upd_partial_p = nullptr;
     double* trial = nullptr;
@@ -170,7 +171,7 @@
     F(b->cams[0]); F(b->cams[1]); F(b->pts[0]); F(b->pts[1]); F(b->feat); F(b->obs_cam); F(b->obs_pt);
     F(b->pt_start); F(b->cam_perm); F(b->chunk_begin); F(b->chunk_end); F(b->cam_chunk_start); F(b->cam_fixed);
     F(b->pt_fixed); F(b->r); F(b->J8); F(b->Jc12); F(b->omask); F(b->Hpp6); F(b->gp); F(b->Hinv6); F(b->dp); F(b->scale_p);
-    F(b->Hcc); F(b->gc); F(b->cam_partial); F(b->dc); F(b->scale_c); F(b->Sbuf); F(b->Spack); F(b->pk_blocks); F(b->dxc); F(b->dxp);
+    F(b->Hcc); F(b->gc); F(b->cam_partial); F(b->dc); F(b->scale_c); F(b->Sbuf); F(b->Afac); F(b->Spack); F(b->pk_blocks); F(b->dxc); F(b->dxp);
     F(b->task_cam); F(b->cam_start); F(b->task_col_lo); F(b->task_col_hi); F(b->row_col_ptr); F(b->row_cols);
     F(b->task_p_lo); F(b->task_p_hi); F(b->row_task_ptr); F(b->row_tasks); F(b->task_part_off); F(b->schur_part);
     F(b->pair_begin); F(b->pair_end); F(b->pair_rec); F(b->task_vs_ptr); F(b->vs_first); F(b->Y); F(b->yv); F(b->yws); F(b->dup_run);
@@ -735,8 +736,8 @@
         ++iter;
         int flag_h = 0, pcg_fail = 0;
         if (b->iterative) STBA_TRY(ba_pcg_solve(b, &pcg_fail));
-        else if (b->stage_cooldown > 0) { --b->stage_cooldown; STBA_TRY(chol_factor_solve_stages(b->S(), b->lda, b->n, b->dxc, b->flag, b->st)); }
-        else STBA_TRY(chol_factor_solve_dev(b->S(), b->lda, b->n, b->dxc, b->flag, b->st));
+        else if (b->stage_cooldown > 0) { --b->stage_cooldown; STBA_TRY(chol_factor_solve_stages(b->Afac, b->lda, b->n, b->dxc, b->flag, b->st, b->S())); }
+        else STBA_TRY(chol_factor_solve_dev(b->Afac, b->lda, b->n, b->dxc, b->flag, b->st, b->S()));
         if (timing) STBA_HIP(hipEventRecord(ev[4], b->st));
         STBA_TRY(ba_backsub_trial(b));
         if (timing) STBA_HIP(hipEventRecord(ev[5], b->st));
@@ -931,7 +932,7 @@
 }
 
 static int ba_dogleg_gauss_newton(stba_ba* b, const Damping& dm) {
-    STBA_TRY(chol_factor_solve_dev(b->S(), b->lda, b->n, b->dxc, b->flag, b->st));
+    STBA_TRY(chol_factor_solve_dev(b->Afac, b->lda, b->n, b->dxc, b->flag, b->st, b->S()));
     STBA_TRY(launch_backsub(b->np, b->pt_start, b->obs_cam, b->J8, b->omask, b->Hinv6, b->gp, b->dxc, b->dxp, b->st, nullptr,
                             b->hl_fn ? b->Jc12 : nullptr));
     DoglegArgs a;
@@ -1614,6 +1615,7 @@
     A_(dev_alloc(&b->Hcc, nc * 36)); A_(dev_alloc(&b->gc, nc * 6)); A_(dev_alloc(&b->cam_partial, (size_t)b->n_chunks * 28));
     A_(dev_alloc(&b->dc, nc * 6)); A_(dev_alloc(&b->scale_c, nc * 6));
     A_(dev_alloc(&b->Sbuf, b->sbuf_count()));
+    if (!iterative) A_(dev_alloc(&b->Afac, b->s_count()));
     A_(dev_alloc(&b->dxc, (size_t)b->lda)); A_(dev_alloc(&b->dxp, np * 3));
     A_(dev_alloc(&b->cost_partial, (size_t)b->lin_grid));
     A_(dev_alloc(&b->upd_partial_c, (size_t)backsub_cam_grid(n_cams) * 4));
@@ -1778,6 +1780,7 @@
     if (mode == STBA_SCHUR_DENSE && ba->dup_overflow)
         return fail(STBA_ERR_INVALID_ARGUMENT, "stba_ba_set_schur_mode: more than 255 observations of one (camera, landmark) pair: the dense form cannot take this problem");
     if (mode == STBA_SCHUR_DENSE) STBA_TRY(ba_dense_alloc(ba));
+    if (mode != ba->schur_mode) STBA_HIP(hipMemsetAsync(ba->S(), 0, ba->s_count() * sizeof(double), ba->st));
     ba->schur_mode = mode;
     ba->have_reduced = ba->have_dxc = ba->have_dxp = false;
     return STBA_OK;
@@ -1955,7 +1958,7 @@
     STBA_TRY(refuse_iterative(b, "stba_ba_solve_reduced", "which has no reduced system to factor"));
     if (!b) return fail(STBA_ERR_INVALID_ARGUMENT, "null engine");
     if (!b->have_reduced) return fail(STBA_ERR_STATE, "stba_ba_solve_reduced needs stba_ba_reduced_system first");
-    STBA_TRY(chol_factor_solve_dev(b->S(), b->lda, b->n, b->dxc, b->flag, b->st));
+    STBA_TRY(chol_factor_solve_dev(b->Afac, b->lda, b->n, b->dxc, b->flag, b->st, b->S()));
     int flag_h = 0;
     STBA_TRY(download(&flag_h, b->flag, 1, b->st));
     if (dxc) STBA_TRY(download(dxc, b->dxc, (size_t)b->n, b->st));
@@ -1967,7 +1970,7 @@
         dm.explicit_d = true;
         STBA_HIP(hipMemsetAsync(b->ex_scalar(), 0, (size_t)b->lda * sizeof(double), b->st));
         STBA_TRY(ba_build_reduced(b, dm));
-        STBA_TRY(chol_factor_solve_stages(b->S(), b->lda, b->n, b->dxc, b->flag, b->st));
+        STBA_TRY(chol_factor_solve_stages(b->Afac, b->lda, b->n, b->dxc, b->flag, b->st, b->S()));
         STBA_TRY(download(&flag_h, b->flag, 1, b->st));
         if (dxc) STBA_TRY(download(dxc, b->dxc, (size_t)b->n, b->st));
         STBA_HIP(hipStreamSynchronize(b->st));
```

Result: no change. 367.8 (-0.6%).
